# maniac-mc/maniac-mc

Measured on AMD Instinct MI355X. Metric: MC moves/sec, higher is better.
Workload: dtype f64

## Files before the change

include/maniac_gpu.h:

```cpp
#ifndef MANIAC_GPU_H
#define MANIAC_GPU_H

#ifdef __cplusplus
extern "C" {
#endif

#define MGPU_OK 0
#define MGPU_ERR_INVALID_ARG 1
#define MGPU_ERR_HIP 2
#define MGPU_ERR_CAPACITY 3
#define MGPU_ERR_NO_DEVICE 4
#define MGPU_ERR_STATE 5


#define MGPU_MOVE 0
#define MGPU_CREATION 1
#define MGPU_DELETION 2
#define MGPU_NONE 3
#define MGPU_FOURIER_ADD 4

#define MGPU_KERNEL_PAIR 0
#define MGPU_KERNEL_RECIP 1
#define MGPU_KERNEL_COMMIT 2
#define MGPU_KERNEL_SFACTOR 3
#define MGPU_KERNEL_COUNT 4

typedef struct mgpu_engine mgpu_engine;

const char *mgpu_last_error(void);

#define MGPU_ABI_VERSION 2
int mgpu_abi_version(void);

int mgpu_device_count(int *count);


int mgpu_box_prepare(const double box_matrix[9], int *box_type, double *volume,
                     double reciprocal[9], double metrics[9]);

int mgpu_ewald_setup(const double metrics[9], double *rc, double *tol, double *alpha,
                     double *screening_factor, double *fourier_precision, int kmax[3],
                     int *n_kvectors);

int mgpu_ewald_kvectors(const double reciprocal[9], double alpha, const int kmax[3], int n_kvectors,
                        int *kx, int *ky, int *kz, double *k2mag, double *form_factor,
                        double *weights);

int mgpu_coulomb_table_eval(double alpha, double r2_max, int n, const double *r2, double *out);

int mgpu_rng_seed_streams(long long seed, int n_streams, long long *state);
int mgpu_rng_fill(long long *state, int n_streams, int n_per, double *out);
void mgpu_host_prefetch(const void *p, int bytes);


int mgpu_engine_create(mgpu_engine **out, int device, int n_replicas, int n_res,
                       const int *atoms_in_res, const int *mol_capacity, int max_atom,
                       const int *atom_types, const double *charges, const int *is_active,
                       int n_types, const double *epsilon, const double *sigma,
                       const double box_matrix[9], const double bounds_lo[3],
                       double real_space_cutoff, double ewald_tolerance);
int mgpu_engine_destroy(mgpu_engine *e);

int mgpu_engine_get_ewald(const mgpu_engine *e, double *alpha, double *real_space_cutoff,
                          double *ewald_tolerance, int kmax[3], int *n_kvectors, double *volume,
                          int *box_type);
int mgpu_engine_get_kvectors(const mgpu_engine *e, int *kx, int *ky, int *kz, double *k2mag,
                             double *form_factor, double *weights);


int mgpu_replica_set_molecules(mgpu_engine *e, int replica, int t, int n_mol, const double *sites);
int mgpu_replica_get_molecules(mgpu_engine *e, int replica, int t, int *n_mol, double *sites);
int mgpu_replica_num_molecules(const mgpu_engine *e, int replica, int t, int *n_mol);
int mgpu_replica_copy(mgpu_engine *e, int dst, int src);


int mgpu_system_energy(mgpu_engine *e, int replica, double out[6]);

int mgpu_init_structure_factor(mgpu_engine *e, int replica, int mode);
int mgpu_get_structure_factor(mgpu_engine *e, int replica, double *a);
int mgpu_set_structure_factor(mgpu_engine *e, int replica, const double *a);
int mgpu_structure_factor_add(mgpu_engine *e, int replica, int t, const double *sites);


int mgpu_pair_energy_candidates(mgpu_engine *e, int n_candidates, const int *replica, const int *t,
                                const int *m, const int *use_resident, const double *sites,
                                int site_stride, double *e_non_coulomb, double *e_coulomb);

int mgpu_recip_energy_candidates(mgpu_engine *e, int n_candidates, const int *replica, const int *t,
                                 const int *m, const int *kind, const double *sites,
                                 int site_stride, double *u_recip);

#define MGPU_RECIP_TRIAL 0
#define MGPU_RECIP_COMMIT 1
#define MGPU_RECIP_FORM_ROWS 0
#define MGPU_RECIP_FORM_WIDE_VECTOR 1
#define MGPU_RECIP_FORM_WIDE_MFMA 2
#define MGPU_RECIP_FORM_WIDE_MFMA_TILED 3
#define MGPU_RECIP_FORM_PER_K 4
int mgpu_recip_form(const mgpu_engine *e, int n1_max, int kind, int out[4]);

#define MGPU_PAIR_LAYOUT_LEN 12
int mgpu_pair_layout(const mgpu_engine *e, int out[MGPU_PAIR_LAYOUT_LEN]);

int mgpu_self_energy(const mgpu_engine *e, int t, double *e_self);

int mgpu_intra_energy_candidates(mgpu_engine *e, int n_candidates, const int *replica, const int *t,
                                 const int *m, const int *use_resident, const double *sites,
                                 int site_stride, double *u_intra);

int mgpu_trial_energy_candidates(mgpu_engine *e, int n_candidates, const int *replica, const int *t,
                                 const int *m, const double *sites, int site_stride,
                                 double *old_energy, double *new_energy);

int mgpu_commit_candidates(mgpu_engine *e, int n_candidates, const int *replica, const int *t,
                           const int *m, const int *kind, const double *sites, int site_stride,
                           const int *accept);

#define MGPU_LANES 4
int mgpu_replica_set_frames(mgpu_engine *e, int replica, int t, int n_mol, const double *com, const double *off);
int mgpu_replica_get_frames(mgpu_engine *e, int replica, int t, int *n_mol, double *com, double *off);
int mgpu_move_trial_submit(mgpu_engine *e, int lane, int n_candidates, const int *replica, const int *t, const int *m,
                           const int *move, const double *u, double translation_step, double rotation_step);
int mgpu_set_triclinic_moves(mgpu_engine *e, int on);
int mgpu_replica_set_reservoir(mgpu_engine *e, int replica, int t, int n, int cap, const double *off);
int mgpu_replica_get_reservoir(mgpu_engine *e, int replica, int t, int *n, double *off);
int mgpu_farm_snapshot_submit(mgpu_engine *e, int n, const int *replicas, long long *bytes);
int mgpu_farm_snapshot_wait(mgpu_engine *e, const void **data, long long *bytes);
int mgpu_move_trial_decide_submit(mgpu_engine *e, int lane, int n_candidates, const int *replica, const int *t, const int *m,
                                  const int *move, const double *u, double translation_step, double rotation_step,
                                  const double *accept_u, const double *accept_pref, double temperature);
int mgpu_gcmc_trial_decide_submit(mgpu_engine *e, int lane, int n_candidates, const int *replica, const int *t, const int *m,
                                  const int *kind, const double *sites, int site_stride, const double *accept_u,
                                  const double *accept_pref, double temperature);
int mgpu_trial_decide_wait(mgpu_engine *e, int lane, double *old_energy, double *new_energy, int *accepted);
int mgpu_lane_site_buffer(mgpu_engine *e, int lane, int n_max, int site_stride, double **sites);
int mgpu_set_host_team(mgpu_engine *e, int n_threads);
int mgpu_trial_submit(mgpu_engine *e, int lane, int n_candidates, const int *replica, const int *t,
                      const int *m, const double *sites, int site_stride);
int mgpu_trial_wait(mgpu_engine *e, int lane, double *old_energy, double *new_energy);
int mgpu_commit_submit(mgpu_engine *e, int lane, int n_candidates, const int *replica, const int *t,
                       const int *m, const int *kind, const double *sites, int site_stride,
                       const int *accept);

int mgpu_gcmc_trial_submit(mgpu_engine *e, int lane, int n_candidates, const int *replica, const int *t,
                           const int *m, const int *kind, const double *sites, int site_stride);
int mgpu_gcmc_trial_wait(mgpu_engine *e, int lane, double *old_energy, double *new_energy);

int mgpu_replica_replace_molecule(mgpu_engine *e, int replica, int t, int m_dst, int m_src);
int mgpu_replica_set_num_molecules(mgpu_engine *e, int replica, int t, int n_mol);


int mgpu_chain_window_capacity(const mgpu_engine *e, int *max_candidates);
int mgpu_chain_set_wide(mgpu_engine *e, int on);
int mgpu_chain_window(mgpu_engine *e, int replica, int n, const int *t, const int *m, const int *kind, const int *link,
                      const double *sites, int site_stride, const double *accept_u, const double *accept_pref,
                      double temperature, double recip_energy, double *old_energy, double *new_energy,
                      int *first_accepted, int *undecided);
int mgpu_chain_set_margin(mgpu_engine *e, double relative_margin);
int mgpu_chain_get_stats(const mgpu_engine *e, long long *windows, long long *undecided);
int mgpu_chain_set_timing(mgpu_engine *e, int on);
int mgpu_chain_get_timing(mgpu_engine *e, double us[15]);

int mgpu_farm_window_capacity(const mgpu_engine *e, int *max_chains, int *max_in_flight);
int mgpu_farm_window_submit(mgpu_engine *e, int lane, int n, const int *replica, const int *t, const int *m, const int *move,
                            const int *forced, const double *u5, const double *accept_u, const double *accept_pref,
                            const double *slot_u, double t_step, double r_step, double temperature);
int mgpu_farm_window_wait(mgpu_engine *e, int lane, double *old_energy, double *new_energy, int *verdict);
int mgpu_farm_window_flush(mgpu_engine *e);
int mgpu_farm_window_get_stats(const mgpu_engine *e, long long *windows, long long *undecided);

int mgpu_chain_run_capacity(const mgpu_engine *e, int *max_k, int *max_in_flight, int *ring_steps);
int mgpu_chain_run_set_triclinic(mgpu_engine *e, int on);
int mgpu_chain_run_open(mgpu_engine *e, int replica, int k, double t_step, double r_step, double temperature);
int mgpu_chain_run_push(mgpu_engine *e, int n, const int *t, const int *m, const int *move, const double *u5, const double *accept_u);
int mgpu_chain_run_launch(mgpu_engine *e, int n_launches);
int mgpu_chain_run_collect(mgpu_engine *e, int max_steps, int wait, double *old_energy, double *new_energy, int *verdict, int *n_got,
                           int *stalled_at);
int mgpu_chain_run_force(mgpu_engine *e, int step, int accept);
int mgpu_chain_run_close(mgpu_engine *e);
int mgpu_chain_run_get_stats(mgpu_engine *e, long long *launches, long long *steps, long long *void_launches, long long *undecided);
int mgpu_chain_run_get_launches(mgpu_engine *e, int max_launches, int *first, int *consumed, int *n_got);

typedef struct mgpu_comm mgpu_comm;
#define MGPU_COMM_ID_BYTES 128
int mgpu_comm_unique_id(void *id128);
// ... 24 lines not shown
```

maniac_mc_amd/_lib.py:

```python
from __future__ import annotations

import ctypes as C
import os
import subprocess

_HERE = os.path.dirname(os.path.abspath(__file__))
LIB_PATH = os.path.join(_HERE, "libmaniac_hip.so")
CSRC = os.path.join(_HERE, "csrc")
SOURCES = ["mgpu_engine.hip", "mgpu_launch.hip", "mgpu_lanes.hip", "mgpu_windows.hip", "mgpu_host_setup.cpp", "mgpu_comm.cpp"]
HEADERS = ["mgpu_kernels.h", "mgpu_kernels_common.h", "mgpu_kernels_pair.h", "mgpu_kernels_recip.h", "mgpu_kernels_windows.h",
           "mgpu_internal.h", "mgpu_engine.h"]

MGPU_OK = 0
ABI_VERSION = 2
MGPU_MOVE, MGPU_CREATION, MGPU_DELETION, MGPU_NONE = 0, 1, 2, 3
KERNEL_PAIR, KERNEL_RECIP, KERNEL_COMMIT, KERNEL_SFACTOR = 0, 1, 2, 3
RECIP_TRIAL, RECIP_COMMIT = 0, 1
RECIP_FORMS = ("rows", "wide-vector", "wide-mfma", "wide-mfma-tiled", "per-k")
PAIR_LAYOUT_LEN = 12

EXPORTS = [
    "mgpu_last_error", "mgpu_abi_version", "mgpu_device_count", "mgpu_box_prepare", "mgpu_ewald_setup",
    "mgpu_ewald_kvectors", "mgpu_coulomb_table_eval", "mgpu_rng_seed_streams", "mgpu_rng_fill", "mgpu_host_prefetch", "mgpu_engine_create", "mgpu_engine_destroy", "mgpu_engine_get_ewald",
    "mgpu_engine_get_kvectors", "mgpu_replica_set_molecules", "mgpu_replica_get_molecules",
    "mgpu_replica_num_molecules", "mgpu_replica_copy", "mgpu_system_energy", "mgpu_init_structure_factor",
    "mgpu_get_structure_factor", "mgpu_set_structure_factor", "mgpu_structure_factor_add", "mgpu_pair_energy_candidates",
    "mgpu_recip_energy_candidates", "mgpu_recip_form", "mgpu_pair_layout", "mgpu_self_energy", "mgpu_intra_energy_candidates",
    "mgpu_trial_energy_candidates", "mgpu_commit_candidates", "mgpu_trial_submit", "mgpu_trial_wait",
    "mgpu_commit_submit", "mgpu_lane_site_buffer", "mgpu_set_host_team", "mgpu_set_triclinic_moves", "mgpu_replica_set_frames", "mgpu_replica_get_frames", "mgpu_replica_set_reservoir", "mgpu_replica_get_reservoir", "mgpu_farm_snapshot_submit", "mgpu_farm_snapshot_wait", "mgpu_move_trial_submit", "mgpu_move_trial_decide_submit", "mgpu_gcmc_trial_decide_submit", "mgpu_trial_decide_wait", "mgpu_gcmc_trial_submit", "mgpu_gcmc_trial_wait", "mgpu_replica_replace_molecule",
    "mgpu_replica_set_num_molecules", "mgpu_chain_window_capacity", "mgpu_chain_window", "mgpu_chain_set_margin", "mgpu_chain_set_wide",
    "mgpu_chain_get_stats", "mgpu_chain_set_timing", "mgpu_chain_get_timing", "mgpu_farm_window_capacity", "mgpu_farm_window_submit",
    "mgpu_farm_window_wait", "mgpu_farm_window_flush", "mgpu_farm_window_get_stats",
    "mgpu_chain_run_capacity", "mgpu_chain_run_open", "mgpu_chain_run_push", "mgpu_chain_run_launch", "mgpu_chain_run_collect",
    "mgpu_chain_run_force", "mgpu_chain_run_close", "mgpu_chain_run_get_stats", "mgpu_chain_run_get_launches", "mgpu_chain_run_set_triclinic", "mgpu_comm_unique_id", "mgpu_comm_create",
    "mgpu_comm_destroy", "mgpu_comm_rank", "mgpu_allgather_block_stats", "mgpu_append_atom_records", "mgpu_format_fixed", "mgpu_phase_factors", "mgpu_synchronize", "mgpu_profile_enable", "mgpu_profile_reset",
    "mgpu_profile_get",
]


class MgpuError(RuntimeError):
    def __init__(self, code, msg):
        super().__init__(f"maniac_gpu error {code}: {msg}")
        self.code = code


def build(force: bool = False, verbose: bool = False) -> str:
    srcs = [os.path.join(CSRC, s) for s in SOURCES]
    deps = srcs + [os.path.join(CSRC, h) for h in HEADERS if os.path.exists(os.path.join(CSRC, h))]
    deps.append(os.path.join(_HERE, "..", "include", "maniac_gpu.h"))
    if not force and os.path.exists(LIB_PATH):
        if os.path.getmtime(LIB_PATH) >= max(os.path.getmtime(d) for d in deps):
            return LIB_PATH
    from concurrent.futures import ThreadPoolExecutor
    obj_dir = os.path.join(_HERE, "..", "build", "hip_obj")
    os.makedirs(obj_dir, exist_ok=True)
    flags = ["--offload-arch=gfx950", "-O3", "-fPIC", "-std=c++17", "-fopenmp"]

    def compile_one(src):
        obj = os.path.join(obj_dir, os.path.basename(src) + ".o")
        cmd = ["hipcc"] + flags + ["-c", src, "-o", obj]
        if verbose:
            print(" ".join(cmd), flush=True)
        subprocess.check_call(cmd)
        return obj

    with ThreadPoolExecutor(max_workers=min(len(srcs), max(1, (os.cpu_count() or 2) // 2))) as pool:
        objs = list(pool.map(compile_one, srcs))
    cmd = ["hipcc", "--offload-arch=gfx950", "-fPIC", "-shared", "-fopenmp", "-o", LIB_PATH] + objs + \
          ["-L/opt/rocm/lib", "-lrccl", "-Wl,-rpath,/opt/rocm/lib"]
    if verbose:
        print(" ".join(cmd), flush=True)
    subprocess.check_call(cmd)
    return LIB_PATH


def source_digest() -> str:
    import hashlib
    h = hashlib.sha256()
    files = sorted(os.path.join(CSRC, f) for f in os.listdir(CSRC) if f.endswith((".hip", ".cpp", ".h")))
    files.append(os.path.join(_HERE, "..", "include", "maniac_gpu.h"))
    for f in files:
        h.update(os.path.basename(f).encode() + b"\0")
        with open(f, "rb") as fh:
            h.update(fh.read())
    return h.hexdigest()


_lib = None


def lib():
    global _lib
    if _lib is None:
        if not os.path.exists(LIB_PATH):
            raise RuntimeError(f"{LIB_PATH} is missing: build it with `python -c 'import __graft_entry__ as g; "
                               "g.build()'` (hipcc --offload-arch=gfx950); there is no CPU fallback")
        L = C.CDLL(LIB_PATH)
        L.mgpu_last_error.restype = C.c_char_p
        L.mgpu_abi_version.restype = C.c_int
        if L.mgpu_abi_version() != ABI_VERSION:
            raise RuntimeError(f"{LIB_PATH} reports ABI version {L.mgpu_abi_version()}, this package binds version {ABI_VERSION}: "
                               "rebuild it (python -c 'import __graft_entry__ as g; g.build()')")
        for name in EXPORTS:
            if name in ("mgpu_last_error", "mgpu_host_prefetch"):
                continue
            getattr(L, name).restype = C.c_int
        _lib = L
    return _lib


# ... 4 lines not shown
```

maniac_mc_amd/csrc/mgpu_engine.h:

```cpp
#ifndef MGPU_ENGINE_H
#define MGPU_ENGINE_H

#include <hip/hip_runtime.h>
#include <hip/hip_ext.h>

#include <algorithm>
#include <cmath>
#include <cstdio>
#include <cstdlib>
#include <cstring>
#include <deque>
#include <omp.h>
#include <string>
#include <atomic>
#include <mutex>
#include <type_traits>
#include <vector>

#include "../../include/maniac_gpu.h"
#include "mgpu_internal.h"
#include "mgpu_kernels.h"

namespace mgpu {

// ... 118 lines not shown
            if (d_res) (void)hipFree(d_res);
            if (d_tickets) (void)hipFree(d_tickets);
            h_recs = nullptr; h_out = nullptr; h_tag = nullptr; d_part = nullptr; d_res = nullptr; d_tickets = nullptr;
            cap = 0;
            pending.clear();
        }
    } farm;
    void release() {
        farm.release();
        if (commit_staged_ev) { (void)hipEventDestroy(commit_staged_ev); commit_staged_ev = nullptr; }
        d_items.release(); d_items2.release(); d_sites.release(); d_partials.release(); d_out.release();
        d_scratch.release(); d_recip_sums.release();
        d_tickets.release();
        h_in.release(); h_commit.release(); h_out.release();
    }
};
constexpr int kLanes = 4;
constexpr int kFarmDepth = 4;
constexpr int kFarmMaxChains = 4096;
constexpr int kRunRingSteps = 4096;
constexpr int kRunMaxInFlight = 64;
constexpr int kRunLaunchRing = 256;
constexpr int kRunLogMax = 1024;
constexpr size_t kChainWideRowsBytes = (size_t)kChainMaxCand * kFarmWideSites * 3 * sizeof(double);

template <class F>
void with_bools(F &&f) { f(); }
template <class F, class... Rest>
void with_bools(F &&f, bool first, Rest... rest) {
    if (first) with_bools([&](auto... cs) { f(std::true_type{}, cs...); }, rest...);
    else with_bools([&](auto... cs) { f(std::false_type{}, cs...); }, rest...);
}
template <int Lo, int Hi, class F>
bool with_int(int v, F &&f) {
    if constexpr (Lo > Hi) return false;
    else {
        if (v == Lo) { f(std::integral_constant<int, Lo>{}); return true; }
        return with_int<Lo + 1, Hi>(v, f);
    }
}
template <class F, class... Done>
void for_all_bools(F &&f, std::integral_constant<int, 0>, Done... done) { f(done...); }
template <int N, class F, class... Done>
void for_all_bools(F &&f, std::integral_constant<int, N>, Done... done) {
    for_all_bools(f, std::integral_constant<int, N - 1>{}, done..., std::false_type{});
    for_all_bools(f, std::integral_constant<int, N - 1>{}, done..., std::true_type{});
}

}

using namespace mgpu;

struct mgpu_engine {
    int device = 0;
    int n_replicas = 0;
    Lane lanes[kLanes];
    Topo tp{};
    BoxDev bx{};
    std::vector<int> atoms_in_res, mol_capacity, is_active, atom_types;
    std::vector<double> charges, epsilon, sigma;
    std::vector<int> kx, ky, kz;
    std::vector<double> k2mag, form_factor, weights;
    std::vector<int> h_nmol;
    std::vector<char> in_range;
    double rc = 0, tol = 0, alpha = 0, volume = 0;
    int box_type = 0, kmax[3] = {0, 0, 0}, nk = 0;
    double box_matrix[9]{}, bounds_lo[3]{}, reciprocal[9]{}, metrics[9]{};
    double *d_pos = nullptr;
    int *d_nmol = nullptr;
    double2 *d_A = nullptr;
    int *d_kpack = nullptr;
    double *d_kw = nullptr;
    int *d_trj = nullptr;
    double2 *d_tw = nullptr;
    int *d_kslot = nullptr;
    std::vector<int> kslot;
    int n_slots = 0;
    RecipRow *d_rrows = nullptr;
    int *d_row_first = nullptr;
    int n_rtasks = 0, n_rrows = 0;
    double2 *d_pair_tab = nullptr;
    char *d_coul_tab = nullptr;
    size_t coul_bytes = 0;
    int n_cu = 256;
    int pair_blocks_per_cu = kPairBlock >= 1024 ? 1 : 2;
    int pair_nsplit = 1;
    std::vector<double> self_of_type;
    bool rows_contiguous = false;
    bool recip_no_mfma = false;
    bool pair_fast_fold = true;
    bool recip_force_per_k = false;
    double *d_res_q = nullptr;
    int *d_res_atype = nullptr;
    std::vector<std::vector<int>> site_perm;
    std::vector<char> frozen;
    bool any_frozen = false;
    int flat_groups = 0, flat_planes = 0;
    int *d_atom_ty = nullptr;
    std::vector<std::vector<double>> frozen_ref;
    std::vector<char> frozen_same;
    std::vector<int> frozen_diff;
    bool frozen_batch = true;
    int host_team = 1;
    double *d_com = nullptr, *d_off = nullptr;
    std::vector<char> frames_ok;
    std::vector<char> frames_tight;
    std::vector<char> frames_held;
    std::vector<double *> rsv_ptr;
    std::vector<int> rsv_cap;
    std::vector<char> rsv_tight;
    double **d_rsv = nullptr;
    int *d_rsv_nc = nullptr;
    bool tri_moves = false;
    bool rsv_any = false;
    bool pair_flat = false;
    int *d_atom_res = nullptr, *d_atom_mol = nullptr;
    double *d_atom_q = nullptr;
    double *d_atom_q_on = nullptr;
    double2 *d_phase_tab = nullptr;
    double2 *d_S = nullptr;
    hipStream_t &stream = lanes[0].stream;
    DevBuf &d_items = lanes[0].d_items, &d_items2 = lanes[0].d_items2, &d_sites = lanes[0].d_sites,
           &d_partials = lanes[0].d_partials, &d_out = lanes[0].d_out;
    HostBuf &h_out = lanes[0].h_out;
    HostBuf h_stage;
    DevBuf d_snap, d_snap_items;
    HostBuf h_snap, h_snap_items;
    size_t snap_bytes = 0;
    bool snap_pending = false;
    struct Chain {
        double *h_out = nullptr;
        unsigned long long *h_tag = nullptr;
        Topo *d_topo = nullptr;
        bool topo_stale = true;
        ChainResult *d_res = nullptr;
        double2 *d_part = nullptr;
        double2 *d_alt = nullptr;
        int *d_ticket = nullptr;
        unsigned long long seq = 0;
        double margin = 16.0 * 2.220446049250313e-16;
        long long windows = 0, undecided = 0;
        bool timing = false;
        bool wide = false;
        double *h_rows = nullptr;
        size_t wide_lds_opted = 0;
    } chain;
    double2 *d_A_alt = nullptr;
    int *d_acur = nullptr;
    std::atomic<bool> a_switched{false};
    std::vector<unsigned long long> alt_owner;
    std::atomic<unsigned long long> trial_stamps{0};
    bool commit_pass = false;
    std::mutex alt_mu;
    struct Farm {
        int *d_stalled = nullptr;
        std::atomic<long long> windows{0}, undecided{0};
        std::mutex mu;
    } farm;
    struct Run {
        bool open = false;
        bool triclinic = false;
        int replica = -1, k = 0;
        double t_step = 0.0, r_step = 0.0, temperature = 0.0;
        bool fast = false;
        RunState *d_state = nullptr;
        RunRec *d_ring = nullptr, *h_ring = nullptr;
        int *h_pushed = nullptr;
        double *h_out = nullptr;
        unsigned long long *h_step_tag = nullptr;
        unsigned long long *h_launch = nullptr;
        double2 *d_part = nullptr, *d_alt = nullptr;
        ChainResult *d_res = nullptr;
        int *d_ticket = nullptr;
        long long pushed = 0, collected = 0;
        long long stalled_at = -1;
        bool dev_stalled = false;
        unsigned long long seq = 0, seq_done = 0;
        long long launches = 0, steps = 0, void_launches = 0, undecided = 0;
        std::deque<std::pair<int, int>> log;
    } run;
    bool profiling = false;
};

namespace mgpu {

const char *last_error_text();
int use_device(const mgpu_engine *e);
int prof_begin(mgpu_engine *e, Lane &ln, int kernel, hipEvent_t *a, hipEvent_t *b);
int prof_end(mgpu_engine *e, Lane &ln, int kernel, hipEvent_t a, hipEvent_t b);
int prof_collect(mgpu_engine *e, Lane &ln);
void finish_decided(mgpu_engine *e, Lane &ln);
void frozen_changed(mgpu_engine *e, int replica, int t);
int sync_lane(mgpu_engine *e, Lane &ln);
int sync_stream(mgpu_engine *e);
int sync_all_lanes(mgpu_engine *e);
int check_candidate(const mgpu_engine *e, int c, int replica, int t, int m, bool need_resident);
bool sites_in_range(const mgpu_engine *e, const double *sites, int n_sites);
bool replica_in_range(const mgpu_engine *e, int replica);
inline bool has_reservoir(const mgpu_engine *e, size_t idx) { return !e->rsv_ptr.empty() && e->rsv_ptr[idx] != nullptr; }
enum { kAdmitFrames = 1, kAdmitMove = 2, kAdmitInsertion = 4, kAdmitRange = 8, kAdmitAll = 15 };
inline int admit_built(const mgpu_engine *e, size_t idx, int k, int mv, int checks, const char *who, const char *noun, int c,
                       std::string &msg, char &ok, bool &fast) {
    if ((checks & kAdmitFrames) && (!e->d_com || !e->frames_ok[idx])) {
        msg = std::string(who) + ": no molecule frames for " + noun + " " + std::to_string(c) + " (mgpu_replica_set_frames)";
        return MGPU_ERR_STATE;
    }
    if ((checks & kAdmitMove) && (mv < 1 || mv > 4 || (k == MGPU_MOVE) != (mv <= 2) || (k == MGPU_CREATION) != (mv == 3))) {
        msg = std::string(who) + ": move code does not match the candidate kind";
        return MGPU_ERR_INVALID_ARG;
    }
    if ((checks & kAdmitInsertion) && k == MGPU_CREATION && !e->frames_held[idx] && !has_reservoir(e, idx)) {
        msg = std::string(who) + ": an insertion copies the geometry of molecule 1 of its type, and this type has never held one on this replica";
        return MGPU_ERR_STATE;
    }
    if ((checks & kAdmitRange) && k != MGPU_DELETION) { ok = e->frames_tight[idx]; fast = fast && ok; }
    return MGPU_OK;
}
int engine_nsplit(const mgpu_engine *e);
void permute_frozen_rows(const mgpu_engine *e, double *rows, int n_rows, int site_stride, const int *t);
bool any_frozen(const mgpu_engine *e, int n, const int *t);
int upload_sites(Lane &ln, const double *sites, int n_rows, int site_stride);
int upload_sites(mgpu_engine *e, const double *sites, int n_rows, int site_stride, const int *t);
double self_energy_host(const mgpu_engine *e, int t);
int normalize_A(mgpu_engine *e);
int alt_reserve(mgpu_engine *e);
void alt_forget(mgpu_engine *e, int replica);
bool one_record_per_replica(Lane &ln, int n_replicas, const int *replica, int n);
int wait_for_tag(hipStream_t stream, const volatile unsigned long long *tag, int n, unsigned long long seq, long long first_check,
                 long long check_every, const char *what);
int farm_clear_stall(mgpu_engine *e, int replica);
int chain_topo(mgpu_engine *e, const Topo **d_topo);
void chain_run_release(mgpu_engine *e);
int launch_pair(mgpu_engine *e, Lane &ln, const PairItem *d_items, int n_items, int common_n1, int site_stride,
                int nsplit, double *d_lj, double *d_c, bool ordered = false, double2 *host_partials = nullptr,
                bool fused = false, bool fast_fold = false, bool skip_frozen = false);
int frozen_chunk_atoms(const mgpu_engine *e, int n_atoms);
int launch_frozen(mgpu_engine *e, Lane &ln, const PairItem *d_items, int n_items, int n1, int site_stride, bool fused, bool fast_fold,
                  int t_frozen, double2 *d_scratch, double2 *d_extra);
static_assert((3 * sizeof(PairItem) + sizeof(RecipItem)) % 8 == 0, "the items end 8-byte aligned: TrialStaging::moves is their end");
inline TrialStaging trial_staging(int n, int site_stride, bool built, bool reservoir_pick, bool decide) {
    return trial_staging<sizeof(PairItem), sizeof(RecipItem), sizeof(DecideItem)>(n, site_stride, built, reservoir_pick, decide);
}
inline size_t lane_site_buffer_bytes(int n_max, int site_stride) {
    return lane_site_buffer_bytes<sizeof(PairItem), sizeof(RecipItem), sizeof(DecideItem)>(n_max, site_stride);
}
static_assert(sizeof(double2) == kLdsPhase && sizeof(int4) == kLdsRowRec, "mgpu_internal.h sizes the LDS tables with these");
inline int recip_ktot(const mgpu_engine *e) { return recip_ktot(e->kmax); }
inline size_t recip_rows_lds_bytes(const mgpu_engine *e, int n1_max) { return recip_rows_lds_bytes(recip_ktot(e), e->n_rrows, n1_max); }
inline size_t farm_resolver_scratch_bytes(int nsplit) { return (size_t)kPairWaves * (4 * nsplit + 4) * sizeof(double); }
bool recip_by_rows(const mgpu_engine *e, int n1_max);
struct RecipPlan {
    int form = MGPU_RECIP_FORM_ROWS;
    bool by_rows = true;
    int tile = 1;
    int mfma_tile = 0;
    int wide_rpt = 0;
    int wide_nss = 0;
    size_t lds = 0;
    size_t wide_lds = 0;
};
RecipPlan recip_plan(const mgpu_engine *e, int n1_max, bool wide_ok);
void recip_groups(const mgpu_engine *e, const RecipItem *items, int n, std::vector<RecipGroup> &groups, std::vector<int> &order);
int launch_recip(mgpu_engine *e, Lane &ln, const RecipItem *d_items, int n_items, int n1_max, int site_stride,
                 bool commit, double2 *A_base, double *d_u, double *d_u_old = nullptr, const AcceptBits *accept = nullptr,
                 const double *sites_override = nullptr, const DecideArgs *decide = nullptr, bool store_alt = false);
int launch_commit_switch(mgpu_engine *e, Lane &ln, const RecipItem *d_items, int n_items, int site_stride, const AcceptBits &accept);
int launch_sfactor(mgpu_engine *e, int replica, double2 *dst);
int launch_intra(mgpu_engine *e, Lane &ln, const PairItem *d_items, int n_items, const double *d_sites, int site_stride, double *d_out);

constexpr int kHostPartMin = 1024;
constexpr int kMaxHostParts = 16;
static int host_parts(const mgpu_engine *e, int n) {
    return (e->host_team > 1 && n >= kHostPartMin) ? std::min(e->host_team, kMaxHostParts) : 1;
}
static void part_range(int n, int parts, int part, int &c0, int &c1) {
    const int words = (n + 31) / 32;
    c0 = std::min(n, (int)((long long)words * part / parts) * 32);
    c1 = std::min(n, (int)((long long)words * (part + 1) / parts) * 32);
}
template <class F>
static void for_parts(int parts, F &&f) {
    if (parts <= 1) { f(0); return; }
#pragma omp parallel for num_threads(parts) schedule(static, 1)
    for (int part = 0; part < parts; ++part) f(part);
}
struct PartError {
    int c = -1, rc = MGPU_OK;
    std::string msg;
    void set(int cand, int code, const std::string &m) { if (c < 0) { c = cand; rc = code; msg = m; } }
};
static int report_first(const PartError *errs, int parts) {
    const PartError *first = nullptr;
    for (int q = 0; q < parts; ++q)
        if (errs[q].c >= 0 && (!first || errs[q].c < first->c)) first = &errs[q];
    return first ? set_error(first->rc, first->msg) : MGPU_OK;
}

template <class Item>
int common_site_count(const mgpu_engine *e, const std::vector<Item> &items) {
    int n1 = 0;
    for (const auto &it : items) {
// ... 11 lines not shown
```

maniac_mc_amd/csrc/mgpu_engine.hip:

```cpp
#include "mgpu_engine.h"

namespace mgpu {

static thread_local std::string g_last_error;

int set_error(int code, const std::string &msg) {
    g_last_error = msg;
    return code;
}
const char *last_error_text() { return g_last_error.c_str(); }

int use_device(const mgpu_engine *e) {
    HIP_TRY(hipSetDevice(e->device));
    return MGPU_OK;
}

int prof_begin(mgpu_engine *e, Lane &ln, int kernel, hipEvent_t *a, hipEvent_t *b) {
    if (!e->profiling) return MGPU_OK;
    for (hipEvent_t *ev : {a, b}) {
        if (!ln.ev_pool.empty()) { *ev = ln.ev_pool.back(); ln.ev_pool.pop_back(); }
        else HIP_TRY(hipEventCreate(ev));
    }
    (void)kernel;
    return MGPU_OK;
// ... 11 lines not shown
        ln.prof[p.kernel].total_ms += ms;
        ln.ev_pool.push_back(p.a);
        ln.ev_pool.push_back(p.b);
    }
    ln.pending.clear();
    return MGPU_OK;
}

void finish_decided(mgpu_engine *e, Lane &ln);
void frozen_changed(mgpu_engine *e, int replica, int t);
int sync_lane(mgpu_engine *e, Lane &ln) {
    HIP_TRY(hipStreamSynchronize(ln.stream));
    ln.dirty = false;
    if (ln.decided_n) finish_decided(e, ln);
    return prof_collect(e, ln);
}
int sync_stream(mgpu_engine *e) { return sync_lane(e, e->lanes[0]); }
int sync_all_lanes(mgpu_engine *e) {
    for (auto &ln : e->lanes)
        if (&ln == &e->lanes[0] || ln.dirty || !ln.pending.empty())
            if (int rc = sync_lane(e, ln)) return rc;
    if (e->a_switched) return normalize_A(e);
    alt_forget(e, -1);
    return MGPU_OK;
}

void finish_decided(mgpu_engine *e, Lane &ln) {
    const int n = ln.decided_n;
    ln.decided_n = 0;
    const int *flags = (const int *)((const char *)ln.h_out.p + ln.result.flags_bytes());
    const RecipItem *items = ln.h_trial_items;
    for (int c = 0; c < n; ++c) {
        if (!flags[c]) continue;
        const int idx = items[c].replica * e->tp.n_res + items[c].t;
        if (items[c].kind == MGPU_CREATION) e->h_nmol[idx] += 1;
        if (items[c].kind == MGPU_DELETION) e->h_nmol[idx] -= 1;
        if (items[c].kind != MGPU_DELETION && !(c < (int)ln.cand_ok.size() && ln.cand_ok[c])) e->in_range[idx] = 0;
        frozen_changed(e, items[c].replica, items[c].t);
    }
    ln.forget_trial();
}

bool one_record_per_replica(Lane &ln, int n_replicas, const int *replica, int n) {
    if ((int)ln.mark.size() != n_replicas) ln.mark.assign(n_replicas, -1);
    bool twice = false;
    for (int c = 0; c < n; ++c) {
        twice = twice || ln.mark[replica[c]] == -3;
        ln.mark[replica[c]] = -3;
    }
    for (int c = 0; c < n; ++c) ln.mark[replica[c]] = -1;
    return !twice;
}

void frozen_changed(mgpu_engine *e, int replica, int t) {
    if (!e->frozen[t]) return;
    auto clear = [&](int r) {
        char &f = e->frozen_same[(size_t)r * e->tp.n_res + t];
        if (f) { e->frozen_diff[t] += 1; f = 0; }
    };
    if (replica == 0) for (int r = 0; r < e->n_replicas; ++r) clear(r);
    else clear(replica);
}
int check_candidate(const mgpu_engine *e, int c, int replica, int t, int m, bool need_resident) {
    if (replica < 0 || replica >= e->n_replicas)
        return set_error(MGPU_ERR_INVALID_ARG, "candidate " + std::to_string(c) + ": replica out of range");
    if (t < 0 || t >= e->tp.n_res)
        return set_error(MGPU_ERR_INVALID_ARG, "candidate " + std::to_string(c) + ": residue type out of range");
    const int nm = e->h_nmol[replica * e->tp.n_res + t];
    if (m >= nm || m < -1)
        return set_error(MGPU_ERR_INVALID_ARG, "candidate " + std::to_string(c) + ": molecule slot " +
                                                   std::to_string(m) + " not live (count " + std::to_string(nm) + ")");
    if (need_resident && m < 0)
        return set_error(MGPU_ERR_INVALID_ARG, "candidate " + std::to_string(c) + ": needs a resident molecule");
    return MGPU_OK;
}

constexpr double kFastFoldRange = 0.745;
bool sites_in_range(const mgpu_engine *e, const double *sites, int n_sites) {
    for (int i = 0; i < n_sites; ++i)
        for (int d = 0; d < 3; ++d)
            if (!(std::fabs(sites[3 * (size_t)i + d] - e->bx.ctr[d]) <= kFastFoldRange * e->bx.L[d])) return false;
    return true;
}
bool replica_in_range(const mgpu_engine *e, int replica) {
    for (int t = 0; t < e->tp.n_res; ++t)
        if (!e->in_range[(size_t)replica * e->tp.n_res + t]) return false;
    return true;
}

int engine_nsplit(const mgpu_engine *e) {
    int units = 0;
    for (int t = 0; t < e->tp.n_res; ++t) {
        const int cap = e->tp.cap[t], n1 = e->tp.n1[t];
        units += e->tp.site_major[t] ? cap * ((n1 + 63) / 64) : n1 * ((cap + 63) / 64);
    }
    int cap_split = 32, per_wave = 2;
    if (e->n_replicas >= 48 && e->n_replicas <= 1024) {
        const int want = (e->n_replicas < 512 ? 1024 : 2048) / e->n_replicas;
        cap_split = 2;
        while (cap_split * 2 <= std::min(want, 32)) cap_split *= 2;
    } else if (e->n_replicas >= 256) {
        per_wave = 8;
        int want = std::max(1, e->n_cu * 64 / e->n_replicas);
        if (units <= 128) want *= 2;
        const int cap_want = e->n_replicas >= 1024 ? std::min(want, 4) : std::min(want / 4, 16);
        cap_split = 1;
        while (cap_split * 2 <= cap_want) cap_split *= 2;
    }
    int ns = std::max(1, std::min(units / per_wave, cap_split));
    if (const char *ov = std::getenv("MGPU_PAIR_NSPLIT")) ns = std::max(1, std::min(std::atoi(ov), std::max(1, units)));
    return ns;
}

void permute_frozen_rows(const mgpu_engine *e, double *rows, int n_rows, int site_stride, const int *t) {
    std::vector<double> tmp;
    for (int c = 0; c < n_rows; ++c) {
        if (t[c] < 0 || t[c] >= e->tp.n_res || !e->frozen[t[c]]) continue;
        const int n1 = e->tp.n1[t[c]];
        if (n1 > site_stride) continue;
        double *r = rows + (size_t)c * site_stride * 3;
        tmp.assign(r, r + (size_t)n1 * 3);
        const int *perm = e->site_perm[t[c]].data();
        for (int a = 0; a < n1; ++a)
            for (int d = 0; d < 3; ++d) r[(size_t)perm[a] * 3 + d] = tmp[(size_t)a * 3 + d];
    }
}
bool any_frozen(const mgpu_engine *e, int n, const int *t) {
    for (int c = 0; c < n; ++c)
        if (t[c] >= 0 && t[c] < e->tp.n_res && e->frozen[t[c]]) return true;
    return false;
}

int upload_sites(Lane &ln, const double *sites, int n_rows, int site_stride) {
    if (!sites || n_rows == 0) return MGPU_OK;
    ln.forget_trial();
    const size_t bytes = (size_t)n_rows * site_stride * 3 * sizeof(double);
    int rc = ln.d_sites.reserve(bytes);
    if (rc) return rc;
    HIP_TRY(hipMemcpyAsync(ln.d_sites.p, sites, bytes, hipMemcpyHostToDevice, ln.stream));
    return MGPU_OK;
}
int upload_sites(mgpu_engine *e, const double *sites, int n_rows, int site_stride, const int *t) {
    if (sites && n_rows > 0 && any_frozen(e, n_rows, t)) {
        const size_t bytes = (size_t)n_rows * site_stride * 3 * sizeof(double);
        int rc = e->h_stage.reserve(bytes);
        if (rc) return rc;
        std::memcpy(e->h_stage.p, sites, bytes);
        permute_frozen_rows(e, (double *)e->h_stage.p, n_rows, site_stride, t);
        if ((rc = upload_sites(e->lanes[0], (const double *)e->h_stage.p, n_rows, site_stride))) return rc;
        HIP_TRY(hipStreamSynchronize(e->lanes[0].stream));
        return MGPU_OK;
    }
    return upload_sites(e->lanes[0], sites, n_rows, site_stride);
}

double self_energy_host(const mgpu_engine *e, int t) {
    double s = 0.0;
    const double sqrtpi = std::sqrt(kPi);
    for (int a = 0; a < e->tp.n1[t]; ++a) {
        const double q = e->charges[(size_t)t * e->tp.max_atom + a];
        if (std::fabs(q) < kErrorTol) continue;
        s = s - e->alpha / sqrtpi * (q * q);
    }
    return s * kEps0InvEvA / kKbEvK;
}

// ... 243 lines not shown
        for (size_t r = 0; r < rrows.size(); ++r)
            for (int j = 0; j <= e->kmax[2]; ++j)
                if (plus[r][j] >= 0 || minus[r][j] >= 0) rtasks.push_back(RecipTask{plus[r][j], minus[r][j], (int)r, j});
        size_t covered = 0;
        for (const auto &tk : rtasks) covered += (tk.kp >= 0) + (tk.km >= 0);
        if (covered != (size_t)e->nk) { rrows.clear(); rtasks.clear(); }
        e->rows_contiguous = !rtasks.empty() && e->kmax[2] < 255;
        for (size_t ti = 1; ti < rtasks.size(); ++ti)
            if (rtasks[ti].row == rtasks[ti - 1].row && rtasks[ti].j != rtasks[ti - 1].j + 1) e->rows_contiguous = false;
    }
    e->n_rrows = (int)rrows.size();
    e->n_rtasks = (int)rtasks.size();
    e->kslot.assign(e->nk, 0);
    std::vector<int> trj(rtasks.size());
    std::vector<double2> tw(rtasks.size());
    if (e->n_rtasks > 0) {
        e->n_slots = 2 * e->n_rtasks;
        for (size_t ti = 0; ti < rtasks.size(); ++ti) {
            const RecipTask &tk = rtasks[ti];
            trj[ti] = (tk.row << 8) | tk.j | (tk.kp >= 0 ? kTaskHasP : 0) | (tk.km >= 0 ? kTaskHasM : 0);
            tw[ti] = make_double2(tk.kp >= 0 ? kw[tk.kp] : 0.0, tk.km >= 0 ? kw[tk.km] : 0.0);
            if (tk.kp >= 0) e->kslot[tk.kp] = 2 * (int)ti;
            if (tk.km >= 0) e->kslot[tk.km] = 2 * (int)ti + 1;
        }
    } else {
        e->n_slots = e->nk;
        for (int i = 0; i < e->nk; ++i) e->kslot[i] = i;
    }
    bx.n_slots = e->n_slots;
    std::vector<double2> ptab((size_t)n_types * n_types);
    for (int i = 0; i < n_types * n_types; ++i) ptab[i] = make_double2(4.0 * epsilon[i], sigma[i] * sigma[i]);
    std::vector<int> atype0((size_t)n_res * max_atom, 0);
    std::vector<double> q_dev((size_t)n_res * max_atom, 0.0);
    for (int t = 0; t < n_res; ++t)
        for (int a = 0; a < atoms_in_res[t]; ++a) {
            const int ap = e->site_perm[t][a];
            atype0[(size_t)t * max_atom + ap] = atom_types[(size_t)t * max_atom + a] - 1;
            q_dev[(size_t)t * max_atom + ap] = charges[(size_t)t * max_atom + a];
        }
    std::vector<int> a_res(tp.n_cap_atoms), a_mol(tp.n_cap_atoms), a_ty(tp.n_cap_atoms);
    std::vector<double> a_q(tp.n_cap_atoms);
    for (int t = 0; t < n_res; ++t)
        for (int m = 0; m < tp.cap[t]; ++m)
            for (int a = 0; a < tp.n1[t]; ++a) {
                const int ap = e->site_perm[t][a];
                const int j = tp.site_major[t] ? tp.seg_off[t] + m * tp.n1[t] + ap : tp.seg_off[t] + ap * tp.cap[t] + m;
                a_res[j] = t; a_mol[j] = m; a_q[j] = charges[(size_t)t * max_atom + a];
                a_ty[j] = atom_types[(size_t)t * max_atom + a] - 1;
            }

    auto fail = [&](int code) { mgpu_engine_destroy(e); return code; };
#define HIP_TRY_E(expr)                                                                                          \
    do {                                                                                                         \
        hipError_t err__ = (expr);                                                                               \
        if (err__ != hipSuccess)                                                                                 \
            return fail(set_error(MGPU_ERR_HIP, std::string(#expr) + ": " + hipGetErrorString(err__)));          \
    } while (0)
    HIP_TRY_E(hipSetDevice(device));
    for (auto &ln : e->lanes) HIP_TRY_E(hipStreamCreateWithFlags(&ln.stream, hipStreamNonBlocking));
    const size_t ncap = tp.n_cap_atoms, R = n_replicas;
    const int ktot = recip_ktot(e);
    HIP_TRY_E(hipMalloc(&e->d_pos, R * 3 * ncap * sizeof(double)));
    HIP_TRY_E(hipMemset(e->d_pos, 0, R * 3 * ncap * sizeof(double)));
    HIP_TRY_E(hipMalloc(&e->d_nmol, R * n_res * sizeof(int)));
    HIP_TRY_E(hipMemset(e->d_nmol, 0, R * n_res * sizeof(int)));
    HIP_TRY_E(hipMalloc(&e->d_A, R * e->n_slots * sizeof(double2)));
    HIP_TRY_E(hipMemset(e->d_A, 0, R * e->n_slots * sizeof(double2)));
    HIP_TRY_E(hipMalloc(&e->d_kpack, e->nk * sizeof(int)));
    HIP_TRY_E(hipMalloc(&e->d_kw, e->nk * sizeof(double)));
    HIP_TRY_E(hipMalloc(&e->d_pair_tab, ptab.size() * sizeof(double2)));
    {
        std::vector<CoulRow> rows;
        const double sum_len = e->metrics[0] + e->metrics[1] + e->metrics[2];
        const double s_max = bx.triclinic ? sum_len * sum_len
                                          : 0.25 * (bx.L[0] * bx.L[0] + bx.L[1] * bx.L[1] + bx.L[2] * bx.L[2]) * 1.0001;
        int idx_base = 0;
        if (int rc2 = build_coulomb_table(e->alpha, std::max(s_max, 1.0), rows, &idx_base)) return fail(rc2);
        e->bx.coul_idx_base = idx_base;
        e->bx.coul_last_row = (int)rows.size() - 1;
        e->coul_bytes = rows.size() * sizeof(CoulRow);
        if (e->coul_bytes + 16 * 1024 > 150 * 1024) return fail(set_error(MGPU_ERR_CAPACITY, "Coulomb table does not fit LDS"));
        HIP_TRY_E(hipMalloc(&e->d_coul_tab, e->coul_bytes));
        HIP_TRY_E(hipMemcpy(e->d_coul_tab, rows.data(), e->coul_bytes, hipMemcpyHostToDevice));
    }
    {
        hipDeviceProp_t prop;
        HIP_TRY_E(hipGetDeviceProperties(&prop, device));
        e->n_cu = std::max(1, prop.multiProcessorCount);
        e->pair_nsplit = engine_nsplit(e);
    }
    HIP_TRY_E(hipMalloc(&e->d_res_q, e->charges.size() * sizeof(double)));
    HIP_TRY_E(hipMalloc(&e->d_res_atype, atype0.size() * sizeof(int)));
    HIP_TRY_E(hipMalloc(&e->d_atom_res, ncap * sizeof(int)));
    HIP_TRY_E(hipMalloc(&e->d_atom_mol, ncap * sizeof(int)));
    HIP_TRY_E(hipMalloc(&e->d_atom_q, ncap * sizeof(double)));
    HIP_TRY_E(hipMalloc(&e->d_atom_q_on, ncap * sizeof(double)));
    HIP_TRY_E(hipMalloc(&e->d_phase_tab, (size_t)ktot * ncap * sizeof(double2)));
    HIP_TRY_E(hipMalloc(&e->d_S, e->n_slots * sizeof(double2)));
    HIP_TRY_E(hipMemset(e->d_S, 0, e->n_slots * sizeof(double2)));
    HIP_TRY_E(hipMalloc(&e->d_kslot, e->nk * sizeof(int)));
    HIP_TRY_E(hipMemcpy(e->d_kslot, e->kslot.data(), e->nk * sizeof(int), hipMemcpyHostToDevice));
    HIP_TRY_E(hipMemcpy(e->d_kpack, kpack.data(), e->nk * sizeof(int), hipMemcpyHostToDevice));
    if (e->n_rtasks > 0) {
        HIP_TRY_E(hipMalloc(&e->d_trj, trj.size() * sizeof(int)));
        HIP_TRY_E(hipMalloc(&e->d_tw, tw.size() * sizeof(double2)));
        HIP_TRY_E(hipMalloc(&e->d_rrows, rrows.size() * sizeof(RecipRow)));
        HIP_TRY_E(hipMemcpy(e->d_trj, trj.data(), trj.size() * sizeof(int), hipMemcpyHostToDevice));
        HIP_TRY_E(hipMemcpy(e->d_tw, tw.data(), tw.size() * sizeof(double2), hipMemcpyHostToDevice));
        HIP_TRY_E(hipMemcpy(e->d_rrows, rrows.data(), rrows.size() * sizeof(RecipRow), hipMemcpyHostToDevice));
        std::vector<int> row_first(rrows.size() + 1, (int)rtasks.size());
        for (int ti = (int)rtasks.size() - 1; ti >= 0; --ti) row_first[rtasks[ti].row] = ti;
        HIP_TRY_E(hipMalloc(&e->d_row_first, row_first.size() * sizeof(int)));
        HIP_TRY_E(hipMemcpy(e->d_row_first, row_first.data(), row_first.size() * sizeof(int), hipMemcpyHostToDevice));
    }
    HIP_TRY_E(hipMemcpy(e->d_kw, kw.data(), e->nk * sizeof(double), hipMemcpyHostToDevice));
    HIP_TRY_E(hipMemcpy(e->d_pair_tab, ptab.data(), ptab.size() * sizeof(double2), hipMemcpyHostToDevice));
    HIP_TRY_E(hipMemcpy(e->d_res_q, q_dev.data(), q_dev.size() * sizeof(double), hipMemcpyHostToDevice));
    HIP_TRY_E(hipMalloc(&e->d_atom_ty, ncap * sizeof(int)));
    HIP_TRY_E(hipMemcpy(e->d_atom_ty, a_ty.data(), ncap * sizeof(int), hipMemcpyHostToDevice));
    tp.slot_q = e->d_atom_q;
    tp.slot_ty = e->d_atom_ty;
    HIP_TRY_E(hipMemcpy(e->d_res_atype, atype0.data(), atype0.size() * sizeof(int), hipMemcpyHostToDevice));
    HIP_TRY_E(hipMemcpy(e->d_atom_res, a_res.data(), ncap * sizeof(int), hipMemcpyHostToDevice));
    HIP_TRY_E(hipMemcpy(e->d_atom_mol, a_mol.data(), ncap * sizeof(int), hipMemcpyHostToDevice));
    HIP_TRY_E(hipMemcpy(e->d_atom_q, a_q.data(), ncap * sizeof(double), hipMemcpyHostToDevice));
    {
        std::vector<double> a_q_on(a_q);
        for (double &q : a_q_on)
            if (!(std::fabs(q) >= kErrorTol)) q = 0.0;
        HIP_TRY_E(hipMemcpy(e->d_atom_q_on, a_q_on.data(), ncap * sizeof(double), hipMemcpyHostToDevice));
    }
#undef HIP_TRY_E
    e->self_of_type.resize(n_res);
    for (int t = 0; t < n_res; ++t) e->self_of_type[t] = self_energy_host(e, t);
    *out = e;
    return MGPU_OK;
}

int mgpu_engine_destroy(mgpu_engine *e) {
    if (!e) return MGPU_OK;
    (void)hipSetDevice(e->device);
    for (auto &ln : e->lanes) if (ln.stream) (void)hipStreamSynchronize(ln.stream);
    for (void *p : {(void *)e->d_pos, (void *)e->d_nmol, (void *)e->d_A, (void *)e->d_kpack, (void *)e->d_kw,
                    (void *)e->d_pair_tab, (void *)e->d_coul_tab, (void *)e->d_res_q, (void *)e->d_res_atype, (void *)e->d_atom_res,
                    (void *)e->d_atom_mol, (void *)e->d_atom_q, (void *)e->d_atom_q_on, (void *)e->d_phase_tab, (void *)e->d_S, (void *)e->d_trj,
                    (void *)e->d_tw, (void *)e->d_kslot, (void *)e->d_rrows, (void *)e->d_row_first, (void *)e->d_atom_ty, (void *)e->d_com, (void *)e->d_off})
        if (p) (void)hipFree(p);
    for (double *p : e->rsv_ptr)
        if (p) (void)hipFree(p);
    for (void *p : {(void *)e->d_rsv, (void *)e->d_rsv_nc})
        if (p) (void)hipFree(p);
    e->h_stage.release();
    e->h_snap.release();
    e->h_snap_items.release();
    e->d_snap.release();
    e->d_snap_items.release();
    for (void *p : {(void *)e->chain.h_out, (void *)e->chain.h_tag, (void *)e->chain.h_rows})
        if (p) (void)hipHostFree(p);
    for (void *p : {(void *)e->chain.d_res, (void *)e->chain.d_part, (void *)e->chain.d_ticket, (void *)e->chain.d_topo, (void *)e->chain.d_alt,
                    (void *)e->d_A_alt, (void *)e->d_acur, (void *)e->farm.d_stalled})
        if (p) (void)hipFree(p);
    chain_run_release(e);
    for (auto &ln : e->lanes) {
        ln.release();
        for (auto &p : ln.pending) { (void)hipEventDestroy(p.a); (void)hipEventDestroy(p.b); }
        if (ln.stream) (void)hipStreamDestroy(ln.stream);
    }
    for (auto &ln : e->lanes)
        for (auto ev : ln.ev_pool) (void)hipEventDestroy(ev);
    delete e;
    return MGPU_OK;
}

int mgpu_engine_get_ewald(const mgpu_engine *e, double *alpha, double *rc, double *tol, int kmax[3], int *nk,
                          double *volume, int *box_type) {
    if (!e) return set_error(MGPU_ERR_INVALID_ARG, "null engine");
    if (alpha) *alpha = e->alpha;
    if (rc) *rc = e->rc;
    if (tol) *tol = e->tol;
    if (kmax) { kmax[0] = e->kmax[0]; kmax[1] = e->kmax[1]; kmax[2] = e->kmax[2]; }
    if (nk) *nk = e->nk;
    if (volume) *volume = e->volume;
    if (box_type) *box_type = e->box_type;
    return MGPU_OK;
}

int mgpu_engine_get_kvectors(const mgpu_engine *e, int *kx, int *ky, int *kz, double *k2mag, double *ff, double *w) {
    if (!e) return set_error(MGPU_ERR_INVALID_ARG, "null engine");
    if (kx) std::memcpy(kx, e->kx.data(), e->nk * sizeof(int));
    if (ky) std::memcpy(ky, e->ky.data(), e->nk * sizeof(int));
    if (kz) std::memcpy(kz, e->kz.data(), e->nk * sizeof(int));
    if (k2mag) std::memcpy(k2mag, e->k2mag.data(), e->nk * sizeof(double));
    if (ff) std::memcpy(ff, e->form_factor.data(), e->nk * sizeof(double));
    if (w) std::memcpy(w, e->weights.data(), e->nk * sizeof(double));
    return MGPU_OK;
}


static int check_replica_t(const mgpu_engine *e, int replica, int t) {
    if (!e) return set_error(MGPU_ERR_INVALID_ARG, "null engine");
    if (replica < 0 || replica >= e->n_replicas) return set_error(MGPU_ERR_INVALID_ARG, "replica out of range");
    if (t < 0 || t >= e->tp.n_res) return set_error(MGPU_ERR_INVALID_ARG, "residue type out of range");
    return MGPU_OK;
}

int mgpu_replica_set_molecules(mgpu_engine *e, int replica, int t, int n_mol, const double *sites) {
    int rc = check_replica_t(e, replica, t);
    if (rc) return rc;
    if (n_mol < 0 || n_mol > e->tp.cap[t]) return set_error(MGPU_ERR_CAPACITY, "n_mol exceeds the residue type's mol_capacity");
    if (n_mol > 0 && !sites) return set_error(MGPU_ERR_INVALID_ARG, "null sites");
    if ((rc = use_device(e))) return rc;
    const Topo &tp = e->tp;
    const int n1 = tp.n1[t], cap = tp.cap[t];
    const size_t seg = (size_t)n1 * cap;
    rc = e->h_stage.reserve(3 * seg * sizeof(double));
    if (rc) return rc;
    double *st = (double *)e->h_stage.p;
    std::memset(st, 0, 3 * seg * sizeof(double));
    const int *perm = e->site_perm[t].data();
    for (int m = 0; m < n_mol; ++m)
        for (int a = 0; a < n1; ++a) {
            const size_t j = tp.site_major[t] ? (size_t)m * n1 + perm[a] : (size_t)a * cap + m;
            for (int d = 0; d < 3; ++d) st[d * seg + j] = sites[((size_t)m * n1 + a) * 3 + d];
        }
    if ((rc = sync_all_lanes(e))) return rc;
    if ((rc = farm_clear_stall(e, replica))) return rc;
    for (int d = 0; d < 3; ++d)
// ... 617 lines not shown
```

maniac_mc_amd/csrc/mgpu_host_setup.cpp:

```cpp
#include <cmath>
#include <cstdio>
#include <cstring>
#include <string>
#include <vector>

#include "../../include/maniac_gpu.h"
#include "mgpu_internal.h"

namespace mgpu {

static inline void cross3(const double a[3], const double b[3], double c[3]) {
    c[0] = a[1] * b[2] - a[2] * b[1];
    c[1] = a[2] * b[0] - a[0] * b[2];
    c[2] = a[0] * b[1] - a[1] * b[0];
}
static inline double dot3(const double a[3], const double b[3]) {
    return a[0] * b[0] + a[1] * b[1] + a[2] * b[2];
}

int box_prepare(const double m[9], int *box_type, double *volume, double rcp[9], double metrics[9]) {
    if (!m || !box_type || !volume || !rcp || !metrics) return set_error(MGPU_ERR_INVALID_ARG, "box_prepare: null argument");
    const double od[6] = {m[1], m[2], m[3], m[5], m[6], m[7]};
    double mx = 0.0;
    for (double v : od) mx = std::fmax(mx, std::fabs(v));
// ... 82 lines not shown
    for (int i = 0; i < nk; ++i) w[i] = std::exp(-k2mag[i] / (4.0 * a2)) / k2mag[i];
    return MGPU_OK;
}

int build_coulomb_table(double alpha, double s_max, std::vector<CoulRow> &rows, int *idx_base) {
    if (!(alpha > 0.0) || !(s_max > 0.0) || !std::isfinite(s_max))
        return set_error(MGPU_ERR_INVALID_ARG, "build_coulomb_table: bad alpha / range");
    int emax = kCoulEmin;
    while (std::ldexp(1.0, emax + 1) <= s_max) ++emax;
    if (emax - kCoulEmin + 1 > 40) return set_error(MGPU_ERR_CAPACITY, "build_coulomb_table: range too large");
    const int per_oct = 1 << kCoulM, n_oct = emax - kCoulEmin + 1;
    rows.assign((size_t)n_oct * per_oct + 1, CoulRow{});
    *idx_base = (1023 + kCoulEmin) * per_oct;
    constexpr int N = kCoulDeg + 1;
    const long double pi = 3.14159265358979323846264338327950288L;
    long double node[N], cosjk[N][N];
    for (int k = 0; k < N; ++k) {
        node[k] = cosl(pi * (2 * k + 1) / (2.0L * N));
        for (int j = 0; j < N; ++j) cosjk[j][k] = cosl(pi * j * (2 * k + 1) / (2.0L * N));
    }
    long double T[N][N] = {};
    T[0][0] = 1.0L;
    T[1][1] = 1.0L;
    for (int j = 2; j < N; ++j)
        for (int i = 0; i < N; ++i) T[j][i] = (i > 0 ? 2.0L * T[j - 1][i - 1] : 0.0L) - T[j - 2][i];
    long double binom[N][N] = {};
    for (int j = 0; j < N; ++j) {
        binom[j][0] = 1.0L;
        for (int i = 1; i <= j; ++i) binom[j][i] = binom[j - 1][i - 1] + (i <= j - 1 ? binom[j - 1][i] : 0.0L);
    }
    const long double al = alpha;
    for (int o = 0; o < n_oct; ++o)
        for (int q = 0; q < per_oct; ++q) {
            const long double base = ldexpl(1.0L, kCoulEmin + o);
            const long double a = base * (1.0L + (long double)q / per_oct), b = base * (1.0L + (long double)(q + 1) / per_oct);
            long double f[N], c[N], mono[N] = {}, tc[N] = {};
            for (int k = 0; k < N; ++k) {
                const long double sv = 0.5L * (a + b) + 0.5L * (b - a) * node[k], r = sqrtl(sv);
                f[k] = erfcl(al * r) / r;
            }
            for (int j = 0; j < N; ++j) {
                long double acc = 0.0L;
                for (int k = 0; k < N; ++k) acc += f[k] * cosjk[j][k];
                c[j] = acc * 2.0L / N;
            }
            c[0] *= 0.5L;
            for (int j = 0; j < N; ++j)
                for (int i = 0; i <= j; ++i) mono[i] += c[j] * T[j][i];
            for (int j = 0; j < N; ++j)
                for (int i = 0; i <= j; ++i) {
                    const long double sign = ((j - i) & 1) ? -1.0L : 1.0L;
                    tc[i] += mono[j] * binom[j][i] * ldexpl(1.0L, i) * sign;
                }
            CoulRow &row = rows[(size_t)o * per_oct + q];
            const int sh = kCoulM - (kCoulEmin + o);
            for (int i = 0; i < 5; ++i) row.c[i] = (double)ldexpl(tc[i], sh * i);
            row.c5 = (float)ldexpl(tc[5], sh * 5);
            row.c6 = (float)ldexpl(tc[6], sh * 6);
        }
    return MGPU_OK;
}

double coulomb_table_eval_host(const std::vector<CoulRow> &rows, int idx_base, double alpha, double s) {
    unsigned long long bits;
    std::memcpy(&bits, &s, 8);
    const int hi = (int)(bits >> 32);
    int row = (hi >> (20 - kCoulM)) - idx_base;
    if (row < 0) {
        const double r = std::sqrt(s);
        return std::erfc(alpha * r) / r;
    }
    const int last = (int)rows.size() - 1;
    if (row > last) row = last;
    const unsigned long long ab = bits & ~((1ull << (52 - kCoulM)) - 1);
    double a;
    std::memcpy(&a, &ab, 8);
    const double t = s - a;
    const CoulRow &r = rows[row];
    double p = std::fma((double)r.c6, t, (double)r.c5);
    for (int i = 4; i >= 0; --i) p = std::fma(p, t, r.c[i]);
    return p;
}

}

namespace {

bool format_fixed(char *out, int w, int d, double x) {
    if (!std::isfinite(x)) return false;
    const bool neg = std::signbit(x);
    const double ax = std::fabs(x);
    auto stars = [&]() { std::memset(out, '*', (size_t)w); return true; };
    int e = 0;
    unsigned long long m = 0;
    if (ax != 0.0) {
        const double fr = std::frexp(ax, &e);
        m = (unsigned long long)std::ldexp(fr, 53);
        e -= 53;
    }
    if (e >= 0 && m != 0) return stars();
    static const unsigned long long p10[] = {1ull, 10ull, 100ull, 1000ull, 10000ull, 100000ull, 1000000ull, 10000000ull, 100000000ull,
                                             1000000000ull};
    if (d < 0 || d > 9) return false;
    unsigned __int128 P = (unsigned __int128)m * p10[d];
    unsigned __int128 N = 0;
    const int sh = -e;
    if (m != 0) {
        if (sh >= 127) {
            N = 0;
        } else {
            N = P >> sh;
            const unsigned __int128 rem = P & ((((unsigned __int128)1) << sh) - 1), half = ((unsigned __int128)1) << (sh - 1);
            if (rem > half || (rem == half && (N & 1))) N += 1;
        }
    }
    if (N >> 64) return stars();
    const unsigned long long n64 = (unsigned long long)N, ip = n64 / p10[d], fp = n64 % p10[d];
    char tmp[64];
    int len = 0;
    char digits[24];
    int nd = 0;
    unsigned long long v = ip;
    do { digits[nd++] = (char)('0' + v % 10); v /= 10; } while (v);
    if (neg) tmp[len++] = '-';
    for (int k = nd - 1; k >= 0; --k) tmp[len++] = digits[k];
    tmp[len++] = '.';
    for (int k = d - 1; k >= 0; --k) tmp[len++] = (char)('0' + (fp / p10[k]) % 10);
    if (len > w) {
        if (ip == 0 && len - 1 == w) {
            std::memmove(tmp + (neg ? 1 : 0), tmp + (neg ? 2 : 1), (size_t)(len - (neg ? 2 : 1)));
            len -= 1;
        } else {
            return stars();
        }
    }
    std::memset(out, ' ', (size_t)(w - len));
    std::memcpy(out + (w - len), tmp, (size_t)len);
    return true;
}

void format_int(char *out, int w, long long v) {
    char tmp[32];
    const int len = std::snprintf(tmp, sizeof tmp, "%lld", v);
    if (len > w) { std::memset(out, '*', (size_t)w); return; }
    std::memset(out, ' ', (size_t)(w - len));
    std::memcpy(out + (w - len), tmp, (size_t)len);
}

}

using mgpu::set_error;

extern "C" {

int mgpu_append_atom_records(const char *path, int n, int first_serial, const int *mol, const int *type, const double *charge,
                             const double *xyz) {
    if (!path || n < 0 || !type || !xyz || (mol && !charge)) return set_error(MGPU_ERR_INVALID_ARG, "append_atom_records: bad argument");
    const int reclen = mol ? (6 + 1 + 6 + 1 + 4 + 1 + 12 + 3 * 13 + 1) : (6 + 1 + 4 + 3 * 13 + 1);
    std::vector<char> buf((size_t)n * reclen);
    for (int i = 0; i < n; ++i) {
        char *r = buf.data() + (size_t)i * reclen;
        int at = 0;
        format_int(r + at, 6, (long long)first_serial + i); at += 6;
        r[at++] = ' ';
        if (mol) {
            format_int(r + at, 6, mol[i]); at += 6;
            r[at++] = ' ';
        }
        format_int(r + at, 4, type[i]); at += 4;
        if (mol) {
            r[at++] = ' ';
            if (!format_fixed(r + at, 12, 8, charge[i])) return set_error(MGPU_ERR_INVALID_ARG, "append_atom_records: charge not finite");
            at += 12;
        }
        for (int dd = 0; dd < 3; ++dd) {
            r[at++] = ' ';
            if (!format_fixed(r + at, 12, 7, xyz[(size_t)i * 3 + dd])) return set_error(MGPU_ERR_INVALID_ARG, "append_atom_records: coordinate not finite");
            at += 12;
        }
        r[at++] = '\n';
    }
    FILE *f = std::fopen(path, "ab");
    if (!f) return set_error(MGPU_ERR_STATE, std::string("append_atom_records: cannot open ") + path);
    const size_t wrote = buf.empty() ? 0 : std::fwrite(buf.data(), 1, buf.size(), f);
    const int rc = std::fclose(f);
    if (wrote != buf.size() || rc != 0) return set_error(MGPU_ERR_STATE, std::string("append_atom_records: short write to ") + path);
    return MGPU_OK;
}

int mgpu_format_fixed(int n, const double *x, int w, int d, char *out) {
    if (n < 0 || !x || !out || w < 1 || w > 40) return set_error(MGPU_ERR_INVALID_ARG, "format_fixed: bad argument");
    for (int i = 0; i < n; ++i)
        if (!format_fixed(out + (size_t)i * w, w, d, x[i])) std::memset(out + (size_t)i * w, '?', (size_t)w);
    return MGPU_OK;
}

int mgpu_box_prepare(const double box_matrix[9], int *box_type, double *volume, double reciprocal[9], double metrics[9]) {
    return mgpu::box_prepare(box_matrix, box_type, volume, reciprocal, metrics);
}

int mgpu_ewald_setup(const double metrics[9], double *rc, double *tol, double *alpha, double *screening_factor,
                     double *fourier_precision, int kmax[3], int *n_kvectors) {
    return mgpu::ewald_setup(metrics, rc, tol, alpha, screening_factor, fourier_precision, kmax, n_kvectors);
}

int mgpu_coulomb_table_eval(double alpha, double r2_max, int n, const double *r2, double *out) {
    if (n < 0 || (n > 0 && (!r2 || !out))) return mgpu::set_error(MGPU_ERR_INVALID_ARG, "mgpu_coulomb_table_eval: bad argument");
    std::vector<mgpu::CoulRow> rows;
    int idx_base = 0;
    int rc = mgpu::build_coulomb_table(alpha, r2_max, rows, &idx_base);
    if (rc) return rc;
    for (int k = 0; k < n; ++k) out[k] = mgpu::coulomb_table_eval_host(rows, idx_base, alpha, r2[k]);
    return MGPU_OK;
}

void mgpu_host_prefetch(const void *p, int bytes) {
    for (int o = 0; o < bytes; o += 64) __builtin_prefetch((const char *)p + o, 0, 3);
}

int mgpu_rng_seed_streams(long long seed, int n_streams, long long *state) {
    if (n_streams < 0 || (n_streams > 0 && !state)) return mgpu::set_error(MGPU_ERR_INVALID_ARG, "mgpu_rng_seed_streams: bad argument");
    auto splitmix = [](unsigned long long &x) {
        unsigned long long z = (x += 0x9e3779b97f4a7c15ULL);
        z = (z ^ (z >> 30)) * 0xbf58476d1ce4e5b9ULL;
        z = (z ^ (z >> 27)) * 0x94d049bb133111ebULL;
        return z ^ (z >> 31);
    };
    unsigned long long base = (unsigned long long)seed;
    base = splitmix(base);
    for (int r = 0; r < n_streams; ++r) {
        unsigned long long x = base + 0xd1342543de82ef95ULL * (unsigned long long)(r + 1);
        unsigned long long w[4];
        do {
            for (auto &v : w) v = splitmix(x);
        } while ((w[0] | w[1] | w[2] | w[3]) == 0ULL);
        for (int i = 0; i < 4; ++i) state[4 * (size_t)r + i] = (long long)w[i];
    }
    return MGPU_OK;
}

namespace {
inline void rng_fill_scalar(unsigned long long *st, int n, int n_per, double *out) {
    for (int r = 0; r < n; ++r) {
        unsigned long long s0 = st[4 * (size_t)r], s1 = st[4 * (size_t)r + 1], s2 = st[4 * (size_t)r + 2], s3 = st[4 * (size_t)r + 3];
        double *o = out + (size_t)r * n_per;
        for (int i = 0; i < n_per; ++i) {
            o[i] = (double)((s0 + s3) >> 11) * (1.0 / 9007199254740992.0);
            const unsigned long long t = s1 << 17;
            s2 ^= s0; s3 ^= s1; s1 ^= s2; s0 ^= s3;
            s2 ^= t;
            s3 = (s3 << 45) | (s3 >> 19);
        }
        st[4 * (size_t)r] = s0; st[4 * (size_t)r + 1] = s1; st[4 * (size_t)r + 2] = s2; st[4 * (size_t)r + 3] = s3;
    }
}
#if defined(__x86_64__)
#include <immintrin.h>
__attribute__((target("avx2"))) void rng_fill_avx2(unsigned long long *st, int n, int n_per, double *out) {
    const __m256i magic = _mm256_set1_epi64x(0x4330000000000000LL);
    const __m256d two52 = _mm256_set1_pd(4503599627370496.0), two32 = _mm256_set1_pd(4294967296.0);
    const __m256d scale = _mm256_set1_pd(1.0 / 9007199254740992.0);
    const __m256i lo_mask = _mm256_set1_epi64x(0xffffffffLL);
    int r = 0;
    for (; r + 4 <= n; r += 4) {
        const __m256i a = _mm256_loadu_si256((const __m256i *)(st + 4 * (size_t)r)), b = _mm256_loadu_si256((const __m256i *)(st + 4 * (size_t)r + 4));
        const __m256i c = _mm256_loadu_si256((const __m256i *)(st + 4 * (size_t)r + 8)), d = _mm256_loadu_si256((const __m256i *)(st + 4 * (size_t)r + 12));
        const __m256i ab_lo = _mm256_unpacklo_epi64(a, b), ab_hi = _mm256_unpackhi_epi64(a, b);
        const __m256i cd_lo = _mm256_unpacklo_epi64(c, d), cd_hi = _mm256_unpackhi_epi64(c, d);
        __m256i s0 = _mm256_permute2x128_si256(ab_lo, cd_lo, 0x20), s1 = _mm256_permute2x128_si256(ab_hi, cd_hi, 0x20);
        __m256i s2 = _mm256_permute2x128_si256(ab_lo, cd_lo, 0x31), s3 = _mm256_permute2x128_si256(ab_hi, cd_hi, 0x31);
        for (int i = 0; i < n_per; ++i) {
            const __m256i x = _mm256_srli_epi64(_mm256_add_epi64(s0, s3), 11);
            const __m256d hi = _mm256_sub_pd(_mm256_castsi256_pd(_mm256_or_si256(_mm256_srli_epi64(x, 32), magic)), two52);
            const __m256d lo = _mm256_sub_pd(_mm256_castsi256_pd(_mm256_or_si256(_mm256_and_si256(x, lo_mask), magic)), two52);
            const __m256d v = _mm256_mul_pd(_mm256_add_pd(_mm256_mul_pd(hi, two32), lo), scale);
            alignas(32) double tmp[4];
            _mm256_store_pd(tmp, v);
            for (int q = 0; q < 4; ++q) out[(size_t)(r + q) * n_per + i] = tmp[q];
            const __m256i t = _mm256_slli_epi64(s1, 17);
            s2 = _mm256_xor_si256(s2, s0); s3 = _mm256_xor_si256(s3, s1); s1 = _mm256_xor_si256(s1, s2); s0 = _mm256_xor_si256(s0, s3);
            s2 = _mm256_xor_si256(s2, t);
            s3 = _mm256_or_si256(_mm256_slli_epi64(s3, 45), _mm256_srli_epi64(s3, 19));
        }
        const __m256i t0 = _mm256_unpacklo_epi64(s0, s1), t1 = _mm256_unpackhi_epi64(s0, s1);
        const __m256i t2 = _mm256_unpacklo_epi64(s2, s3), t3 = _mm256_unpackhi_epi64(s2, s3);
        _mm256_storeu_si256((__m256i *)(st + 4 * (size_t)r), _mm256_permute2x128_si256(t0, t2, 0x20));
        _mm256_storeu_si256((__m256i *)(st + 4 * (size_t)r + 4), _mm256_permute2x128_si256(t1, t3, 0x20));
        _mm256_storeu_si256((__m256i *)(st + 4 * (size_t)r + 8), _mm256_permute2x128_si256(t0, t2, 0x31));
        _mm256_storeu_si256((__m256i *)(st + 4 * (size_t)r + 12), _mm256_permute2x128_si256(t1, t3, 0x31));
    }
    if (r < n) rng_fill_scalar(st + 4 * (size_t)r, n - r, n_per, out + (size_t)r * n_per);
}
#endif
}

// ... 21 lines not shown
```

maniac_mc_amd/csrc/mgpu_internal.h:

```cpp
#ifndef MGPU_INTERNAL_H
#define MGPU_INTERNAL_H

#include <algorithm>
#include <cstddef>
#include <string>
#include <vector>

namespace mgpu {

constexpr double kPi = 3.14159265358979323846;
constexpr double kTwoPi = 2.0 * kPi;
constexpr double kEps0InvEvA = 14.40198;
constexpr double kKbEvK = 8.6173852e-5;
constexpr double kErrorTol = 1.0e-10;

int set_error(int code, const std::string &msg);

int box_prepare(const double m[9], int *box_type, double *volume, double rcp[9], double metrics[9]);
int ewald_setup(const double metrics[9], double *rc, double *tol, double *alpha, double *screening,
                double *fourier_precision, int kmax[3], int *nk);
int ewald_kvectors(const double rcp[9], double alpha, const int kmax[3], int nk, int *kx, int *ky, int *kz,
                   double *k2mag, double *ff, double *w);

constexpr int kCoulM = 6;
constexpr int kCoulDeg = 6;
constexpr int kCoulEmin = -2;
constexpr double kCoulSlowBelow = 0.25;
struct CoulRow {
    double c[5];
    float c5, c6;
};
static_assert(sizeof(CoulRow) == 48, "CoulRow must be three 16-byte LDS reads");
constexpr int kCoulRowVec = sizeof(CoulRow) / 16;
int build_coulomb_table(double alpha, double s_max, std::vector<CoulRow> &rows, int *idx_base);
double coulomb_table_eval_host(const std::vector<CoulRow> &rows, int idx_base, double alpha, double s);

constexpr size_t kLdsDefaultMax = 64 * 1024;
constexpr size_t kLdsPhase = 16, kLdsRowRec = 16;
inline int recip_ktot(const int kmax[3]) { return kmax[0] + kmax[1] + kmax[2] + 3; }
inline size_t recip_lds_bytes(int ktot, int n1) { return (size_t)2 * n1 * ktot * kLdsPhase + (size_t)n1 * sizeof(double); }
inline size_t recip_rows_lds_bytes(int ktot, int n_rrows, int n1) {
    return recip_lds_bytes(ktot, n1) + (size_t)n_rrows * (2 * n1 * kLdsPhase);
}
inline size_t recip_wide_lds_bytes(int ktot, int n_rrows, size_t nss, int rpt, bool mfma) {
    return nss * ktot * kLdsPhase + (size_t)rpt * nss * kLdsPhase + nss * sizeof(double) + (mfma ? (size_t)n_rrows * kLdsRowRec : 0);
}
constexpr size_t kRecipTileBytes = 48 * 1024;
constexpr size_t kRecipRowsLdsMax = 40 * 1024;
constexpr size_t kRecipWideTableBytes = 40 * 1024, kRecipWideLdsBytes = 60 * 1024;
inline int recip_tile_sites(int ktot, int n1_max) {
    return std::max(1, std::min(n1_max, (int)(kRecipTileBytes / recip_lds_bytes(ktot, 1))));
}
inline int recip_wide_rows_per_tile(int ktot, int n_rrows, int n1_max) {
    const size_t nss = (size_t)2 * n1_max, tables = recip_wide_lds_bytes(ktot, 0, nss, 0, false);
    if (tables > kRecipWideTableBytes) return 0;
    const int rpt = (int)((kRecipWideLdsBytes - tables) / (nss * kLdsPhase));
    return rpt >= 8 ? std::min(rpt, n_rrows) : 0;
}
inline int recip_wide_mfma_tile(int ktot, int n_rrows, int n1_max) {
    const size_t nss = ((size_t)2 * n1_max + 3) & ~(size_t)3;
    const size_t per_ss = recip_wide_lds_bytes(ktot, 0, 1, 0, false), fixed = recip_wide_lds_bytes(ktot, n_rrows, 0, 0, true);
    if (fixed + 4 * per_ss > kRecipWideLdsBytes) return 0;
    const size_t fit = ((kRecipWideLdsBytes - fixed) / per_ss) & ~(size_t)3;
    const size_t n_tiles = (nss + fit - 1) / fit;
    return (int)((((nss + n_tiles - 1) / n_tiles) + 3) & ~(size_t)3);
}

constexpr int kWideRowSites = 64;
constexpr size_t wide_k_front_bytes() { return (size_t)kWideRowSites * 3 * sizeof(double) + 2 * (size_t)kWideRowSites * 4 * sizeof(double); }
inline size_t chain_wide_k_lds_bytes(size_t form_bytes) { return wide_k_front_bytes() + form_bytes; }
inline size_t chain_wide_pair_at(size_t coul_bytes) { return (coul_bytes + 15) & ~(size_t)15; }
constexpr size_t wide_pair_slab_bytes(int pair_waves, int site_chunk) {
    return (size_t)pair_waves * (((size_t)kWideRowSites * 3 + (size_t)site_chunk * 4) * sizeof(double) + (size_t)site_chunk * sizeof(int));
}
inline size_t chain_wide_pair_lds_bytes(size_t coul_bytes, int pair_waves, int site_chunk) {
    return chain_wide_pair_at(coul_bytes) + wide_pair_slab_bytes(pair_waves, site_chunk);
}
inline size_t chain_resolver_lds_bytes(int n_ent, int nsplit) { return (size_t)n_ent * nsplit * kLdsPhase; }
inline int chain_window_steps_by_lds(int nsplit) { return (int)(kLdsDefaultMax / chain_resolver_lds_bytes(2, nsplit)); }
inline size_t chain_run_resolver_lds_bytes(int k, int nsplit) { return chain_resolver_lds_bytes(2 * k, nsplit); }

struct TrialStaging {
    int row_sites, frame_at, pick_at;
    size_t sites, pair_items, k_items, intra_items, moves, uniforms, decide_items, total;
};
template <size_t PairB, size_t RecipB, size_t DecideB>
inline TrialStaging trial_staging(int n, int site_stride, bool built, bool reservoir_pick, bool decide) {
    const auto up8 = [](size_t v) { return (v + 7) & ~(size_t)7; };
    TrialStaging s{};
    s.row_sites = built ? 2 * site_stride + 1 + (reservoir_pick ? 1 : 0) : site_stride;
    s.frame_at = built ? site_stride : 0;
    s.pick_at = built && reservoir_pick ? 2 * site_stride + 1 : 0;
    s.pair_items = (size_t)n * s.row_sites * 3 * sizeof(double);
    s.k_items = s.pair_items + 2 * (size_t)n * PairB;
    s.intra_items = s.k_items + (size_t)n * RecipB;
    s.moves = up8(s.intra_items + (size_t)n * PairB);
    s.uniforms = s.moves + up8((size_t)n * sizeof(int));
    s.decide_items = up8(built ? s.uniforms + (size_t)5 * n * sizeof(double) : s.moves);
    s.total = s.decide_items + (decide ? (size_t)n * DecideB : 0);
    return s;
}
template <size_t PairB, size_t RecipB, size_t DecideB>
inline size_t lane_site_buffer_bytes(int n_max, int site_stride) {
    const TrialStaging host = trial_staging<PairB, RecipB, DecideB>(n_max, site_stride, false, false, true);
    const TrialStaging built = trial_staging<PairB, RecipB, DecideB>(n_max, site_stride, true, true, true);
    return std::max(host.total + 16, built.total + 32 + (size_t)n_max * sizeof(int) + 8 - (built.uniforms - built.moves));
}
struct TrialResult {
    size_t partials, u_old, u_new, intra, extra, flags, total;
    size_t flags_bytes() const { return flags * sizeof(double); }
};
inline TrialResult trial_result(int n, int n_partials, int n_pair, bool frozen_extra, bool decide) {
    TrialResult r{};
    r.u_old = 2 * (size_t)n_partials;
    r.u_new = r.u_old + n;
    r.intra = r.u_new + n;
    r.extra = r.intra + n;
    r.flags = r.extra + (frozen_extra ? 2 * (size_t)n_pair : 0);
// ... 8 lines not shown
```

maniac_mc_amd/csrc/mgpu_kernels_common.h:

```cpp
#ifndef MGPU_KERNELS_COMMON_H
#define MGPU_KERNELS_COMMON_H

#include <hip/hip_runtime.h>

#include <type_traits>

#include "mgpu_internal.h"

namespace mgpu {

constexpr int kMaxRes = 8;
constexpr int kBlock = 256;
constexpr int kWavesPerBlock = kBlock / 64;
constexpr int kSiteChunk = 32;
#ifndef MGPU_PAIR_BLOCK
#define MGPU_PAIR_BLOCK 512
#endif
#ifndef MGPU_PAIR_MINWAVES
#define MGPU_PAIR_MINWAVES 4
#endif
constexpr int kPairBlock = MGPU_PAIR_BLOCK;
constexpr int kPairWaves = kPairBlock / 64;
constexpr int kMaxTypes = 16;
constexpr int kMaxGrp = 32;
// ... 146 lines not shown
__device__ __forceinline__ double image_r2_search27(double dx, double dy, double dz, const double *__restrict__ m) {
    double best = 1.7976931348623157e308;
    for (int sx = -1; sx <= 1; ++sx)
        for (int sy = -1; sy <= 1; ++sy)
            for (int sz = -1; sz <= 1; ++sz) {
                const double tx = dx + sx * m[0] + sy * m[1] + sz * m[2];
                const double ty = dy + sx * m[3] + sy * m[4] + sz * m[5];
                const double tz = dz + sx * m[6] + sy * m[7] + sz * m[8];
                const double t2 = fma(tz, tz, fma(ty, ty, tx * tx));
                best = t2 < best ? t2 : best;
            }
    return best;
}

template <bool TRI>
__device__ __forceinline__ double image_r2(double dx, double dy, double dz, const BoxDev &bx) {
    if constexpr (TRI) {
        if (bx.tri_lower) {
            double r2;
            if (!image_r2_tri_lower(dx, dy, dz, bx, r2)) r2 = image_r2_search27(dx, dy, dz, bx.m);
            return r2;
        }
    }
    if constexpr (!TRI) {
        dx = min_image(dx, bx.L[0], bx.invL[0]);
        dy = min_image(dy, bx.L[1], bx.invL[1]);
        dz = min_image(dz, bx.L[2], bx.invL[2]);
        return fma(dz, dz, fma(dy, dy, dx * dx));
    } else {
        double best = 1.7976931348623157e308;
        for (int sx = -1; sx <= 1; ++sx)
            for (int sy = -1; sy <= 1; ++sy)
                for (int sz = -1; sz <= 1; ++sz) {
                    const double tx = dx + sx * bx.m[0] + sy * bx.m[1] + sz * bx.m[2];
                    const double ty = dy + sx * bx.m[3] + sy * bx.m[4] + sz * bx.m[5];
                    const double tz = dz + sx * bx.m[6] + sy * bx.m[7] + sz * bx.m[8];
                    const double t2 = fma(tz, tz, fma(ty, ty, tx * tx));
                    best = t2 < best ? t2 : best;
                }
        return best;
    }
}

__device__ __forceinline__ double image_r2_fast(double dx, double dy, double dz, const BoxDev &bx) {
    const double ax = fabs(dx), ay = fabs(dy), az = fabs(dz);
    const double mx = fmin(ax, bx.L[0] - ax), my = fmin(ay, bx.L[1] - ay), mz = fmin(az, bx.L[2] - az);
    return fma(mz, mz, fma(my, my, mx * mx));
}

__device__ __forceinline__ double fast_rsqrt(double x) {
    const double y = __builtin_amdgcn_rsq(x);
    const double e = fma(-(x * y), y, 1.0);
    return fma(y * e, fma(0.375, e, 0.5), y);
}

__device__ __forceinline__ double fast_rcp(double x) {
    const double y = __builtin_amdgcn_rcp(x);
    const double e = fma(-x, y, 1.0);
    return fma(y, fma(e, e, e), y);
}

__device__ __forceinline__ const char *coul_tab_adjusted(const char *tab, int idx_base) {
    return tab - (size_t)idx_base * sizeof(CoulRow);
}
__device__ __forceinline__ double coul_lds(double s, const char *__restrict__ tab_adj, unsigned &sh_out) {
    const int hi = __double2hiint(s);
    const unsigned sh = (unsigned)hi >> (20 - kCoulM);
    sh_out = sh;
    constexpr int kMant = (1 << (20 - kCoulM)) - 1;
    const double s0 = __hiloint2double(hi & ~kMant, 0);
    const double t = s - s0;
    const double2 *r = reinterpret_cast<const double2 *>(tab_adj + __umul24(sh, (unsigned)sizeof(CoulRow)));
    const double2 c01 = r[0], c23 = r[1], c4f = r[2];
    const double c5 = (double)__int_as_float(__double2loint(c4f.y));
    double p = fma((double)__int_as_float(__double2hiint(c4f.y)), t, c5);
    p = fma(p, t, c4f.x);
    p = fma(p, t, c23.y);
    p = fma(p, t, c23.x);
    p = fma(p, t, c01.y);
    p = fma(p, t, c01.x);
    return p;
}

__device__ __attribute__((noinline)) double coul_slow(double s, double alpha, bool guard) {
    const double r = sqrt(s);
    if (guard && r < kErrorTol) return 0.0;
    return erfc(alpha * r) / r;
}

template <bool GUARD_R0, bool TRI, bool FASTW = false>
__device__ __forceinline__ void pair_term(double dx, double dy, double dz, const BoxDev &bx, double qq,
                                          double eps4, double sig2, bool do_lj, bool do_c,
                                          const char *__restrict__ coul_tab, double &elj, double &ec) {
    const double r2 = FASTW ? image_r2_fast(dx, dy, dz, bx) : image_r2<TRI>(dx, dy, dz, bx);
    if (do_lj) {
        const double s2 = sig2 * fast_rcp(r2);
        const double s6 = s2 * s2 * s2;
        const double e = eps4 * fma(s6, s6, -s6);
        elj += (r2 < bx.rc2) ? e : 0.0;
    }
    if (do_c) {
        unsigned sh;
        double g = coul_lds(r2, coul_tab_adjusted(coul_tab, bx.coul_idx_base), sh);
        if (sh >= (unsigned)(bx.coul_idx_base + bx.coul_last_row)) g = 0.0;
        if (sh < (unsigned)bx.coul_idx_base) g = coul_slow(r2, bx.alpha, GUARD_R0);
        ec += qq * g;
    }
}

}

#endif
```

maniac_mc_amd/csrc/mgpu_kernels_pair.h:

```cpp
#ifndef MGPU_KERNELS_PAIR_H
#define MGPU_KERNELS_PAIR_H

#include "mgpu_kernels_common.h"

namespace mgpu {

template <int NS, bool ORDERED, bool TRI, bool FUSED, bool FASTW, bool SC1OUT = false>
__device__ __forceinline__ void pair_sweep_item(
    const Topo &tp, const BoxDev &bx, const double *__restrict__ pos, const int *__restrict__ nmol,
    const double *__restrict__ res_q, const int *__restrict__ res_atype, const double2 *__restrict__ pair_tab,
    const char *__restrict__ s_coul, const double2 *__restrict__ s_pair, double *__restrict__ w_site, int *__restrict__ w_sty,
    const PairItem it, const double *__restrict__ cand_sites, int site_stride, int split, int nsplit, int lane,
    double2 *__restrict__ partials, int w) {
    static_assert(!FUSED || (NS > 0 && !ORDERED && !TRI), "the fused old + new sweep is a register-site, unordered, orthorhombic path");
    static_assert(!FASTW || (NS > 0 && !ORDERED && !TRI), "the two-instruction fold is a register-site, unordered, orthorhombic path");
    constexpr int NTY = NS > 0 ? NS : 1;
    constexpr int NST = FUSED ? 2 : 1;
    constexpr int NREG = NTY * NST;
    const int nt = tp.n_types;
    [[maybe_unused]] const char *coul_adj = coul_tab_adjusted(s_coul, bx.coul_idx_base);
    {
        const double *px = pos + (size_t)it.replica * 3 * tp.n_cap_atoms;
        const double *py = px + tp.n_cap_atoms, *pz = py + tp.n_cap_atoms;
        const int *nm_r = nmol + it.replica * tp.n_res;
        const int n1 = NS > 0 ? NS : tp.n1[it.t];
        constexpr bool ordered = ORDERED;

        auto load_site = [&](int a, double &x, double &y, double &z) {
            if (it.src < 0) {
                const int j = atom_slot(tp, it.t, it.m, a);
                x = px[j]; y = py[j]; z = pz[j];
            } else {
                const double *c = cand_sites + ((size_t)it.src * site_stride + a) * 3;
                x = c[0]; y = c[1]; z = c[2];
            }
        };
        double rx[NREG], ry[NREG], rz[NREG], rq[NTY];
        int rty[NTY];
        if constexpr (NS > 0) {
#pragma unroll
            for (int a = 0; a < NTY; ++a) {
                if constexpr (FUSED) {
                    const int j = atom_slot(tp, it.t, it.m, a);
                    rx[a] = px[j]; ry[a] = py[j]; rz[a] = pz[j];
                    const double *c = cand_sites + ((size_t)it.src * site_stride + a) * 3;
                    rx[NTY + a] = c[0]; ry[NTY + a] = c[1]; rz[NTY + a] = c[2];
                    asm volatile("" : "+v"(rx[NTY + a]), "+v"(ry[NTY + a]), "+v"(rz[NTY + a]));
                } else {
                    load_site(a, rx[a], ry[a], rz[a]);
                }
                rq[a] = res_q[it.t * tp.max_atom + a];
                rty[a] = res_atype[it.t * tp.max_atom + a];
                asm volatile("" : "+v"(rx[a]), "+v"(ry[a]), "+v"(rz[a]));
            }
        }

        double elj[NST], ec[NST];
#pragma unroll
        for (int st = 0; st < NST; ++st) { elj[st] = 0.0; ec[st] = 0.0; }
        for (int sb = 0; sb < n1; sb += kSiteChunk) {
            const int ns = NS > 0 ? NS : min(kSiteChunk, n1 - sb);
            if constexpr (NS == 0) {
                __builtin_amdgcn_fence(__ATOMIC_ACQ_REL, "wavefront");
                __builtin_amdgcn_wave_barrier();
                if (lane < ns) {
                    double x, y, z;
                    load_site(sb + lane, x, y, z);
                    w_site[lane * 4 + 0] = x; w_site[lane * 4 + 1] = y; w_site[lane * 4 + 2] = z;
                    w_site[lane * 4 + 3] = res_q[it.t * tp.max_atom + sb + lane];
                    w_sty[lane] = res_atype[it.t * tp.max_atom + sb + lane];
                }
                __builtin_amdgcn_fence(__ATOMIC_ACQ_REL, "wavefront");
                __builtin_amdgcn_wave_barrier();
            }
            for (int t2 = 0, plane_base = 0; t2 < tp.n_res; plane_base += tp.n1[t2], ++t2) {
                if (ordered && t2 < it.t) continue;
                const int nm = nm_r[t2], n2 = tp.n1[t2];
                if (nm == 0) continue;
                const bool same_t = (t2 == it.t) && (it.m >= 0);
                [[maybe_unused]] auto plane_sweep = [&](const double *pxp, const double *pyp, const double *pzp,
                                                        int nm, bool excl, int dummy_m, double qj, int tyj, int key) {
                    const int cpp = (nm + 63) >> 6;
                    const bool qj_on = fabs(qj) >= kErrorTol;
                    double e4[NTY], sg2[NTY], qq[NTY];
                    bool lj[NTY], c_on[NTY];
                    bool any_c = false, all_c = true, any_lj = false;
#pragma unroll
                    for (int s = 0; s < NTY; ++s) {
                        const double2 pt = pair_tab[rty[s] * nt + tyj];
                        e4[s] = pt.x; sg2[s] = pt.y;
                        lj[s] = pt.x != 0.0;
                        c_on[s] = qj_on && (fabs(rq[s]) >= kErrorTol);
                        qq[s] = c_on[s] ? rq[s] * qj : 0.0;
                        any_c = any_c || c_on[s]; all_c = all_c && c_on[s]; any_lj = any_lj || lj[s];
                    }
                    if (!(any_c || any_lj)) return;
                    int c = split - (key * cpp) % nsplit;
                    if (c < 0) c += nsplit;
                    if (c >= cpp) return;
                    auto is_special = [&](int cc) {
                        return ORDERED || (cc == cpp - 1 && (nm & 63) != 0) || (excl && cc == (it.m >> 6));
                    };
                    auto fetch = [&](int cc, bool special, double &x, double &y, double &z, bool &ok) {
                        int m2 = cc * 64 + lane;
                        ok = true;
                        if (special) {
                            asm volatile("" ::: "memory");
                            ok = m2 < nm;
                            if (excl) ok = ok && (ORDERED ? (m2 > it.m) : (m2 != it.m));
                            m2 = ok ? m2 : dummy_m;
                        }
                        const unsigned ob = (unsigned)m2 * 8u;
                        x = *reinterpret_cast<const double *>(reinterpret_cast<const char *>(pxp) + ob);
                        y = *reinterpret_cast<const double *>(reinterpret_cast<const char *>(pyp) + ob);
                        z = *reinterpret_cast<const double *>(reinterpret_cast<const char *>(pzp) + ob);
                    };
                    double acc[NREG];
#pragma unroll
                    for (int s = 0; s < NREG; ++s) acc[s] = 0.0;
                    auto sweep_plane = [&](auto all_tag) {
                        constexpr bool ALL_C = decltype(all_tag)::value;
                        auto unit = [&](double xj, double yj, double zj, double wq, bool valid) {
                            const double rc2l = valid ? bx.rc2 : -1.0;
                            double r2[NREG], g[NREG];
                            unsigned sh_min = ~0u;
                            if constexpr (TRI) {
                                bool ok = bx.tri_lower != 0;
                                if (ok) {
#pragma unroll
                                    for (int s = 0; s < NREG; ++s) ok = image_r2_tri_lower(xj - rx[s], yj - ry[s], zj - rz[s], bx, r2[s]) && ok;
                                }
                                if (!__all(ok)) {
                                    asm volatile("" ::: "memory");
#pragma unroll
                                    for (int s = 0; s < NREG; ++s) r2[s] = image_r2_search27(xj - rx[s], yj - ry[s], zj - rz[s], bx.m);
                                }
                            } else {
#pragma unroll
                                for (int s = 0; s < NREG; ++s) {
                                    r2[s] = FASTW ? image_r2_fast(xj - rx[s], yj - ry[s], zj - rz[s], bx)
                                                  : image_r2<false>(xj - rx[s], yj - ry[s], zj - rz[s], bx);
                                }
                            }
#pragma unroll
                            for (int s = 0; s < NREG; ++s) {
                                if (!ALL_C && !c_on[s % NTY]) { g[s] = 0.0; continue; }
                                unsigned sh;
                                g[s] = coul_lds(r2[s], coul_adj, sh);
                                sh_min = min(sh_min, sh);
                            }
                            if (sh_min < (unsigned)bx.coul_idx_base) {
#pragma unroll
                                for (int s = 0; s < NREG; ++s)
                                    if ((ALL_C || c_on[s % NTY]) && r2[s] < kCoulSlowBelow) g[s] = coul_slow(r2[s], bx.alpha, ORDERED);
                            }
#pragma unroll
                            for (int s = 0; s < NREG; ++s)
                                if (ALL_C || c_on[s % NTY]) acc[s] = fma(wq, g[s], acc[s]);
                            if (any_lj) {
#pragma unroll
                                for (int s = 0; s < NREG; ++s) {
                                    if (!lj[s % NTY]) continue;
                                    const double s2 = sg2[s % NTY] * fast_rcp(r2[s]);
                                    const double s6 = s2 * s2 * s2;
                                    const double e = e4[s % NTY] * fma(s6, s6, -s6);
                                    elj[s / NTY] += (r2[s] < rc2l) ? e : 0.0;
                                }
                            }
                        };
                        double xj, yj, zj;
                        bool valid, special = is_special(c);
                        fetch(c, special, xj, yj, zj, valid);
                        for (; c < cpp; c += nsplit) {
                            double xn = xj, yn = yj, zn = zj;
                            bool vn = true;
                            const bool special_n = is_special(c + nsplit);
                            if (c + nsplit < cpp) fetch(c + nsplit, special_n, xn, yn, zn, vn);
                            unit(xj, yj, zj, valid ? 1.0 : 0.0, valid);
                            xj = xn; yj = yn; zj = zn; valid = vn; special = special_n;
                        }
                    };
                    if (all_c) sweep_plane(std::true_type{});
                    else sweep_plane(std::false_type{});
#pragma unroll
                    for (int s = 0; s < NREG; ++s) ec[s / NTY] = fma(qq[s % NTY], acc[s], ec[s / NTY]);
                };
                if (!tp.site_major[t2]) {
                    if constexpr (NS > 0) {
                        const int cap2 = tp.cap[t2], seg2 = tp.seg_off[t2];
                        int dummy_m = 0;
                        if (same_t) {
                            if (ORDERED) { if (it.m + 1 >= nm) continue; dummy_m = nm - 1; }
                            else { if (nm == 1) continue; dummy_m = (it.m == 0) ? 1 : 0; }
                        }
                        for (int a2 = 0; a2 < n2; ++a2) {
                            const double qj = res_q[t2 * tp.max_atom + a2];
                            const int tyj = res_atype[t2 * tp.max_atom + a2];
                            plane_sweep(px + seg2 + a2 * cap2, py + seg2 + a2 * cap2, pz + seg2 + a2 * cap2, nm, same_t, dummy_m, qj, tyj,
                                        plane_base + a2);
                        }
                    } else {
                        const int cpp = (nm + 63) >> 6, units = n2 * cpp;
                        for (int u = split; u < units; u += nsplit) {
                            const int a2 = u / cpp, m2 = (u - a2 * cpp) * 64 + lane;
                            bool valid = m2 < nm;
                            if (same_t) valid = valid && (ordered ? (m2 > it.m) : (m2 != it.m));
                            const double qj = res_q[t2 * tp.max_atom + a2];
                            const int tyj = res_atype[t2 * tp.max_atom + a2];
                            const bool qj_on = fabs(qj) >= kErrorTol;
                            double xj = 0.0, yj = 0.0, zj = 0.0;
                            if (valid) {
                                const int j = tp.seg_off[t2] + a2 * tp.cap[t2] + m2;
                                xj = px[j]; yj = py[j]; zj = pz[j];
                            }
                            for (int s = 0; s < ns; ++s) {
                                const double qs = w_site[s * 4 + 3];
                                const double2 pt = s_pair[w_sty[s] * nt + tyj];
                                const bool do_c = qj_on && (fabs(qs) >= kErrorTol);
                                const bool do_lj = pt.x != 0.0;
                                if ((do_c || do_lj) && valid)
                                    pair_term<ORDERED, TRI>(xj - w_site[s * 4 + 0], yj - w_site[s * 4 + 1], zj - w_site[s * 4 + 2],
                                                       bx, qs * qj, pt.x, pt.y, do_lj, do_c, s_coul, elj[0], ec[0]);
                            }
                        }
                    }
                } else {
                    const int cpp = (n2 + 63) >> 6, units = nm * cpp;
                    for (int u = split; u < units; u += nsplit) {
                        const int m2 = u / cpp, a2 = (u - m2 * cpp) * 64 + lane;
                        if (same_t && (ordered ? (m2 <= it.m) : (m2 == it.m))) continue;
                        const bool valid = a2 < n2;
                        double xj = 0.0, yj = 0.0, zj = 0.0, qj = 0.0;
                        int tyj = 0;
                        if (valid) {
                            const int j = tp.seg_off[t2] + m2 * n2 + a2;
                            xj = px[j]; yj = py[j]; zj = pz[j];
                            qj = res_q[t2 * tp.max_atom + a2];
                            tyj = res_atype[t2 * tp.max_atom + a2];
                        }
                        const bool qj_on = fabs(qj) >= kErrorTol;
                        auto one_site = [&](double sx, double sy, double sz, double qs, int tys, double &elj_s, double &ec_s) {
                            const double2 pt = s_pair[tys * nt + tyj];
                            const bool do_c = qj_on && (fabs(qs) >= kErrorTol);
                            const bool do_lj = pt.x != 0.0;
                            if (valid && (do_lj || do_c))
                                pair_term<ORDERED, TRI, FASTW>(xj - sx, yj - sy, zj - sz, bx, qs * qj, pt.x, pt.y, do_lj, do_c, s_coul, elj_s, ec_s);
                        };
                        if constexpr (NS > 0) {
#pragma unroll
                            for (int s = 0; s < NREG; ++s) one_site(rx[s], ry[s], rz[s], rq[s % NTY], rty[s % NTY], elj[s / NTY], ec[s / NTY]);
                        } else {
                            for (int s = 0; s < ns; ++s)
                                one_site(w_site[s * 4 + 0], w_site[s * 4 + 1], w_site[s * 4 + 2], w_site[s * 4 + 3], w_sty[s], elj[0], ec[0]);
                        }
                    }
                }
            }
        }
#pragma unroll
        for (int st = 0; st < NST; ++st) {
            const double a = wave_sum(elj[st]), b = wave_sum(ec[st]);
            if (lane == 0) store_partial<SC1OUT>(partials + (size_t)w * NST + st, a, b);
        }
    }
}

template <int NS, bool ORDERED, bool TRI, bool FUSED = false, bool FASTW = false>
__global__ __launch_bounds__(kPairBlock, MGPU_PAIR_MINWAVES) void pair_sweep_kernel(
    Topo tp, BoxDev bx, const double *__restrict__ pos, const int *__restrict__ nmol,
    const double *__restrict__ res_q, const int *__restrict__ res_atype, const double2 *__restrict__ pair_tab,
    const char *__restrict__ coul_tab_g, const PairItem *__restrict__ items, const double *__restrict__ cand_sites,
    int site_stride, int nsplit, int n_work, double2 *__restrict__ partials) {
    constexpr int NST = FUSED ? 2 : 1;
    constexpr int NSLAB = NS > 0 ? 1 : kPairWaves * kSiteChunk;
    extern __shared__ __attribute__((aligned(16))) char s_coul[];
    __shared__ double2 s_pair[kMaxTypes * kMaxTypes];
    __shared__ double s_site[NSLAB * 4];
    __shared__ int s_sty[NSLAB];

    for (int i = threadIdx.x; i < (bx.coul_last_row + 1) * kCoulRowVec; i += kPairBlock)
        reinterpret_cast<double2 *>(s_coul)[i] = reinterpret_cast<const double2 *>(coul_tab_g)[i];
    const int nt = tp.n_types;
    for (int i = threadIdx.x; i < nt * nt; i += kPairBlock) s_pair[i] = pair_tab[i];
    __syncthreads();

    const int lane = threadIdx.x & 63;
    const int wave = __builtin_amdgcn_readfirstlane(threadIdx.x >> 6);
    const int n_waves = gridDim.x * kPairWaves;
    double *w_site = s_site + (NS > 0 ? 0 : wave * kSiteChunk * 4);
    int *w_sty = s_sty + (NS > 0 ? 0 : wave * kSiteChunk);

    for (int w = blockIdx.x * kPairWaves + wave; w < n_work; w += n_waves) {
        const int item_id = w / nsplit, split = w - item_id * nsplit;
        const PairItem it = items[item_id];
        pair_sweep_item<NS, ORDERED, TRI, FUSED, FASTW>(tp, bx, pos, nmol, res_q, res_atype, pair_tab, s_coul, s_pair, w_site, w_sty, it,
                                                        cand_sites, site_stride, split, nsplit, lane, partials, w);
    }
}


template <int NS, bool FUSED, bool FASTW, bool SC1OUT = false>
__device__ __forceinline__ void pair_flat_item(
    const Topo &tp, const BoxDev &bx, const double *__restrict__ pos, const int *__restrict__ nmol,
    const double *__restrict__ res_q, const int *__restrict__ res_atype, const char *__restrict__ s_coul,
    const double2 *__restrict__ s_pair, const int4 *__restrict__ s_grp, int4 *__restrict__ w_plane, const PairItem it,
    const double *__restrict__ cand_sites, int site_stride, int split, int nsplit, int lane, int skip_frozen,
    double2 *__restrict__ partials, int w) {
    static_assert(NS > 0, "register sites only");
    constexpr int NTY = NS;
    constexpr int NST = FUSED ? 2 : 1;
    constexpr int NREG = NTY * NST;
    const int nt = tp.n_types;
    const char *coul_adj = coul_tab_adjusted(s_coul, bx.coul_idx_base);
    {
        const double *px = pos + (size_t)it.replica * 3 * tp.n_cap_atoms;
        const double *py = px + tp.n_cap_atoms, *pz = py + tp.n_cap_atoms;
        const int *nm_r = nmol + it.replica * tp.n_res;
        int nmv[kMaxRes];
#pragma unroll
        for (int i = 0; i < kMaxRes; ++i) nmv[i] = i < tp.n_res ? nm_r[i] : 0;

        double rx[NREG], ry[NREG], rz[NREG], rq[NTY];
        int rty[NTY];
#pragma unroll
        for (int a = 0; a < NTY; ++a) {
            if constexpr (FUSED) {
                const int j = atom_slot(tp, it.t, it.m, a);
                rx[a] = px[j]; ry[a] = py[j]; rz[a] = pz[j];
                const double *c = cand_sites + ((size_t)it.src * site_stride + a) * 3;
                rx[NTY + a] = c[0]; ry[NTY + a] = c[1]; rz[NTY + a] = c[2];
            } else if (it.src < 0) {
                const int j = atom_slot(tp, it.t, it.m, a);
                rx[a] = px[j]; ry[a] = py[j]; rz[a] = pz[j];
            } else {
                const double *c = cand_sites + ((size_t)it.src * site_stride + a) * 3;
                rx[a] = c[0]; ry[a] = c[1]; rz[a] = c[2];
            }
            rq[a] = res_q[it.t * tp.max_atom + a];
            rty[a] = res_atype[it.t * tp.max_atom + a] * nt;
        }
#pragma unroll
        for (int k = 0; k < NREG; ++k) asm volatile("" : "+v"(rx[k]), "+v"(ry[k]), "+v"(rz[k]));
        bool any_c = false;
#pragma unroll
        for (int s = 0; s < NTY; ++s) {
            const bool on = fabs(rq[s]) >= kErrorTol;
            any_c = any_c || on;
            rq[s] = on ? rq[s] : 0.0;
        }

        int e_off = 0, e_cnt = 0, e_flags = 0;
        {
            int first = 0;
#pragma unroll
            for (int i = 0; i < kMaxRes; ++i) {
                const int nm2 = nmv[i];
                const bool frozen = tp.site_major[i] == 2;
                const int npl = nm2 == 0 ? 0 : (frozen ? nm2 * tp.n_grp[i] : tp.n1[i]);
                const bool same_t = (i == it.t) && (it.m >= 0);
                const int pl = lane - first;
                if (pl >= 0 && pl < npl) {
                    if (frozen) {
                        const int ng = tp.n_grp[i];
                        const int m2 = nm2 == 1 ? 0 : pl / ng;
                        const int4 gr = s_grp[tp.grp_off[i] + (pl - m2 * ng)];
                        e_off = tp.seg_off[i] + m2 * tp.n1[i] + gr.x;
                        e_cnt = ((same_t && m2 == it.m) || skip_frozen) ? 0 : gr.y;
                        e_flags = 0;
                    } else {
                        e_off = tp.seg_off[i] + pl * tp.cap[i];
                        e_cnt = (same_t && nm2 == 1) ? 0 : nm2;
                        e_flags = same_t ? (1 | ((it.m == 0 ? 1 : 0) << 1)) : 0;
                    }
                }
                first += npl;
            }
        }
        const int e_units = (e_cnt + 63) >> 6;
        int e_incl = e_units;
// ... 401 lines not shown
```

maniac_mc_amd/csrc/mgpu_lanes.hip:

```cpp
#include "mgpu_engine.h"

extern "C" {

static int frozen_batch_type(const mgpu_engine *e) {
    if (!e->pair_flat || !e->frozen_batch || e->bx.triclinic) return -1;
    int nf = 0, t_frozen = -1;
    for (int tt = 0; tt < e->tp.n_res; ++tt)
        if (e->frozen[tt]) { ++nf; t_frozen = tt; }
    if (nf != 1 || e->frozen_diff[t_frozen] != 0 || e->h_nmol[t_frozen] < 1) return -1;
    return t_frozen;
}


static int candidate_pair_items(const mgpu_engine *e, int n, const int *replica, const int *t, const int *m, const int *use_resident,
                                const double *sites, int site_stride, const char *who, std::vector<PairItem> &items, bool &any_sites) {
    items.resize(n);
    any_sites = false;
    for (int c = 0; c < n; ++c) {
        const bool res = use_resident && use_resident[c];
        if (int rc = check_candidate(e, c, replica[c], t[c], m[c], res)) return rc;
        if (!res) {
            any_sites = true;
            if (e->tp.n1[t[c]] > site_stride) return set_error(MGPU_ERR_INVALID_ARG, "site_stride smaller than atoms_in_res");
        }
// ... 28 lines not shown
        if (fast && !(use_resident && use_resident[c]))
            fast = sites_in_range(e, sites + (size_t)c * site_stride * 3, e->tp.n1[t[c]]);
    }
    if ((rc = launch_pair(e, e->lanes[0], (const PairItem *)e->d_items.p, n, common_site_count(e, items), site_stride, nsplit, d_lj, d_c,
                          false, nullptr, false, fast))) return rc;
    HIP_TRY(hipMemcpyAsync(e->h_out.p, e->d_out.p, (size_t)2 * n * sizeof(double), hipMemcpyDeviceToHost, e->stream));
    if ((rc = sync_stream(e))) return rc;
    std::memcpy(e_nc, e->h_out.p, n * sizeof(double));
    std::memcpy(e_c, (double *)e->h_out.p + n, n * sizeof(double));
    return MGPU_OK;
}

int mgpu_recip_energy_candidates(mgpu_engine *e, int n, const int *replica, const int *t, const int *m, const int *kind,
                                 const double *sites, int site_stride, double *u) {
    if (!e) return set_error(MGPU_ERR_INVALID_ARG, "null engine");
    if (n == 0) return MGPU_OK;
    if (n < 0 || !replica || !t || !m || !kind || !u) return set_error(MGPU_ERR_INVALID_ARG, "recip_energy_candidates: bad argument");
    int rc = use_device(e);
    if (rc) return rc;
    if ((rc = sync_all_lanes(e))) return rc;
    std::vector<RecipItem> items(n);
    bool any_sites = false;
    for (int c = 0; c < n; ++c) {
        if (kind[c] < MGPU_MOVE || kind[c] > MGPU_NONE) return set_error(MGPU_ERR_INVALID_ARG, "unknown candidate kind");
        const bool need_old = (kind[c] == MGPU_MOVE || kind[c] == MGPU_DELETION);
        const bool need_new = (kind[c] == MGPU_MOVE || kind[c] == MGPU_CREATION);
        if ((rc = check_candidate(e, c, replica[c], t[c], m[c], need_old))) return rc;
        if (need_new) {
            any_sites = true;
            if (e->tp.n1[t[c]] > site_stride) return set_error(MGPU_ERR_INVALID_ARG, "site_stride smaller than atoms_in_res");
        }
        items[c] = RecipItem{replica[c], t[c], m[c], kind[c], need_new ? c : -1, 0};
    }
    if (any_sites && !sites) return set_error(MGPU_ERR_INVALID_ARG, "recip_energy_candidates: sites is null");
    std::vector<RecipGroup> groups;
    std::vector<int> order;
    recip_groups(e, items.data(), n, groups, order);
    if (!order.empty()) {
        std::vector<RecipItem> by_form(n);
        for (int s = 0; s < n; ++s) by_form[s] = items[order[s]];
        items.swap(by_form);
    }
    if ((rc = e->d_items2.reserve(n * sizeof(RecipItem)))) return rc;
    if ((rc = e->d_out.reserve((size_t)n * sizeof(double)))) return rc;
    if ((rc = e->h_out.reserve((size_t)n * sizeof(double)))) return rc;
    HIP_TRY(hipMemcpyAsync(e->d_items2.p, items.data(), n * sizeof(RecipItem), hipMemcpyHostToDevice, e->stream));
    if (any_sites && (rc = upload_sites(e, sites, n, site_stride, t))) return rc;
    for (const RecipGroup &g : groups)
        if ((rc = launch_recip(e, e->lanes[0], (const RecipItem *)e->d_items2.p + g.first, g.n, g.n1_max, site_stride, false, e->d_A,
                               (double *)e->d_out.p + g.first)))
            return rc;
    HIP_TRY(hipMemcpyAsync(e->h_out.p, e->d_out.p, (size_t)n * sizeof(double), hipMemcpyDeviceToHost, e->stream));
    if ((rc = sync_stream(e))) return rc;
    if (order.empty()) std::memcpy(u, e->h_out.p, n * sizeof(double));
    else for (int s = 0; s < n; ++s) u[order[s]] = ((const double *)e->h_out.p)[s];
    return MGPU_OK;
}

int mgpu_recip_form(const mgpu_engine *e, int n1_max, int kind, int out[4]) {
    if (!e || !out) return set_error(MGPU_ERR_INVALID_ARG, "mgpu_recip_form: null argument");
    if (n1_max < 1) return set_error(MGPU_ERR_INVALID_ARG, "mgpu_recip_form: n1_max must be positive");
    if (kind != MGPU_RECIP_TRIAL && kind != MGPU_RECIP_COMMIT) return set_error(MGPU_ERR_INVALID_ARG, "mgpu_recip_form: unknown kind");
    const RecipPlan p = recip_plan(e, n1_max, true);
    if (p.lds > kLdsDefaultMax) return set_error(MGPU_ERR_CAPACITY, "mgpu_recip_form: kmax too large for the LDS phase tables");
    out[0] = p.form;
    out[2] = 0;
    out[3] = 1;
    switch (p.form) {
        case MGPU_RECIP_FORM_ROWS: out[1] = 2 * n1_max; out[2] = e->n_rrows; break;
        case MGPU_RECIP_FORM_WIDE_VECTOR: out[1] = 2 * n1_max; out[2] = p.wide_rpt; break;
        case MGPU_RECIP_FORM_PER_K: out[1] = 2 * p.tile; out[3] = (n1_max + p.tile - 1) / p.tile; break;
        default: out[1] = p.mfma_tile; out[3] = (((2 * n1_max + 3) & ~3) + p.mfma_tile - 1) / p.mfma_tile; break;
    }
    return MGPU_OK;
}

int mgpu_pair_layout(const mgpu_engine *e, int out[MGPU_PAIR_LAYOUT_LEN]) {
    if (!e || !out) return set_error(MGPU_ERR_INVALID_ARG, "mgpu_pair_layout: null argument");
    out[0] = e->pair_flat ? 1 : 0;
    out[1] = e->flat_groups;
    out[2] = e->flat_planes;
    out[3] = frozen_batch_type(e);
    for (int t = 0; t < kMaxRes; ++t) out[4 + t] = t < e->tp.n_res ? e->tp.site_major[t] : -1;
    return MGPU_OK;
}

int mgpu_self_energy(const mgpu_engine *e, int t, double *e_self) {
    if (!e || !e_self) return set_error(MGPU_ERR_INVALID_ARG, "mgpu_self_energy: null argument");
    if (t < 0 || t >= e->tp.n_res) return set_error(MGPU_ERR_INVALID_ARG, "residue type out of range");
    *e_self = self_energy_host(e, t);
    return MGPU_OK;
}

int mgpu_intra_energy_candidates(mgpu_engine *e, int n, const int *replica, const int *t, const int *m,
                                 const int *use_resident, const double *sites, int site_stride, double *u) {
    if (!e) return set_error(MGPU_ERR_INVALID_ARG, "null engine");
    if (n == 0) return MGPU_OK;
    if (n < 0 || !replica || !t || !m || !u) return set_error(MGPU_ERR_INVALID_ARG, "intra_energy_candidates: bad argument");
    int rc = use_device(e);
    if (rc) return rc;
    if ((rc = sync_all_lanes(e))) return rc;
    std::vector<PairItem> items;
    bool any_sites;
    if ((rc = candidate_pair_items(e, n, replica, t, m, use_resident, sites, site_stride, "intra_energy_candidates", items, any_sites))) return rc;
    if ((rc = e->d_items.reserve(n * sizeof(PairItem)))) return rc;
    if ((rc = e->d_out.reserve((size_t)n * sizeof(double)))) return rc;
    if ((rc = e->h_out.reserve((size_t)n * sizeof(double)))) return rc;
    HIP_TRY(hipMemcpyAsync(e->d_items.p, items.data(), n * sizeof(PairItem), hipMemcpyHostToDevice, e->stream));
    if (any_sites && (rc = upload_sites(e, sites, n, site_stride, t))) return rc;
    if ((rc = launch_intra(e, e->lanes[0], (const PairItem *)e->d_items.p, n, (const double *)e->d_sites.p, site_stride, (double *)e->d_out.p)))
        return rc;
    HIP_TRY(hipMemcpyAsync(e->h_out.p, e->d_out.p, (size_t)n * sizeof(double), hipMemcpyDeviceToHost, e->stream));
    if ((rc = sync_stream(e))) return rc;
    std::memcpy(u, e->h_out.p, n * sizeof(double));
    return MGPU_OK;
}

struct TrialBuild {
    const int *move;
    const double *u;
    double t_step, r_step;
};
struct TrialDecide {
    const double *u, *pref;
    double temperature;
};
constexpr double kSwitchMinShare = 0.5;

struct Seg { int n1, fused, first_item, n_items, first_entry, n_entries, type, nsplit, first_partial, batched; };
struct TrialPlan {
    int n = 0, n_cls = 0;
    int cls_n1[kMaxRes], cls_moves[kMaxRes], cls_single[kMaxRes], cls_type[kMaxRes];
    int seg_fused[kMaxRes], seg_single[kMaxRes];
    std::vector<Seg> segs;
    int n_pair = 0, n_partials = 0, n_intra = 0, n1_max = 1;
    bool fast = true;
    int t_frozen = -1, n_chunks_f = 0;
    size_t scratch_records = 0;
    TrialStaging in{};
    TrialResult out{};
};

static int trial_plan(const mgpu_engine *e, int n, const int *t, const int *kind, bool decide, TrialPlan &pl) {
    for (int c = 0; c < n; ++c) {
        const int k = kind ? kind[c] : MGPU_MOVE;
        if (k < MGPU_MOVE || k > MGPU_DELETION) return set_error(MGPU_ERR_INVALID_ARG, "trial_submit: unknown candidate kind");
        if (t[c] < 0 || t[c] >= e->tp.n_res) return set_error(MGPU_ERR_INVALID_ARG, "trial_submit: residue type out of range");
        const int n1 = e->tp.n1[t[c]];
        int ci = 0;
        while (ci < pl.n_cls && pl.cls_type[ci] != t[c]) ++ci;
        if (ci == pl.n_cls) { pl.cls_n1[ci] = n1; pl.cls_moves[ci] = 0; pl.cls_single[ci] = 0; pl.cls_type[ci] = t[c]; ++pl.n_cls; }
        const bool fz = k == MGPU_MOVE && n1 <= kMaxFusedSites && !e->bx.triclinic;
        if (fz) pl.cls_moves[ci] += 1;
        else pl.cls_single[ci] += (k == MGPU_MOVE) ? 2 : 1;
    }
    pl.t_frozen = frozen_batch_type(e);
    const int n_atoms_f = pl.t_frozen >= 0 ? e->h_nmol[pl.t_frozen] * e->tp.n1[pl.t_frozen] : 0;
    pl.n_chunks_f = pl.t_frozen >= 0 ? (n_atoms_f + frozen_chunk_atoms(e, n_atoms_f) - 1) / frozen_chunk_atoms(e, n_atoms_f) : 0;
    int n_items_total = 0;
    for (int ci = 0; ci < pl.n_cls; ++ci) {
        const int n1 = pl.cls_n1[ci], ty = pl.cls_type[ci];
        const int batched = pl.t_frozen >= 0 && ty != pl.t_frozen && n1 <= kMaxFusedSitesWide;
        const int ns_seg = batched ? 0 : e->pair_nsplit;
        auto add_seg = [&](int fused, int n_items, int &seg_of_class) {
            seg_of_class = n_items ? (int)pl.segs.size() : -1;
            if (!n_items) return;
// ... 726 lines not shown
```

maniac_mc_amd/csrc/mgpu_launch.hip:

```cpp
#include "mgpu_engine.h"

namespace mgpu {

template <auto Kernel>
int resident_blocks(Lane &ln, size_t dyn_lds) {
    const void *key = (const void *)Kernel;
    for (const auto &o : ln.occ)
        if (o.kernel == key && o.lds == dyn_lds) return o.blocks;
    int v = 0;
    if (hipOccupancyMaxActiveBlocksPerMultiprocessor(&v, Kernel, kPairBlock, dyn_lds) != hipSuccess || v < 1) v = 1;
    ln.occ.push_back({key, dyn_lds, std::min(v, 4)});
    return ln.occ.back().blocks;
}

int launch_pair(mgpu_engine *e, Lane &ln, const PairItem *d_items, int n_items, int common_n1, int site_stride,
                int nsplit, double *d_lj, double *d_c, bool ordered, double2 *host_partials, bool fused, bool fast_fold,
                bool skip_frozen) {
    const int n_work = n_items * nsplit;
    int rc = MGPU_OK;
    if (fused && (!host_partials || ordered || e->bx.triclinic || common_n1 < 1 || common_n1 > kMaxFusedSites))
        return set_error(MGPU_ERR_STATE, "launch_pair: fused sweep needs register sites, an orthorhombic box and a partials buffer");
    if (!host_partials && (rc = ln.d_partials.reserve((size_t)n_work * sizeof(double2)))) return rc;
    double2 *d_part = host_partials ? host_partials : (double2 *)ln.d_partials.p;
    const int per_cu = e->pair_blocks_per_cu;
    const int grid = std::max(1, std::min((n_work + kPairWaves - 1) / kPairWaves, e->n_cu * per_cu));
    hipEvent_t a = nullptr, b = nullptr;
    rc = prof_begin(e, ln, MGPU_KERNEL_PAIR, &a, &b);
    if (rc) return rc;
    auto launch = [&](auto kernel, int grid_k, auto... tail) {
        hipExtLaunchKernelGGL(kernel, dim3(grid_k), dim3(kPairBlock), e->coul_bytes, ln.stream, a, b, 0, e->tp, e->bx, e->d_pos, e->d_nmol,
                              e->d_res_q, e->d_res_atype, e->d_pair_tab, e->d_coul_tab, d_items, (const double *)ln.d_sites.p, site_stride,
                              nsplit, n_work, d_part, tail...);
    };
    const bool ff = fast_fold && !ordered && !e->bx.triclinic && e->pair_fast_fold;
    auto sweep = [&](auto NS, auto FU) {
        with_bools([&](auto FW) { launch(pair_sweep_kernel<decltype(NS)::value, false, false, decltype(FU)::value, decltype(FW)::value>, grid); }, ff);
    };
    auto flat_sweep = [&](auto NS, auto FU) {
        with_bools([&](auto FW) {
            constexpr auto kernel = &pair_flat_kernel<decltype(NS)::value, decltype(FU)::value, decltype(FW)::value>;
            const int nb = resident_blocks<kernel>(ln, e->coul_bytes);
            launch(kernel, std::max(1, std::min((n_work + kPairWaves - 1) / kPairWaves, e->n_cu * nb)), skip_frozen ? 1 : 0);
        }, ff);
    };
    const bool flat = e->pair_flat && !ordered && !e->bx.triclinic && common_n1 >= 1 && common_n1 <= kMaxFusedSitesWide;
    if (flat && fused) {
        with_int<1, kMaxFusedSites>(common_n1, [&](auto NS) { flat_sweep(NS, std::true_type{}); });
    } else if (flat) {
        with_int<1, kMaxFusedSitesWide>(common_n1, [&](auto NS) { flat_sweep(NS, std::false_type{}); });
    } else if (fused) {
        with_int<1, kMaxFusedSites>(common_n1, [&](auto NS) { sweep(NS, std::true_type{}); });
    } else if (e->bx.triclinic) {
        if (ordered) launch(pair_sweep_kernel<0, true, true>, grid);
        else if (!with_int<1, kMaxFusedSitesWide>(common_n1, [&](auto NS) { launch(pair_sweep_kernel<decltype(NS)::value, false, true>, grid); }))
            launch(pair_sweep_kernel<0, false, true>, grid);
    } else if (ordered) {
        launch(pair_sweep_kernel<0, true, false>, grid);
    } else if (!with_int<1, kMaxFusedSitesWide>(common_n1, [&](auto NS) { sweep(NS, std::false_type{}); })) {
        launch(pair_sweep_kernel<0, false, false>, grid);
    }
    rc = prof_end(e, ln, MGPU_KERNEL_PAIR, a, b);
    if (rc) return rc;
    if (!host_partials)
        hipLaunchKernelGGL(pair_finalize_kernel, dim3((n_items + 255) / 256), dim3(256), 0, ln.stream,
                           (const double2 *)ln.d_partials.p, n_items, nsplit, d_lj, d_c);
    HIP_TRY(hipGetLastError());
    return MGPU_OK;
}

int frozen_chunk_atoms(const mgpu_engine *e, int n_atoms) {
    const int n_slots = kPairWaves * std::max(1, (n_atoms + kPairWaves * 30 - 1) / (kPairWaves * 30));
    return std::max(1, std::min(64, (n_atoms + n_slots - 1) / n_slots));
}

int launch_frozen(mgpu_engine *e, Lane &ln, const PairItem *d_items, int n_items, int n1, int site_stride, bool fused, bool fast_fold,
                  int t_frozen, double2 *d_scratch, double2 *d_extra) {
    const int n_atoms = e->h_nmol[t_frozen] * e->tp.n1[t_frozen];
    const int chunk_atoms = frozen_chunk_atoms(e, n_atoms);
    const int n_chunks = (n_atoms + chunk_atoms - 1) / chunk_atoms;
    if (n_chunks == 0 || n_items == 0) return MGPU_OK;
    const int n_wg_units = ((n_items + 63) / 64) * ((n_chunks + kPairWaves - 1) / kPairWaves);
    const bool ff = fast_fold && e->pair_fast_fold;
    hipEvent_t a = nullptr, b = nullptr;
    int rc;
    {
        const size_t need = (size_t)((n_items + 63) / 64) * sizeof(int);
        const void *before = ln.d_tickets.p;
        if ((rc = ln.d_tickets.reserve(need))) return rc;
        if (ln.d_tickets.p != before) HIP_TRY(hipMemsetAsync(ln.d_tickets.p, 0, ln.d_tickets.bytes, ln.stream));
    }
    if ((rc = prof_begin(e, ln, MGPU_KERNEL_PAIR, &a, &b))) return rc;
    auto launch = [&](auto NS, auto FU) {
        with_bools([&](auto FW) {
            constexpr auto kernel = &pair_frozen_kernel<decltype(NS)::value, decltype(FU)::value, decltype(FW)::value>;
            const int nb = resident_blocks<kernel>(ln, e->coul_bytes);
            hipExtLaunchKernelGGL(kernel, dim3(std::max(1, std::min(n_wg_units, e->n_cu * nb))), dim3(kPairBlock), e->coul_bytes, ln.stream,
                                  a, b, 0, e->tp, e->bx, e->d_pos, e->d_nmol, e->d_res_q, e->d_res_atype, e->d_pair_tab, e->d_coul_tab,
                                  d_items, (const double *)ln.d_sites.p, site_stride, n_items, t_frozen, n_chunks, chunk_atoms, d_scratch,
                                  (int *)ln.d_tickets.p, d_extra, (const double *)e->d_atom_q_on, (const int *)e->tp.slot_ty);
        }, ff);
    };
    if (fused && n1 > kMaxFusedSites) return set_error(MGPU_ERR_STATE, "launch_frozen: fused items have at most three sites");
    const bool took = fused ? with_int<1, kMaxFusedSites>(n1, [&](auto NS) { launch(NS, std::true_type{}); })
                            : with_int<1, kMaxFusedSitesWide>(n1, [&](auto NS) { launch(NS, std::false_type{}); });
    if (!took) return set_error(MGPU_ERR_STATE, "launch_frozen: items of one to five register sites only");
    if ((rc = prof_end(e, ln, MGPU_KERNEL_PAIR, a, b))) return rc;
    HIP_TRY(hipGetLastError());
    return MGPU_OK;
}

bool recip_by_rows(const mgpu_engine *e, int n1_max) {
    return !e->recip_force_per_k && e->n_rtasks > 0 && recip_rows_lds_bytes(e, n1_max) <= kRecipRowsLdsMax;
}

static int wide_rows_per_tile(const mgpu_engine *e, int n1_max) {
    if (e->recip_force_per_k || e->n_rtasks <= 0 || !e->d_row_first) return 0;
    return recip_wide_rows_per_tile(recip_ktot(e), e->n_rrows, n1_max);
}

static int wide_mfma_tile(const mgpu_engine *e, int n1_max) {
    if (e->recip_force_per_k || e->recip_no_mfma || e->n_rtasks <= 0 || !e->d_row_first || !e->rows_contiguous) return 0;
    return recip_wide_mfma_tile(recip_ktot(e), e->n_rrows, n1_max);
}

RecipPlan recip_plan(const mgpu_engine *e, int n1_max, bool wide_ok) {
    RecipPlan p;
    const int ktot = recip_ktot(e);
    p.by_rows = recip_by_rows(e, n1_max);
    p.tile = p.by_rows ? n1_max : recip_tile_sites(ktot, n1_max);
    p.lds = p.by_rows ? recip_rows_lds_bytes(e, n1_max) : recip_lds_bytes(ktot, p.tile);
    const bool wide = wide_ok && !p.by_rows;
    p.mfma_tile = wide ? wide_mfma_tile(e, n1_max) : 0;
    p.wide_rpt = (wide && !p.mfma_tile) ? wide_rows_per_tile(e, n1_max) : 0;
    if (p.mfma_tile || p.wide_rpt) {
        p.wide_nss = p.mfma_tile ? p.mfma_tile : 2 * n1_max;
        p.wide_lds = recip_wide_lds_bytes(ktot, e->n_rrows, p.wide_nss, p.wide_rpt, p.mfma_tile > 0);
    }
    const int nss = ((2 * n1_max + 3) & ~3);
    if (p.by_rows) p.form = MGPU_RECIP_FORM_ROWS;
    else if (p.mfma_tile) p.form = p.mfma_tile < nss ? MGPU_RECIP_FORM_WIDE_MFMA_TILED : MGPU_RECIP_FORM_WIDE_MFMA;
    else if (p.wide_rpt) p.form = MGPU_RECIP_FORM_WIDE_VECTOR;
    else p.form = MGPU_RECIP_FORM_PER_K;
    return p;
// ... 153 lines not shown
```

maniac_mc_amd/csrc/mgpu_windows.hip:

```cpp
#include "mgpu_engine.h"

namespace mgpu {

int chain_topo(mgpu_engine *e, const Topo **d_topo) {
    mgpu_engine::Chain &ch = e->chain;
    if (!ch.d_topo) {
        HIP_TRY(hipMalloc((void **)&ch.d_topo, sizeof(Topo)));
        ch.topo_stale = true;
    }
    if (ch.topo_stale) {
        for (auto &ln : e->lanes) HIP_TRY(hipStreamSynchronize(ln.stream));
        HIP_TRY(hipMemcpy(ch.d_topo, &e->tp, sizeof(Topo), hipMemcpyHostToDevice));
        ch.topo_stale = false;
    }
    *d_topo = ch.d_topo;
    return MGPU_OK;
}

int normalize_A(mgpu_engine *e) {
    e->a_switched = false;
    if (!e->d_A_alt) return MGPU_OK;
    for (auto &ln : e->lanes) HIP_TRY(hipStreamSynchronize(ln.stream));
    hipLaunchKernelGGL(farm_normalize_kernel, dim3(e->n_replicas), dim3(kBlock), 0, e->lanes[0].stream, e->d_acur, e->d_A,
                       (const double2 *)e->d_A_alt, e->n_slots);
// ... 27 lines not shown
    if (e->farm.d_stalled) HIP_TRY(hipMemset(e->farm.d_stalled + replica, 0, sizeof(int)));
    mgpu_engine::Run &rn = e->run;
    if (rn.open && rn.replica == replica) {
        HIP_TRY(hipMemset(&rn.d_state->stalled, 0, sizeof(int)));
        rn.stalled_at = -1;
        rn.dev_stalled = false;
    }
    return MGPU_OK;
}

void chain_run_release(mgpu_engine *e) {
    mgpu_engine::Run &rn = e->run;
    for (void *p : {(void *)rn.h_ring, (void *)rn.h_pushed, (void *)rn.h_out, (void *)rn.h_step_tag, (void *)rn.h_launch})
        if (p) (void)hipHostFree(p);
    for (void *p : {(void *)rn.d_state, (void *)rn.d_ring, (void *)rn.d_part, (void *)rn.d_alt, (void *)rn.d_res, (void *)rn.d_ticket})
        if (p) (void)hipFree(p);
    rn = mgpu_engine::Run{};
}

int wait_for_tag(hipStream_t stream, const volatile unsigned long long *tag, int n, unsigned long long seq, long long first_check,
                 long long check_every, const char *what) {
    long long spins = 0;
    for (int c = 0; c < n; ++c) {
        while (tag[c] != seq) {
            __builtin_ia32_pause();
            if (++spins >= first_check && (spins % check_every) == 0) {
                const hipError_t q = hipStreamQuery(stream);
                if (q == hipSuccess && tag[c] != seq) return set_error(MGPU_ERR_HIP, std::string(what) + ": the kernel finished without publishing its results");
                if (q != hipSuccess && q != hipErrorNotReady) return set_error(MGPU_ERR_HIP, std::string(what) + ": " + hipGetErrorString(q));
            }
        }
    }
    __atomic_thread_fence(__ATOMIC_ACQUIRE);
    return MGPU_OK;
}

}

extern "C" {

struct FarmTypeForm {
    int form = kFarmFormRows, rpt = 0, nss = 0;
    size_t lds = 0;
};
static bool farm_type_form(const mgpu_engine *e, int t, FarmTypeForm &f) {
    const int n1 = e->tp.n1[t];
    if (e->tp.site_major[t] || n1 >= kFarmWideSites) return false;
    const RecipPlan p = recip_plan(e, n1, true);
    f = FarmTypeForm{};
    if (n1 <= kMaxFusedSitesWide) {
        if (p.form != MGPU_RECIP_FORM_ROWS) return false;
        f.lds = recip_rows_lds_bytes(e, n1);
        return true;
    }
    if (e->bx.triclinic) return false;
    switch (p.form) {
        case MGPU_RECIP_FORM_ROWS:
            f.lds = kFarmKFront + recip_rows_lds_bytes(e, n1);
            return true;
        case MGPU_RECIP_FORM_WIDE_VECTOR:
        case MGPU_RECIP_FORM_WIDE_MFMA:
            f.form = p.mfma_tile ? kFarmFormWideMfma : kFarmFormWideVector;
            f.rpt = p.wide_rpt; f.nss = p.wide_nss;
            f.lds = kFarmKFront + p.wide_lds;
            return true;
        default:
            return false;
    }
}


constexpr size_t kFarmWideStaticMax = 16 * 1024, kFarmWideLdsMax = 160 * 1024 - kFarmWideStaticMax;
static size_t chain_wide_lds(const mgpu_engine *e) {
    size_t lds = chain_wide_pair_lds_bytes(e->coul_bytes, kPairWaves, kSiteChunk);
    for (int t = 0; t < e->tp.n_res; ++t) {
        FarmTypeForm f;
        if (e->frozen[t] || !farm_type_form(e, t, f)) continue;
        lds = std::max(lds, e->tp.n1[t] > kMaxFusedSitesWide ? chain_wide_k_lds_bytes(f.lds - kFarmKFront) : f.lds);
    }
    return lds;
}

static int chain_max_candidates(const mgpu_engine *e) {
    int n1_max = 1;
    bool wide = false;
    for (int t = 0; t < e->tp.n_res; ++t) {
        if (!e->is_active[t]) continue;
        if (e->tp.site_major[t]) return 0;
        if (e->tp.n1[t] > kMaxFusedSitesWide) {
            FarmTypeForm f;
            if (!e->chain.wide || !farm_type_form(e, t, f)) return 0;
            wide = true;
            continue;
        }
        n1_max = std::max(n1_max, e->tp.n1[t]);
    }
    if (!recip_by_rows(e, n1_max)) return 0;
    if (e->coul_bytes > kLdsDefaultMax) return 0;
    if (wide && chain_wide_lds(e) > kFarmWideLdsMax) return 0;
    const int by_lds = chain_window_steps_by_lds(e->pair_nsplit);
    return std::max(0, std::min(kChainMaxCand, by_lds));
}

int mgpu_chain_set_wide(mgpu_engine *e, int on) {
    if (!e) return set_error(MGPU_ERR_INVALID_ARG, "null engine");
    e->chain.wide = on != 0;
    return MGPU_OK;
}

int mgpu_chain_window_capacity(const mgpu_engine *e, int *max_candidates) {
    if (!e || !max_candidates) return set_error(MGPU_ERR_INVALID_ARG, "chain_window_capacity: null argument");
    *max_candidates = chain_max_candidates(e);
    return MGPU_OK;
}

int mgpu_chain_set_margin(mgpu_engine *e, double relative_margin) {
    if (!e || !(relative_margin >= 0.0)) return set_error(MGPU_ERR_INVALID_ARG, "chain_set_margin: bad argument");
    e->chain.margin = relative_margin;
    return MGPU_OK;
}

int mgpu_chain_set_timing(mgpu_engine *e, int on) {
    if (!e) return set_error(MGPU_ERR_INVALID_ARG, "null engine");
    e->chain.timing = on != 0;
    return MGPU_OK;
}

int mgpu_chain_get_timing(mgpu_engine *e, double us[15]) {
    if (!e || !us) return set_error(MGPU_ERR_INVALID_ARG, "chain_get_timing: null argument");
    if (!e->chain.h_out) return set_error(MGPU_ERR_STATE, "chain_get_timing: no window has run");
    int rc = use_device(e);
    if (rc) return rc;
    HIP_TRY(hipStreamSynchronize(e->lanes[0].stream));
    const long long *ts = (const long long *)(e->chain.h_out + 10 * kChainMaxCand + 2);
    const long long t0 = std::min(ts[0], ts[kChainStamps]);
    const int first = ((const int *)(e->chain.h_out + 10 * (size_t)kChainMaxCand))[0];
    int k = 0;
    for (int i = 0; i < 4; ++i) us[k++] = (double)(ts[i] - t0) * 0.01;
    for (int i = 0; i < 4; ++i) us[k++] = (double)(ts[kChainStamps + i] - t0) * 0.01;
    for (int i = 0; i < 7; ++i) us[k++] = (i >= 5 && first < 0) ? 0.0 : (double)(ts[2 * kChainStamps + i] - t0) * 0.01;
    return MGPU_OK;
}

int mgpu_chain_get_stats(const mgpu_engine *e, long long *windows, long long *undecided) {
    if (!e) return set_error(MGPU_ERR_INVALID_ARG, "null engine");
    if (windows) *windows = e->chain.windows;
    if (undecided) *undecided = e->chain.undecided;
    return MGPU_OK;
}

int mgpu_chain_window(mgpu_engine *e, int replica, int n, const int *t, const int *m, const int *kind, const int *link,
                      const double *sites, int site_stride, const double *accept_u, const double *accept_pref,
                      double temperature, double recip_energy, double *old_energy, double *new_energy, int *first_accepted,
                      int *undecided) {
    if (!e) return set_error(MGPU_ERR_INVALID_ARG, "null engine");
    if (!t || !m || !kind || !link || !sites || !accept_u || !accept_pref || !old_energy || !new_energy || !first_accepted || !undecided)
        return set_error(MGPU_ERR_INVALID_ARG, "chain_window: null argument");
    const int n_max = chain_max_candidates(e);
    if (n_max == 0) return set_error(MGPU_ERR_STATE, "chain_window: not available for this engine (mgpu_chain_window_capacity)");
    if (n < 1 || n > n_max) return set_error(MGPU_ERR_INVALID_ARG, "chain_window: window size out of range");
    if (replica < 0 || replica >= e->n_replicas) return set_error(MGPU_ERR_INVALID_ARG, "chain_window: replica out of range");
    if (!(temperature > 0.0)) return set_error(MGPU_ERR_INVALID_ARG, "chain_window: temperature must be positive");
    int rc = use_device(e);
    if (rc) return rc;
    Lane &ln = e->lanes[0];
    if (ln.n_submitted != 0) return set_error(MGPU_ERR_STATE, "chain_window: lane 0 still holds an un-waited trial");
    mgpu_engine::Chain &ch = e->chain;
    if (!ch.h_tag) {
        HIP_TRY(hipHostMalloc((void **)&ch.h_out, sizeof(double) * (10 * kChainMaxCand + 2 + 3 * kChainStamps), hipHostMallocCoherent));
        std::memset(ch.h_out, 0, sizeof(double) * (10 * kChainMaxCand + 2 + 3 * kChainStamps));
        HIP_TRY(hipHostMalloc((void **)&ch.h_tag, 64, hipHostMallocCoherent));
        *ch.h_tag = 0;
        HIP_TRY(hipMalloc((void **)&ch.d_res, sizeof(ChainResult) * kChainMaxCand));
        HIP_TRY(hipMalloc((void **)&ch.d_part, sizeof(double2) * 2 * kChainMaxCand * (size_t)e->pair_nsplit));
        HIP_TRY(hipMalloc((void **)&ch.d_alt, sizeof(double2) * kChainMaxCand * (size_t)e->n_slots));
        HIP_TRY(hipMalloc((void **)&ch.d_ticket, sizeof(int)));
        HIP_TRY(hipMemset(ch.d_ticket, 0, sizeof(int)));
        HIP_TRY(hipDeviceSynchronize());
    }
    if (ch.wide && !ch.h_rows) {
        HIP_TRY(hipHostMalloc((void **)&ch.h_rows, 2 * kChainWideRowsBytes, hipHostMallocCoherent));
    }
    const Topo *d_topo = nullptr;
    if ((rc = chain_topo(e, &d_topo))) return rc;
    if (e->a_switched && (rc = normalize_A(e))) return rc;
    alt_forget(e, replica);
    ChainArgs g{};
    bool fast = replica_in_range(e, replica);
    char cand_ok[kChainMaxCand];
    int n1_max = 1, n_ent = 0;
    bool wide = false;
    double *wide_rows = ch.h_rows ? ch.h_rows + ((ch.seq + 1) & 1) * (kChainWideRowsBytes / sizeof(double)) : nullptr;
    for (int c = 0; c < n; ++c) {
        const int k = kind[c];
        if (k < MGPU_MOVE || k > MGPU_DELETION) return set_error(MGPU_ERR_INVALID_ARG, "chain_window: unknown candidate kind");
        if (t[c] < 0 || t[c] >= e->tp.n_res) return set_error(MGPU_ERR_INVALID_ARG, "chain_window: residue type out of range");
        const int n1 = e->tp.n1[t[c]];
        const bool wide_row = n1 > kMaxFusedSitesWide;
        FarmTypeForm tf;
        if (n1 > site_stride || e->tp.site_major[t[c]] || (wide_row && (!ch.wide || !farm_type_form(e, t[c], tf))))
            return set_error(MGPU_ERR_INVALID_ARG, "chain_window: molecule too large for the one-launch path");
        wide = wide || wide_row;
        const size_t idx = (size_t)replica * e->tp.n_res + t[c];
        if (e->d_com && e->frames_ok[idx])
            return set_error(MGPU_ERR_STATE, "chain_window: this replica holds molecule frames (mgpu_replica_set_frames)");
        const int lk = link[c];
        if (lk < -2 || lk >= n) return set_error(MGPU_ERR_INVALID_ARG, "chain_window: bad link");
        if (lk >= 0 && (k != MGPU_DELETION || link[lk] != -2 || kind[lk] != MGPU_CREATION || t[lk] != t[c]))
            return set_error(MGPU_ERR_INVALID_ARG, "chain_window: an as-written deletion links to an energy-only creation row of its type");
        if (lk == -2 && k != MGPU_CREATION) return set_error(MGPU_ERR_INVALID_ARG, "chain_window: energy-only rows are creation-kind");
        const int mc = (k == MGPU_CREATION) ? -1 : m[c];
        if ((rc = check_candidate(e, c, replica, t[c], mc, k != MGPU_CREATION))) return rc;
        if (k == MGPU_CREATION && lk != -2 && e->h_nmol[idx] >= e->tp.cap[t[c]])
            return set_error(MGPU_ERR_CAPACITY, "chain_window: residue type is at mol_capacity");
        if (!wide_row) n1_max = std::max(n1_max, n1);
        g.t[c] = t[c]; g.m[c] = mc; g.kind[c] = (signed char)k; g.link[c] = (signed char)lk;
        g.u[c] = accept_u[c]; g.pref[c] = accept_pref[c];
        const double *row = sites + (size_t)c * site_stride * 3;
        cand_ok[c] = 1;
        if (k != MGPU_DELETION) {
            if (e->frozen[t[c]]) return set_error(MGPU_ERR_INVALID_ARG, "chain_window: frozen residue types do not move");
            std::memcpy(wide_row ? wide_rows + (size_t)c * kFarmWideSites * 3 : &g.sites[c][0][0], row, (size_t)n1 * 3 * sizeof(double));
            cand_ok[c] = sites_in_range(e, row, n1) ? 1 : 0;
            if (lk != -2) fast = fast && cand_ok[c];
        }
        g.ent_old_of[c] = g.ent_new_of[c] = -1;
        if (lk == -2) continue;
        if (k != MGPU_CREATION) { g.ent_old_of[c] = (signed char)n_ent; g.ent_c[n_ent] = (unsigned char)c; g.ent_new[n_ent] = 0; ++n_ent; }
        if (k != MGPU_DELETION) { g.ent_new_of[c] = (signed char)n_ent; g.ent_c[n_ent] = (unsigned char)c; g.ent_new[n_ent] = 1; ++n_ent; }
    }
    const int nsplit = e->pair_nsplit;
    const size_t lds = std::max(wide ? chain_wide_lds(e) : std::max(e->coul_bytes, recip_rows_lds_bytes(e, n1_max)),
                                chain_resolver_lds_bytes(n_ent, nsplit));
    if (lds > (wide ? kFarmWideLdsMax : kLdsDefaultMax)) return set_error(MGPU_ERR_CAPACITY, "chain_window: the window does not fit the LDS budget");
    auto wide_family = [](auto &&f, auto FLAT, auto FASTW) { f(chain_window_kernel<decltype(FLAT)::value, decltype(FASTW)::value, false, true>); };
    if (lds > kLdsDefaultMax && lds > ch.wide_lds_opted) {
        hipError_t err = hipSuccess;
        auto opt_in = [&](auto kernel) {
            if (err == hipSuccess) err = hipFuncSetAttribute((const void *)kernel, hipFuncAttributeMaxDynamicSharedMemorySize, (int)lds);
        };
        for_all_bools([&](auto... flags) { wide_family(opt_in, flags...); }, std::integral_constant<int, 2>{});
        if (err != hipSuccess)
            return set_error(MGPU_ERR_HIP, std::string("hipFuncSetAttribute(k, hipFuncAttributeMaxDynamicSharedMemorySize, (int)lds): ") + hipGetErrorString(err));
        ch.wide_lds_opted = lds;
    }
    ch.seq += 1;
    for (int tt = 0; tt < e->tp.n_res; ++tt) g.self_of_type[tt] = e->self_of_type[tt];
    g.stamps = ch.timing ? 1 : 0;
    g.res = ch.d_res; g.partials = ch.d_part; g.ticket = ch.d_ticket; g.alt = ch.d_alt;
    g.host_out = ch.h_out; g.host_tag = ch.h_tag; g.seq = ch.seq;
    g.n = n; g.n_ent = n_ent; g.nsplit = nsplit; g.replica = replica;
    g.temperature = temperature; g.e_recip = recip_energy; g.margin = ch.margin;
    if (wide) {
        g.wide_sites = wide_rows;
        g.row_first = e->d_row_first;
        g.wide_at = (int)chain_wide_pair_at(e->coul_bytes);
        for (int tt = 0; tt < e->tp.n_res; ++tt) {
            FarmTypeForm f;
            if (!farm_type_form(e, tt, f)) continue;
            g.kform[tt] = (signed char)f.form; g.wide_rpt[tt] = f.rpt; g.wide_nss[tt] = f.nss;
        }
    }
    const int grid = n + (n_ent * nsplit + kPairWaves - 1) / kPairWaves;
    const bool ff = fast && e->pair_fast_fold;
    ln.dirty = true;
    ln.forget_trial();
    auto launch = [&](auto kernel) {
        hipLaunchKernelGGL(kernel, dim3(grid), dim3(kChainBlock), lds, ln.stream, d_topo, e->bx, e->d_pos, e->d_nmol, e->d_res_q, e->d_res_atype,
                           e->d_pair_tab, e->d_coul_tab, e->d_trj, e->d_tw, e->n_rtasks, e->d_rrows, e->n_rrows, e->d_A, g);
    };
    if (e->bx.triclinic) launch(chain_window_kernel<false, false, true>);
    else if (wide) with_bools([&](auto... flags) { wide_family(launch, flags...); }, e->pair_flat, ff);
    else with_bools([&](auto FLAT, auto FASTW) { launch(chain_window_kernel<decltype(FLAT)::value, decltype(FASTW)::value>); }, e->pair_flat, ff);
    HIP_TRY(hipGetLastError());
    if ((rc = wait_for_tag(ln.stream, ch.h_tag, 1, ch.seq, 20000, 4096, "chain_window"))) return rc;
    for (int c = 0; c < n; ++c) {
        std::memcpy(old_energy + 5 * (size_t)c, ch.h_out + 10 * (size_t)c, 5 * sizeof(double));
        std::memcpy(new_energy + 5 * (size_t)c, ch.h_out + 10 * (size_t)c + 5, 5 * sizeof(double));
    }
    const int *hi = (const int *)(ch.h_out + 10 * (size_t)kChainMaxCand);
    const int first = hi[0], und = hi[1];
    *first_accepted = first;
    *undecided = und;
    ch.windows += 1;
    if (und >= 0) ch.undecided += 1;
    if (first >= 0) {
        const size_t idx = (size_t)replica * e->tp.n_res + t[first];
        if (kind[first] == MGPU_CREATION) e->h_nmol[idx] += 1;
        if (kind[first] == MGPU_DELETION) e->h_nmol[idx] -= 1;
        if (kind[first] != MGPU_DELETION && !cand_ok[first]) e->in_range[idx] = 0;
        frozen_changed(e, replica, t[first]);
    }
    return MGPU_OK;
}



static size_t farm_wide_lds(const mgpu_engine *e) {
    size_t lds = ((e->coul_bytes + 15) & ~(size_t)15) + kFarmWidePairBytes;
    lds = std::max(lds, farm_resolver_scratch_bytes(e->pair_nsplit));
    for (int t = 0; t < e->tp.n_res; ++t) {
        FarmTypeForm f;
        if (!e->frozen[t] && farm_type_form(e, t, f)) lds = std::max(lds, f.lds);
    }
    return lds;
}

static int farm_max_chains(const mgpu_engine *e) {
    if (e->bx.triclinic && !e->tri_moves) return 0;
    bool wide = false;
    for (int t = 0; t < e->tp.n_res; ++t) {
        if (!e->is_active[t]) continue;
        FarmTypeForm f;
        if (!farm_type_form(e, t, f)) return 0;
        wide = wide || e->tp.n1[t] > kMaxFusedSitesWide;
    }
    if (e->coul_bytes > kLdsDefaultMax) return 0;
    if (farm_resolver_scratch_bytes(e->pair_nsplit) > kLdsDefaultMax) return 0;
    if (wide && farm_wide_lds(e) > kFarmWideLdsMax) return 0;
    return std::min(kFarmMaxChains, e->n_replicas);
}

int mgpu_farm_window_capacity(const mgpu_engine *e, int *max_chains, int *max_in_flight) {
    if (!e || !max_chains) return set_error(MGPU_ERR_INVALID_ARG, "farm_window_capacity: null argument");
    *max_chains = farm_max_chains(e);
    if (max_in_flight) *max_in_flight = kFarmDepth;
    return MGPU_OK;
}

int mgpu_farm_window_get_stats(const mgpu_engine *e, long long *windows, long long *undecided) {
    if (!e) return set_error(MGPU_ERR_INVALID_ARG, "null engine");
    if (windows) *windows = e->farm.windows;
    if (undecided) *undecided = e->farm.undecided;
    return MGPU_OK;
}

static int farm_lane(mgpu_engine *e, int lane, Lane **ln) {
    if (!e) return set_error(MGPU_ERR_INVALID_ARG, "null engine");
    if (lane < 0 || lane >= kLanes) return set_error(MGPU_ERR_INVALID_ARG, "lane out of range");
    *ln = &e->lanes[lane];
    return MGPU_OK;
}

static int farm_reserve(mgpu_engine *e, Lane &ln, int cap) {
    Lane::FarmWindow &fw = ln.farm;
    if (int rc = alt_reserve(e)) return rc;
    if (!e->farm.d_stalled) {
        HIP_TRY(hipMalloc((void **)&e->farm.d_stalled, (size_t)e->n_replicas * sizeof(int)));
        HIP_TRY(hipMemset(e->farm.d_stalled, 0, (size_t)e->n_replicas * sizeof(int)));
        HIP_TRY(hipDeviceSynchronize());
    }
    if (cap <= fw.cap) return MGPU_OK;
    if (!fw.pending.empty()) return set_error(MGPU_ERR_STATE, "farm_window_submit: a larger window than the lane's blocks while windows are in flight");
    HIP_TRY(hipStreamSynchronize(ln.stream));
    const unsigned long long seq = fw.seq;
    fw.release();
    fw.seq = seq;
    cap = std::max(cap, 64);
    HIP_TRY(hipHostMalloc((void **)&fw.h_recs, (size_t)kFarmDepth * cap * sizeof(FarmRec), hipHostMallocCoherent));
    HIP_TRY(hipHostMalloc((void **)&fw.h_out, (size_t)kFarmDepth * cap * kFarmOut * sizeof(double), hipHostMallocCoherent));
    HIP_TRY(hipHostMalloc((void **)&fw.h_tag, (size_t)kFarmDepth * cap * sizeof(unsigned long long), hipHostMallocCoherent));
    std::memset(fw.h_tag, 0xff, (size_t)kFarmDepth * cap * sizeof(unsigned long long));
    HIP_TRY(hipMalloc((void **)&fw.d_part, (size_t)cap * 2 * e->pair_nsplit * sizeof(double2)));
    HIP_TRY(hipMalloc((void **)&fw.d_res, (size_t)cap * sizeof(ChainResult)));
    HIP_TRY(hipMalloc((void **)&fw.d_tickets, (size_t)cap * sizeof(int)));
    HIP_TRY(hipMemset(fw.d_tickets, 0, (size_t)cap * sizeof(int)));
    HIP_TRY(hipMemset(fw.d_res, 0, (size_t)cap * sizeof(ChainResult)));
    HIP_TRY(hipDeviceSynchronize());
    fw.cap = cap;
    return MGPU_OK;
}

int mgpu_farm_window_submit(mgpu_engine *e, int lane, int n, const int *replica, const int *t, const int *m, const int *move,
                            const int *forced, const double *u5, const double *accept_u, const double *accept_pref,
                            const double *slot_u, double t_step, double r_step, double temperature) {
    Lane *lp = nullptr;
    int rc = farm_lane(e, lane, &lp);
    if (rc) return rc;
    Lane &ln = *lp;
    if (!replica || !t || !m || !move || !u5 || !accept_u || !accept_pref)
        return set_error(MGPU_ERR_INVALID_ARG, "farm_window_submit: null argument");
    const int n_max = farm_max_chains(e);
    if (n_max == 0) return set_error(MGPU_ERR_STATE, "farm_window_submit: not available for this engine (mgpu_farm_window_capacity)");
    if (n < 1 || n > n_max) return set_error(MGPU_ERR_INVALID_ARG, "farm_window_submit: number of chains out of range");
    if (!(temperature > 0.0)) return set_error(MGPU_ERR_INVALID_ARG, "farm_window_submit: temperature must be positive");
    if ((rc = use_device(e))) return rc;
    if (ln.n_submitted != 0) return set_error(MGPU_ERR_STATE, "farm_window_submit: the lane still holds an un-waited trial");
    Lane::FarmWindow &fw = ln.farm;
    if ((int)fw.pending.size() >= kFarmDepth) return set_error(MGPU_ERR_STATE, "farm_window_submit: too many windows of this lane in flight");
    if (!fw.pending.empty() && fw.pending.back().counts_change)
        return set_error(MGPU_ERR_STATE, "farm_window_submit: the lane's last window carries an insertion / deletion: collect it first");
    const Topo *d_topo = nullptr;
    {
        std::lock_guard<std::mutex> lock(e->farm.mu);
        if ((rc = farm_reserve(e, ln, n))) return rc;
        if ((rc = chain_topo(e, &d_topo))) return rc;
    }
    const int slot = (int)(fw.seq % kFarmDepth);
    Lane::FarmWindow::Pending pd;
    pd.seq = fw.seq + 1;
    pd.n = n; pd.slot = slot; pd.counts_change = false;
    pd.rep.assign(replica, replica + n);
    pd.t.assign(t, t + n);
    pd.kind.assign(n, -1);
    pd.ok.assign(n, 1);
    FarmArgs g{};
    FarmRec *recs = n <= kFarmInline ? g.inline_recs : fw.h_recs + (size_t)slot * fw.cap;
    bool fast = true;
    int n1_max = 1;
    std::string why;
    for (int c = 0; c < n; ++c) {
        FarmRec &r = recs[c];
        r = FarmRec{};
        const int mv = move[c];
        if (mv < 0 || mv > 4) { rc = set_error(MGPU_ERR_INVALID_ARG, "farm_window_submit: unknown move code"); break; }
        if (replica[c] < 0 || replica[c] >= e->n_replicas) { rc = set_error(MGPU_ERR_INVALID_ARG, "farm_window_submit: replica out of range"); break; }
        r.replica = replica[c];
        if (mv == 0) continue;
        if (t[c] < 0 || t[c] >= e->tp.n_res) { rc = set_error(MGPU_ERR_INVALID_ARG, "farm_window_submit: residue type out of range"); break; }
        const int n1 = e->tp.n1[t[c]];
        FarmTypeForm tf;
        if (!farm_type_form(e, t[c], tf) || e->frozen[t[c]]) { rc = set_error(MGPU_ERR_INVALID_ARG, "farm_window_submit: molecule too large for the one-launch path"); break; }
        const size_t idx = (size_t)replica[c] * e->tp.n_res + t[c];
        const int k = mv <= 2 ? MGPU_MOVE : (mv == 3 ? MGPU_CREATION : MGPU_DELETION);
        if ((rc = admit_built(e, idx, k, mv, kAdmitFrames, "farm_window_submit", "chain", c, why, pd.ok[c], fast))) { set_error(rc, why); break; }
        const int mc = k == MGPU_CREATION ? -1 : (slot_u ? 0 : m[c]);
        if (!slot_u) {
            if ((rc = check_candidate(e, c, replica[c], t[c], mc, k != MGPU_CREATION))) break;
            if (k == MGPU_CREATION && e->h_nmol[idx] >= e->tp.cap[t[c]]) { rc = set_error(MGPU_ERR_CAPACITY, "farm_window_submit: residue type is at mol_capacity"); break; }
            if (k != MGPU_MOVE) pd.counts_change = true;
        } else {
            if (!(slot_u[c] >= 0.0 && slot_u[c] < 1.0)) { rc = set_error(MGPU_ERR_INVALID_ARG, "farm_window_submit: slot_u must lie in [0, 1)"); break; }
            r.by_count = 1;
            r.sel_u = slot_u[c];
        }
        fast = fast && replica_in_range(e, replica[c]);
        if ((rc = admit_built(e, idx, k, mv, kAdmitInsertion | kAdmitRange, "farm_window_submit", "chain", c, why, pd.ok[c], fast))) { set_error(rc, why); break; }
        n1_max = std::max(n1_max, n1);
        pd.kind[c] = k;
        if (k != MGPU_DELETION && !pd.ok[c]) e->in_range[idx] = 0;
        r.t = t[c]; r.m = (k == MGPU_CREATION || slot_u) ? 0 : m[c]; r.move = mv;
        r.forced = forced ? forced[c] : 0;
        if (r.forced < 0 || r.forced > 2) { rc = set_error(MGPU_ERR_INVALID_ARG, "farm_window_submit: forced is 0, 1 (accept) or 2 (reject)"); break; }
        for (int d = 0; d < 5; ++d) r.u[d] = u5[5 * (size_t)c + d];
        r.acc_u = accept_u[c];
        r.pref = accept_pref[c];
    }
    if (rc) return rc;
    if (!one_record_per_replica(ln, e->n_replicas, replica, n)) return set_error(MGPU_ERR_INVALID_ARG, "farm_window_submit: more than one chain record for a replica");
    if (pd.counts_change && !fw.pending.empty())
        return set_error(MGPU_ERR_STATE, "farm_window_submit: a window with an insertion / deletion needs the lane's earlier windows collected "
                                         "(its molecule counts must be current)");
    const int nsplit = e->pair_nsplit;
    const bool wide = n1_max > kMaxFusedSitesWide;
    const size_t lds = wide ? farm_wide_lds(e)
                            : std::max(std::max(e->coul_bytes, recip_rows_lds_bytes(e, n1_max)), farm_resolver_scratch_bytes(nsplit));
    if (lds > (wide ? kFarmWideLdsMax : kLdsDefaultMax)) return set_error(MGPU_ERR_CAPACITY, "farm_window_submit: the window does not fit the LDS budget");
    auto tri_family = [](auto &&f, auto RSV) { f(farm_window_kernel<false, false, false, decltype(RSV)::value, true>); };
    auto wide_family = [](auto &&f, auto FLAT, auto FASTW, auto RSV) {
        f(farm_window_kernel<decltype(FLAT)::value, decltype(FASTW)::value, true, decltype(RSV)::value>);
    };
    auto narrow_family = [](auto &&f, auto FLAT, auto FASTW, auto RSV) {
        f(farm_window_kernel<decltype(FLAT)::value, decltype(FASTW)::value, false, decltype(RSV)::value>);
    };
    if (lds > kLdsDefaultMax) {
        hipError_t err = hipSuccess;
        auto opt_in = [&](auto kernel) {
            if (err == hipSuccess) err = hipFuncSetAttribute((const void *)kernel, hipFuncAttributeMaxDynamicSharedMemorySize, (int)lds);
        };
        for_all_bools([&](auto... flags) { wide_family(opt_in, flags...); }, std::integral_constant<int, 3>{});
        if (err != hipSuccess)
            return set_error(MGPU_ERR_HIP, std::string("hipFuncSetAttribute(k, hipFuncAttributeMaxDynamicSharedMemorySize, (int)lds): ") + hipGetErrorString(err));
    }
    fw.seq += 1;
    for (int tt = 0; tt < e->tp.n_res; ++tt) g.self_of_type[tt] = e->self_of_type[tt];
    g.recs = fw.h_recs + (size_t)slot * fw.cap;
    g.partials = fw.d_part; g.res = fw.d_res; g.tickets = fw.d_tickets;
    g.stalled = e->farm.d_stalled; g.acur = e->d_acur; g.A_alt = e->d_A_alt;
    g.host_out = fw.h_out + (size_t)slot * fw.cap * kFarmOut;
    g.host_tag = fw.h_tag + (size_t)slot * fw.cap;
    g.seq = pd.seq;
    g.n = n; g.nsplit = nsplit;
    g.t_step = t_step; g.r_step = r_step; g.temperature = temperature; g.margin = e->chain.margin;
    if (wide) {
        g.row_first = e->d_row_first;
        g.wide_at = (int)((e->coul_bytes + 15) & ~(size_t)15);
        for (int tt = 0; tt < e->tp.n_res; ++tt) {
            FarmTypeForm f;
            if (!farm_type_form(e, tt, f)) continue;
            g.kform[tt] = (signed char)f.form; g.wide_rpt[tt] = f.rpt; g.wide_nss[tt] = f.nss;
        }
    }
    const int wpc = 2 * nsplit;
    const int grid = (n * wpc + kPairWaves - 1) / kPairWaves + n;
    const bool ff = fast && e->pair_fast_fold;
    ln.dirty = true;
    ln.forget_trial();
    for (int c = 0; c < n; ++c) alt_forget(e, replica[c]);
    e->a_switched = true;
    auto launch = [&](auto kernel) {
        hipLaunchKernelGGL(kernel, dim3(grid), dim3(kChainBlock), lds, ln.stream, d_topo, e->bx, e->d_pos, e->d_nmol, e->d_res_q, e->d_res_atype,
                           e->d_pair_tab, e->d_coul_tab, e->d_trj, e->d_tw, e->n_rtasks, e->d_rrows, e->n_rrows, e->d_A, g);
    };
    if (e->bx.triclinic) with_bools([&](auto... flags) { tri_family(launch, flags...); }, e->rsv_any);
    else if (wide) with_bools([&](auto... flags) { wide_family(launch, flags...); }, e->pair_flat, ff, e->rsv_any);
    else with_bools([&](auto... flags) { narrow_family(launch, flags...); }, e->pair_flat, ff, e->rsv_any);
    HIP_TRY(hipGetLastError());
    fw.pending.push_back(std::move(pd));
    e->farm.windows += 1;
    return MGPU_OK;
}

int mgpu_farm_window_wait(mgpu_engine *e, int lane, double *old_energy, double *new_energy, int *verdict) {
    Lane *lp = nullptr;
    int rc = farm_lane(e, lane, &lp);
    if (rc) return rc;
    Lane &ln = *lp;
    if (!old_energy || !new_energy || !verdict) return set_error(MGPU_ERR_INVALID_ARG, "farm_window_wait: null argument");
    Lane::FarmWindow &fw = ln.farm;
    if (fw.pending.empty()) return set_error(MGPU_ERR_STATE, "farm_window_wait: no window of this lane is in flight");
    const Lane::FarmWindow::Pending &pd = fw.pending.front();
    const int n = pd.n;
    const double *out = fw.h_out + (size_t)pd.slot * fw.cap * kFarmOut;
    if ((rc = wait_for_tag(ln.stream, fw.h_tag + (size_t)pd.slot * fw.cap, n, pd.seq, 200000, 65536, "farm_window_wait"))) {
        fw.pending.pop_front();
        return rc;
    }
    for (int c = 0; c < n; ++c) {
        const double *o = out + (size_t)kFarmOut * c;
        std::memcpy(old_energy + 5 * (size_t)c, o, 5 * sizeof(double));
        std::memcpy(new_energy + 5 * (size_t)c, o + 5, 5 * sizeof(double));
        const int v = (int)o[10];
        verdict[c] = v;
        if (v == kFarmVerdictUndecided) e->farm.undecided += 1;
        if (v != kFarmVerdictAccepted) continue;
        const size_t idx = (size_t)pd.rep[c] * e->tp.n_res + pd.t[c];
        if (pd.kind[c] == MGPU_CREATION) e->h_nmol[idx] += 1;
        if (pd.kind[c] == MGPU_DELETION) e->h_nmol[idx] -= 1;
    }
    fw.pending.pop_front();
    return MGPU_OK;
}


static int run_max_k(const mgpu_engine *e) {
    if (e->rsv_any) return 0;
    if (e->bx.triclinic && !(e->run.triclinic && e->tri_moves)) return 0;
    for (int t = 0; t < e->tp.n_res; ++t) {
        if (!e->is_active[t]) continue;
        FarmTypeForm f;
        if (e->tp.n1[t] > kMaxFusedSitesWide || !farm_type_form(e, t, f)) return 0;
    }
    if (e->coul_bytes > kLdsDefaultMax) return 0;
    return std::max(0, std::min(kRunMaxK, chain_window_steps_by_lds(e->pair_nsplit)));
}

static void run_poll(mgpu_engine *e) {
    mgpu_engine::Run &rn = e->run;
    const volatile unsigned long long *info = rn.h_launch, *tag = rn.h_launch + kRunLaunchRing;
    while (rn.seq_done < rn.seq) {
        const unsigned long long s = rn.seq_done + 1;
        if (tag[s % kRunLaunchRing] != s) break;
        __atomic_thread_fence(__ATOMIC_ACQUIRE);
        const unsigned long long v = info[s % kRunLaunchRing];
        const int first = (int)(v >> 16), consumed = (int)((v >> 8) & 0xff), flags = (int)(v & 0xff);
        rn.launches += 1;
        rn.steps += consumed;
        if (flags & kRunTagVoid) rn.void_launches += 1;
        else if (flags & kRunTagStalled) rn.undecided += 1;
        rn.dev_stalled = (flags & kRunTagStalled) != 0;
        rn.log.emplace_back(first, consumed);
        if ((int)rn.log.size() > kRunLogMax) rn.log.pop_front();
        rn.seq_done = s;
    }
}

static int run_launch_one(mgpu_engine *e, int force_step, int force_verdict) {
    mgpu_engine::Run &rn = e->run;
    Lane &ln = e->lanes[0];
    const Topo *d_topo = nullptr;
    int rc = chain_topo(e, &d_topo);
    if (rc) return rc;
    const int nsplit = e->pair_nsplit;
    int n1_max = 1;
    for (int t = 0; t < e->tp.n_res; ++t)
        if (e->is_active[t]) n1_max = std::max(n1_max, e->tp.n1[t]);
    const size_t lds = std::max(std::max(e->coul_bytes, recip_rows_lds_bytes(e, n1_max)), chain_run_resolver_lds_bytes(rn.k, nsplit));
    if (lds > kLdsDefaultMax) return set_error(MGPU_ERR_CAPACITY, "chain_run_launch: the launch does not fit the LDS budget");
    ChainRunArgs g{};
    rn.seq += 1;
    g.state = rn.d_state; g.ring = rn.d_ring; g.partials = rn.d_part; g.res = rn.d_res; g.ticket = rn.d_ticket; g.alt = rn.d_alt;
    g.host_out = rn.h_out; g.step_tag = rn.h_step_tag;
    g.launch_info = rn.h_launch + rn.seq % kRunLaunchRing;
    g.launch_tag = rn.h_launch + kRunLaunchRing + rn.seq % kRunLaunchRing;
    g.seq = rn.seq;
    g.k = rn.k; g.nsplit = nsplit; g.replica = rn.replica; g.ring_steps = kRunRingSteps;
    g.force_step = force_step; g.force_verdict = force_verdict;
    g.t_step = rn.t_step; g.r_step = rn.r_step; g.temperature = rn.temperature; g.margin = e->chain.margin;
    const int grid = (rn.k * 2 * nsplit + kPairWaves - 1) / kPairWaves + rn.k;
    const bool ff = rn.fast && e->pair_fast_fold;
    ln.dirty = true;
    ln.forget_trial();
    alt_forget(e, rn.replica);
    auto tri_family = [](auto &&f) { f(chain_run_kernel<false, false, true>); };
    auto ortho_family = [](auto &&f, auto FLAT, auto FASTW) { f(chain_run_kernel<decltype(FLAT)::value, decltype(FASTW)::value>); };
    auto launch = [&](auto kernel) {
        hipLaunchKernelGGL(kernel, dim3(grid), dim3(kChainBlock), lds, ln.stream, d_topo, e->bx, e->d_pos, e->d_nmol, e->d_res_q, e->d_res_atype,
                           e->d_pair_tab, e->d_coul_tab, e->d_trj, e->d_tw, e->n_rtasks, e->d_rrows, e->n_rrows, e->d_A, g);
    };
    if (e->bx.triclinic) tri_family(launch);
    else with_bools([&](auto... flags) { ortho_family(launch, flags...); }, e->pair_flat, ff);
    HIP_TRY(hipGetLastError());
    return MGPU_OK;
}

int mgpu_chain_run_capacity(const mgpu_engine *e, int *max_k, int *max_in_flight, int *ring_steps) {
    if (!e || !max_k) return set_error(MGPU_ERR_INVALID_ARG, "chain_run_capacity: null argument");
    const int k = run_max_k(e);
    *max_k = k;
    if (max_in_flight) *max_in_flight = k ? kRunMaxInFlight : 0;
    if (ring_steps) *ring_steps = k ? kRunRingSteps : 0;
    return MGPU_OK;
}

int mgpu_chain_run_set_triclinic(mgpu_engine *e, int on) {
    if (!e) return set_error(MGPU_ERR_INVALID_ARG, "null engine");
    if (!e->bx.triclinic) return set_error(MGPU_ERR_STATE, "chain_run_set_triclinic: the box is orthorhombic");
    if (!e->tri_moves) return set_error(MGPU_ERR_STATE, "chain_run_set_triclinic: device-built triclinic moves are off (mgpu_set_triclinic_moves)");
    if (e->run.open) return set_error(MGPU_ERR_STATE, "chain_run_set_triclinic: a run is open");
    e->run.triclinic = on != 0;
    return MGPU_OK;
}

int mgpu_chain_run_open(mgpu_engine *e, int replica, int k, double t_step, double r_step, double temperature) {
    if (!e) return set_error(MGPU_ERR_INVALID_ARG, "null engine");
    mgpu_engine::Run &rn = e->run;
    const int k_max = run_max_k(e);
    if (k_max == 0) return set_error(MGPU_ERR_STATE, "chain_run_open: not available for this engine (mgpu_chain_run_capacity)");
    if (rn.open) return set_error(MGPU_ERR_STATE, "chain_run_open: a run is open (one per engine)");
    if (replica < 0 || replica >= e->n_replicas) return set_error(MGPU_ERR_INVALID_ARG, "chain_run_open: replica out of range");
    if (k < 1 || k > k_max) return set_error(MGPU_ERR_INVALID_ARG, "chain_run_open: steps per launch out of range");
    if (!(temperature > 0.0)) return set_error(MGPU_ERR_INVALID_ARG, "chain_run_open: temperature must be positive");
    for (int t = 0; t < e->tp.n_res; ++t)
        if (e->is_active[t] && (!e->d_com || !e->frames_ok[(size_t)replica * e->tp.n_res + t]))
            return set_error(MGPU_ERR_STATE, "chain_run_open: no molecule frames for this replica (mgpu_replica_set_frames)");
    int rc = use_device(e);
    if (rc) return rc;
    Lane &ln = e->lanes[0];
    if (ln.n_submitted != 0 || !ln.farm.pending.empty())
        return set_error(MGPU_ERR_STATE, "chain_run_open: lane 0 still holds an un-waited trial or farm window");
    if ((rc = sync_all_lanes(e))) return rc;
    if (!rn.d_state) {
        HIP_TRY(hipMalloc((void **)&rn.d_state, sizeof(RunState)));
        HIP_TRY(hipMalloc((void **)&rn.d_ring, sizeof(RunRec) * kRunRingSteps));
        HIP_TRY(hipHostMalloc((void **)&rn.h_ring, sizeof(RunRec) * kRunRingSteps, hipHostMallocDefault));
        HIP_TRY(hipHostMalloc((void **)&rn.h_pushed, sizeof(int) * kRunRingSteps, hipHostMallocDefault));
        HIP_TRY(hipHostMalloc((void **)&rn.h_out, sizeof(double) * kRunOut * kRunRingSteps, hipHostMallocCoherent));
        HIP_TRY(hipHostMalloc((void **)&rn.h_step_tag, sizeof(unsigned long long) * kRunRingSteps, hipHostMallocCoherent));
        HIP_TRY(hipHostMalloc((void **)&rn.h_launch, sizeof(unsigned long long) * 2 * kRunLaunchRing, hipHostMallocCoherent));
        std::memset(rn.h_launch, 0, sizeof(unsigned long long) * 2 * kRunLaunchRing);
        HIP_TRY(hipMalloc((void **)&rn.d_part, sizeof(double2) * 2 * kRunMaxK * (size_t)e->pair_nsplit));
        HIP_TRY(hipMalloc((void **)&rn.d_res, sizeof(ChainResult) * kRunMaxK));
        HIP_TRY(hipMalloc((void **)&rn.d_alt, sizeof(double2) * kRunMaxK * (size_t)e->n_slots));
        HIP_TRY(hipMalloc((void **)&rn.d_ticket, sizeof(int)));
        HIP_TRY(hipMemset(rn.d_ticket, 0, sizeof(int)));
    }
    const Topo *d_topo = nullptr;
    if ((rc = chain_topo(e, &d_topo))) return rc;
    HIP_TRY(hipMemset(rn.d_state, 0, sizeof(RunState)));
    HIP_TRY(hipDeviceSynchronize());
    std::memset(rn.h_step_tag, 0, sizeof(unsigned long long) * kRunRingSteps);
    rn.open = true;
    rn.replica = replica; rn.k = k;
    rn.t_step = t_step; rn.r_step = r_step; rn.temperature = temperature;
    rn.fast = replica_in_range(e, replica);
    rn.pushed = rn.collected = 0;
    rn.stalled_at = -1;
    rn.dev_stalled = false;
    rn.seq_done = rn.seq;
    rn.log.clear();
    return MGPU_OK;
}

int mgpu_chain_run_push(mgpu_engine *e, int n, const int *t, const int *m, const int *move, const double *u5, const double *accept_u) {
    if (!e) return set_error(MGPU_ERR_INVALID_ARG, "null engine");
    mgpu_engine::Run &rn = e->run;
    if (!rn.open) return set_error(MGPU_ERR_STATE, "chain_run_push: no run is open");
    if (n < 0 || (n > 0 && (!t || !m || !move || !u5 || !accept_u))) return set_error(MGPU_ERR_INVALID_ARG, "chain_run_push: bad argument");
    if (n == 0) return MGPU_OK;
    if (rn.pushed + n - rn.collected > kRunRingSteps)
        return set_error(MGPU_ERR_INVALID_ARG, "chain_run_push: beyond the ring (steps pushed and not yet collected: mgpu_chain_run_capacity)");
    if (rn.pushed + n >= (1ll << 30)) return set_error(MGPU_ERR_INVALID_ARG, "chain_run_push: too many steps in one run");
    int rc = use_device(e);
    if (rc) return rc;
    bool fast = rn.fast;
    for (int c = 0; c < n; ++c) {
        const int mv = move[c];
        if (mv == 3 || mv == 4) return set_error(MGPU_ERR_INVALID_ARG, "chain_run_push: insertions and deletions do not ride in a run (moves only)");
        if (mv < 0 || mv > 4) return set_error(MGPU_ERR_INVALID_ARG, "chain_run_push: unknown move code");
        if (mv == 0) continue;
        if (t[c] < 0 || t[c] >= e->tp.n_res || !e->is_active[t[c]] || e->frozen[t[c]])
            return set_error(MGPU_ERR_INVALID_ARG, "chain_run_push: residue type out of range or not active");
        if ((rc = check_candidate(e, c, rn.replica, t[c], m[c], true))) return rc;
        fast = fast && e->frames_tight[(size_t)rn.replica * e->tp.n_res + t[c]];
    }
    for (int c = 0; c < n; ++c) {
        RunRec &r = rn.h_ring[(rn.pushed + c) % kRunRingSteps];
        r = RunRec{};
        r.move = move[c];
        if (r.move == 0) continue;
        r.t = t[c]; r.m = m[c];
        for (int d = 0; d < 5; ++d) r.u[d] = u5[5 * (size_t)c + d];
        r.acc_u = accept_u[c];
        const size_t idx = (size_t)rn.replica * e->tp.n_res + t[c];
        if (!e->frames_tight[idx]) e->in_range[idx] = 0;
    }
    rn.fast = fast;
    Lane &ln = e->lanes[0];
    ln.dirty = true;
// ... 146 lines not shown
```

maniac_mc_amd/engine.py:

```python
from __future__ import annotations

import ctypes as C
from typing import Optional, Sequence

import numpy as np

from . import _lib
from ._lib import MGPU_CREATION, MGPU_DELETION, MGPU_MOVE, MGPU_NONE, check
from .system import System, Topology

_dp = C.POINTER(C.c_double)
_ip = C.POINTER(C.c_int)


def _d(a):
    return None if a is None else a.ctypes.data_as(_dp)


def _i(a):
    return None if a is None else a.ctypes.data_as(_ip)


def _ints(x, n=None):
    a = np.ascontiguousarray(np.atleast_1d(x), dtype=np.int32)
# ... 301 lines not shown
    def replace_molecule(self, replica, t, m_dst, m_src):
        check(self.L.mgpu_replica_replace_molecule(self.h, C.c_int(replica), C.c_int(t), C.c_int(m_dst),
                                                   C.c_int(m_src)))

    def kvectors(self):
        nk = self.nk
        kx = np.zeros(nk, np.int32); ky = np.zeros(nk, np.int32); kz = np.zeros(nk, np.int32)
        k2 = np.zeros(nk); ff = np.zeros(nk); w = np.zeros(nk)
        check(self.L.mgpu_engine_get_kvectors(self.h, _i(kx), _i(ky), _i(kz), _d(k2), _d(ff), _d(w)))
        return dict(kx=kx, ky=ky, kz=kz, k2mag=k2, form_factor=ff, weights=w)

    def system_energy(self, replica=0):
        out = np.zeros(6)
        check(self.L.mgpu_system_energy(self.h, C.c_int(replica), _d(out)))
        return dict(non_coulomb=out[0], coulomb=out[1], recip_coulomb=out[2], ewald_self=out[3],
                    intra_coulomb=out[4], total=out[5])

    def init_structure_factor(self, replica=0, full=True):
        check(self.L.mgpu_init_structure_factor(self.h, C.c_int(replica), C.c_int(1 if full else 0)))

    def structure_factor(self, replica=0):
        a = np.zeros((self.nk, 2))
        check(self.L.mgpu_get_structure_factor(self.h, C.c_int(replica), _d(a)))
        return a[:, 0] + 1j * a[:, 1]

    def set_structure_factor(self, z, replica=0):
        a = np.ascontiguousarray(np.stack([np.real(z), np.imag(z)], axis=1), dtype=np.float64)
        check(self.L.mgpu_set_structure_factor(self.h, C.c_int(replica), _d(a)))

    def _cand(self, replica, t, m, sites):
        m = _ints(m)
        n = m.shape[0]
        replica = _ints(replica, n)
        t = _ints(t, n)
        if sites is not None:
            sites = np.ascontiguousarray(sites, dtype=np.float64)
            if sites.ndim == 2:
                sites = sites[None]
            assert sites.shape[0] == n and sites.shape[2] == 3
        return n, replica, t, m, sites

    def pair_energy_candidates(self, replica, t, m, sites=None, use_resident=None):
        n, replica, t, m, sites = self._cand(replica, t, m, sites)
        if use_resident is None:
            use_resident = np.full(n, 1 if sites is None else 0, dtype=np.int32)
        use_resident = _ints(use_resident, n)
        e_nc = np.zeros(n); e_c = np.zeros(n)
        stride = 1 if sites is None else sites.shape[1]
        check(self.L.mgpu_pair_energy_candidates(self.h, C.c_int(n), _i(replica), _i(t), _i(m), _i(use_resident),
                                                 _d(sites), C.c_int(stride), _d(e_nc), _d(e_c)))
        return e_nc, e_c

    def recip_energy_candidates(self, replica, t, m, kind, sites=None):
        n, replica, t, m, sites = self._cand(replica, t, m, sites)
        kind = _ints(kind, n)
        u = np.zeros(n)
        stride = 1 if sites is None else sites.shape[1]
        check(self.L.mgpu_recip_energy_candidates(self.h, C.c_int(n), _i(replica), _i(t), _i(m), _i(kind),
                                                  _d(sites), C.c_int(stride), _d(u)))
        return u

    def intra_energy_candidates(self, replica, t, m, sites=None, use_resident=None):
        n, replica, t, m, sites = self._cand(replica, t, m, sites)
        if use_resident is None:
            use_resident = np.full(n, 1 if sites is None else 0, dtype=np.int32)
        use_resident = _ints(use_resident, n)
        u = np.zeros(n)
        stride = 1 if sites is None else sites.shape[1]
        check(self.L.mgpu_intra_energy_candidates(self.h, C.c_int(n), _i(replica), _i(t), _i(m), _i(use_resident),
                                                  _d(sites), C.c_int(stride), _d(u)))
        return u

    def recip_form(self, n1_max, commit=False):
        out = np.zeros(4, np.int32)
        check(self.L.mgpu_recip_form(self.h, C.c_int(int(n1_max)), C.c_int(_lib.RECIP_COMMIT if commit else _lib.RECIP_TRIAL), _i(out)))
        return dict(form=_lib.RECIP_FORMS[int(out[0])], site_states=int(out[1]), rows_per_tile=int(out[2]), site_tiles=int(out[3]))

    def pair_layout(self):
        out = np.zeros(_lib.PAIR_LAYOUT_LEN, np.int32)
        check(self.L.mgpu_pair_layout(self.h, _i(out)))
        return dict(flat=bool(out[0]), groups=int(out[1]), planes=int(out[2]), frozen_batch=int(out[3]),
                    site_major=[int(v) for v in out[4:4 + self.topo.n_res]])

    def self_energy(self, t):
        e = C.c_double()
        check(self.L.mgpu_self_energy(self.h, C.c_int(t), C.byref(e)))
        return e.value

    def trial_energy_candidates(self, replica, t, m, sites):
        n, replica, t, m, sites = self._cand(replica, t, m, sites)
        old = np.zeros((n, 3)); new = np.zeros((n, 3))
        check(self.L.mgpu_trial_energy_candidates(self.h, C.c_int(n), _i(replica), _i(t), _i(m), _d(sites),
                                                  C.c_int(sites.shape[1]), _d(old), _d(new)))
        return old, new

    def gcmc_trial(self, replica, t, m, kind, sites, lane=0):
        n, replica, t, m, sites = self._cand(replica, t, m, sites)
        kind = _ints(kind, n)
        old = np.zeros((n, 5)); new = np.zeros((n, 5))
        self._last_stride = sites.shape[1]
        check(self.L.mgpu_gcmc_trial_submit(self.h, C.c_int(lane), C.c_int(n), _i(replica), _i(t), _i(m), _i(kind),
                                            _d(sites), C.c_int(sites.shape[1])))
        check(self.L.mgpu_gcmc_trial_wait(self.h, C.c_int(lane), _d(old), _d(new)))
        return old, new

    def chain_window_capacity(self):
        n = C.c_int(0)
        check(self.L.mgpu_chain_window_capacity(self.h, C.byref(n)))
        return n.value

    def chain_window(self, replica, t, m, kind, sites, accept_u, accept_pref, temperature, recip_energy, link=None):
        kind = np.ascontiguousarray(kind, dtype=np.int32)
        n = kind.shape[0]
        t = _ints(t, n); m = _ints(m, n)
        link = _ints(-1 if link is None else link, n)
        sites = np.ascontiguousarray(sites, dtype=np.float64)
        assert sites.ndim == 3 and sites.shape[0] == n and sites.shape[2] == 3
        u = np.ascontiguousarray(accept_u, dtype=np.float64); pref = np.ascontiguousarray(accept_pref, dtype=np.float64)
        assert u.shape == (n,) and pref.shape == (n,)
        old = np.zeros((n, 5)); new = np.zeros((n, 5))
        first = C.c_int(-1); und = C.c_int(-1)
        check(self.L.mgpu_chain_window(self.h, C.c_int(int(replica)), C.c_int(n), _i(t), _i(m), _i(kind), _i(link), _d(sites),
                                       C.c_int(sites.shape[1]), _d(u), _d(pref), C.c_double(temperature), C.c_double(recip_energy),
                                       _d(old), _d(new), C.byref(first), C.byref(und)))
        return old, new, first.value, und.value

    def chain_set_margin(self, rel):
        check(self.L.mgpu_chain_set_margin(self.h, C.c_double(rel)))

    def chain_set_wide(self, on=True):
        check(self.L.mgpu_chain_set_wide(self.h, C.c_int(1 if on else 0)))

    def chain_set_timing(self, on=True):
        check(self.L.mgpu_chain_set_timing(self.h, C.c_int(1 if on else 0)))

    def chain_timing(self):
        us = np.zeros(15)
        check(self.L.mgpu_chain_get_timing(self.h, _d(us)))
        return us

    def chain_stats(self):
        w = C.c_longlong(0); u = C.c_longlong(0)
        check(self.L.mgpu_chain_get_stats(self.h, C.byref(w), C.byref(u)))
        return w.value, u.value

    def commit_lane(self, lane, replica, t, m, kind, accept, sites=None, sync=True):
        n, replica, t, m, sites = self._cand(replica, t, m, sites)
        kind = _ints(kind, n)
        accept = _ints(accept, n)
        stride = self._last_stride if sites is None else sites.shape[1]
        check(self.L.mgpu_commit_submit(self.h, C.c_int(lane), C.c_int(n), _i(replica), _i(t), _i(m), _i(kind),
                                        _d(sites), C.c_int(stride), _i(accept)))
        if sync:
            self.synchronize()

    def commit_candidates(self, replica, t, m, kind, sites, accept):
        n, replica, t, m, sites = self._cand(replica, t, m, sites)
        kind = _ints(kind, n)
        accept = _ints(accept, n)
        stride = 1 if sites is None else sites.shape[1]
        check(self.L.mgpu_commit_candidates(self.h, C.c_int(n), _i(replica), _i(t), _i(m), _i(kind), _d(sites),
                                            C.c_int(stride), _i(accept)))

    def ComputeSystemEnergy(self, replica=0):
        return self.system_energy(replica)

# ... 44 lines not shown
```

Measured before the change: 8.074 million.

## Add split-plane Coulomb table with degree-5 polynomial rows for pair sweep

```diff
diff --git a/include/maniac_gpu.h b/include/maniac_gpu.h
--- a/include/maniac_gpu.h
+++ b/include/maniac_gpu.h
@@ -47,6 +47,8 @@
                         double *weights);
 
 int mgpu_coulomb_table_eval(double alpha, double r2_max, int n, const double *r2, double *out);
+
+int mgpu_coulomb_table_split_eval(double alpha, double r2_max, int n, const double *r2, double *out);
 
 int mgpu_rng_seed_streams(long long seed, int n_streams, long long *state);
 int mgpu_rng_fill(long long *state, int n_streams, int n_per, double *out);
@@ -101,6 +103,8 @@
 
 #define MGPU_PAIR_LAYOUT_LEN 12
 int mgpu_pair_layout(const mgpu_engine *e, int out[MGPU_PAIR_LAYOUT_LEN]);
+
+int mgpu_pair_table_form(const mgpu_engine *e, int *form);
 
 int mgpu_self_energy(const mgpu_engine *e, int t, double *e_self);
 
diff --git a/maniac_mc_amd/_lib.py b/maniac_mc_amd/_lib.py
--- a/maniac_mc_amd/_lib.py
+++ b/maniac_mc_amd/_lib.py
@@ -21,11 +21,11 @@
 
 EXPORTS = [
     "mgpu_last_error", "mgpu_abi_version", "mgpu_device_count", "mgpu_box_prepare", "mgpu_ewald_setup",
-    "mgpu_ewald_kvectors", "mgpu_coulomb_table_eval", "mgpu_rng_seed_streams", "mgpu_rng_fill", "mgpu_host_prefetch", "mgpu_engine_create", "mgpu_engine_destroy", "mgpu_engine_get_ewald",
+    "mgpu_ewald_kvectors", "mgpu_coulomb_table_eval", "mgpu_coulomb_table_split_eval", "mgpu_rng_seed_streams", "mgpu_rng_fill", "mgpu_host_prefetch", "mgpu_engine_create", "mgpu_engine_destroy", "mgpu_engine_get_ewald",
     "mgpu_engine_get_kvectors", "mgpu_replica_set_molecules", "mgpu_replica_get_molecules",
     "mgpu_replica_num_molecules", "mgpu_replica_copy", "mgpu_system_energy", "mgpu_init_structure_factor",
     "mgpu_get_structure_factor", "mgpu_set_structure_factor", "mgpu_structure_factor_add", "mgpu_pair_energy_candidates",
-    "mgpu_recip_energy_candidates", "mgpu_recip_form", "mgpu_pair_layout", "mgpu_self_energy", "mgpu_intra_energy_candidates",
+    "mgpu_recip_energy_candidates", "mgpu_recip_form", "mgpu_pair_layout", "mgpu_pair_table_form", "mgpu_self_energy", "mgpu_intra_energy_candidates",
     "mgpu_trial_energy_candidates", "mgpu_commit_candidates", "mgpu_trial_submit", "mgpu_trial_wait",
     "mgpu_commit_submit", "mgpu_lane_site_buffer", "mgpu_set_host_team", "mgpu_set_triclinic_moves", "mgpu_replica_set_frames", "mgpu_replica_get_frames", "mgpu_replica_set_reservoir", "mgpu_replica_get_reservoir", "mgpu_farm_snapshot_submit", "mgpu_farm_snapshot_wait", "mgpu_move_trial_submit", "mgpu_move_trial_decide_submit", "mgpu_gcmc_trial_decide_submit", "mgpu_trial_decide_wait", "mgpu_gcmc_trial_submit", "mgpu_gcmc_trial_wait", "mgpu_replica_replace_molecule",
     "mgpu_replica_set_num_molecules", "mgpu_chain_window_capacity", "mgpu_chain_window", "mgpu_chain_set_margin", "mgpu_chain_set_wide",
diff --git a/maniac_mc_amd/csrc/mgpu_engine.h b/maniac_mc_amd/csrc/mgpu_engine.h
--- a/maniac_mc_amd/csrc/mgpu_engine.h
+++ b/maniac_mc_amd/csrc/mgpu_engine.h
@@ -224,6 +224,10 @@
     double2 *d_pair_tab = nullptr;
     char *d_coul_tab = nullptr;
     size_t coul_bytes = 0;
+    bool pair_split = false;
+    char *d_coul_split = nullptr;
+    int coul_split_rows = 0;
+    std::vector<const void *> split_opted;
     int n_cu = 256;
     int pair_blocks_per_cu = kPairBlock >= 1024 ? 1 : 2;
     int pair_nsplit = 1;
@@ -359,6 +363,8 @@
     return MGPU_OK;
 }
 int engine_nsplit(const mgpu_engine *e);
+bool engine_pair_split(const mgpu_engine *e, const int *is_active, bool table_fits);
+int refuse_split_form(const mgpu_engine *e, const char *who);
 void permute_frozen_rows(const mgpu_engine *e, double *rows, int n_rows, int site_stride, const int *t);
 bool any_frozen(const mgpu_engine *e, int n, const int *t);
 int upload_sites(Lane &ln, const double *sites, int n_rows, int site_stride);
diff --git a/maniac_mc_amd/csrc/mgpu_engine.hip b/maniac_mc_amd/csrc/mgpu_engine.hip
--- a/maniac_mc_amd/csrc/mgpu_engine.hip
+++ b/maniac_mc_amd/csrc/mgpu_engine.hip
@@ -117,6 +117,22 @@
             if (!(std::fabs(sites[3 * (size_t)i + d] - e->bx.ctr[d]) <= kFastFoldRange * e->bx.L[d])) return false;
     return true;
 }
+bool engine_pair_split(const mgpu_engine *e, const int *is_active, bool table_fits) {
+    bool ok = table_fits && e->box_type != 3 && !e->pair_flat;
+    for (int t = 0; t < e->tp.n_res; ++t) {
+        if (e->tp.site_major[t] != 0) ok = false;
+        if (is_active[t] != 0 && e->tp.n1[t] > kMaxFusedSites) ok = false;
+    }
+    bool want = e->n_replicas > kFarmMaxChains;
+    if (const char *ov = std::getenv("MGPU_PAIR_TABLE")) want = std::string(ov) == "split";
+    return ok && want;
+}
+int refuse_split_form(const mgpu_engine *e, const char *who) {
+    if (!e->pair_split) return MGPU_OK;
+    return set_error(MGPU_ERR_STATE, std::string(who) + ": the engine reads the split form of the Coulomb table (mgpu_pair_table_form), "
+                                     "the window kernels the 48-byte rows: create the engine with MGPU_PAIR_TABLE=rows");
+}
+
 bool replica_in_range(const mgpu_engine *e, int replica) {
     for (int t = 0; t < e->tp.n_res; ++t)
         if (!e->in_range[(size_t)replica * e->tp.n_res + t]) return false;
@@ -526,6 +542,17 @@
         if (e->coul_bytes + 16 * 1024 > 150 * 1024) return fail(set_error(MGPU_ERR_CAPACITY, "Coulomb table does not fit LDS"));
         HIP_TRY_E(hipMalloc(&e->d_coul_tab, e->coul_bytes));
         HIP_TRY_E(hipMemcpy(e->d_coul_tab, rows.data(), e->coul_bytes, hipMemcpyHostToDevice));
+        const double s_split = std::max(s_max, 1.0);
+        if (engine_pair_split(e, is_active, s_split < std::ldexp(1.0, kCoulEmin + (kCoulSplitMaxRows - 1) / (1 << kCoulSplitM)))) {
+            CoulSplitTable tab;
+            if (int rc2 = build_coulomb_table_split(e->alpha, s_split, tab)) return fail(rc2);
+            e->coul_split_rows = tab.n_rows();
+            const size_t plane = (size_t)tab.n_rows() * kCoulSplitEntry;
+            HIP_TRY_E(hipMalloc(&e->d_coul_split, 2 * plane));
+            HIP_TRY_E(hipMemcpy(e->d_coul_split, tab.a.data(), plane, hipMemcpyHostToDevice));
+            HIP_TRY_E(hipMemcpy(e->d_coul_split + plane, tab.b.data(), plane, hipMemcpyHostToDevice));
+            e->pair_split = true;
+        }
     }
     {
         hipDeviceProp_t prop;
@@ -586,7 +613,7 @@
     (void)hipSetDevice(e->device);
     for (auto &ln : e->lanes) if (ln.stream) (void)hipStreamSynchronize(ln.stream);
     for (void *p : {(void *)e->d_pos, (void *)e->d_nmol, (void *)e->d_A, (void *)e->d_kpack, (void *)e->d_kw,
-                    (void *)e->d_pair_tab, (void *)e->d_coul_tab, (void *)e->d_res_q, (void *)e->d_res_atype, (void *)e->d_atom_res,
+                    (void *)e->d_pair_tab, (void *)e->d_coul_tab, (void *)e->d_coul_split, (void *)e->d_res_q, (void *)e->d_res_atype, (void *)e->d_atom_res,
                     (void *)e->d_atom_mol, (void *)e->d_atom_q, (void *)e->d_atom_q_on, (void *)e->d_phase_tab, (void *)e->d_S, (void *)e->d_trj,
                     (void *)e->d_tw, (void *)e->d_kslot, (void *)e->d_rrows, (void *)e->d_row_first, (void *)e->d_atom_ty, (void *)e->d_com, (void *)e->d_off})
         if (p) (void)hipFree(p);
diff --git a/maniac_mc_amd/csrc/mgpu_host_setup.cpp b/maniac_mc_amd/csrc/mgpu_host_setup.cpp
--- a/maniac_mc_amd/csrc/mgpu_host_setup.cpp
+++ b/maniac_mc_amd/csrc/mgpu_host_setup.cpp
@@ -188,6 +188,142 @@
     return p;
 }
 
+int build_coulomb_table_split(double alpha, double s_max, CoulSplitTable &tab) {
+    if (!(alpha > 0.0) || !(s_max > 0.0) || !std::isfinite(s_max))
+        return set_error(MGPU_ERR_INVALID_ARG, "build_coulomb_table_split: bad alpha / range");
+    int emax = kCoulEmin;
+    while (emax < 64 && std::ldexp(1.0, emax + 1) <= s_max) ++emax;
+    const int per_oct = 1 << kCoulSplitM, n_oct = emax - kCoulEmin + 1;
+    if ((long long)n_oct * per_oct + 1 > kCoulSplitMaxRows) return set_error(MGPU_ERR_CAPACITY, "build_coulomb_table_split: range too large");
+    tab.a.assign((size_t)n_oct * per_oct + 1, CoulSplitA{});
+    tab.b.assign((size_t)n_oct * per_oct + 1, CoulSplitB{});
+    constexpr int N = kCoulSplitDeg + 1;
+    const long double pi = 3.14159265358979323846264338327950288L;
+    long double node[N], cosjk[N][N];
+    for (int k = 0; k < N; ++k) {
+        node[k] = cosl(pi * (2 * k + 1) / (2.0L * N));
+        for (int j = 0; j < N; ++j) cosjk[j][k] = cosl(pi * j * (2 * k + 1) / (2.0L * N));
+    }
+    long double T[N][N] = {};
+    T[0][0] = 1.0L;
+    T[1][1] = 1.0L;
+    for (int j = 2; j < N; ++j)
+        for (int i = 0; i < N; ++i) T[j][i] = (i > 0 ? 2.0L * T[j - 1][i - 1] : 0.0L) - T[j - 2][i];
+    long double binom[N][N] = {};
+    for (int j = 0; j < N; ++j) {
+        binom[j][0] = 1.0L;
+        for (int i = 1; i <= j; ++i) binom[j][i] = binom[j - 1][i - 1] + (i <= j - 1 ? binom[j - 1][i] : 0.0L);
+    }
+    auto to_row = [&](const long double *mono, long double *out) {
+        for (int i = 0; i < N; ++i) out[i] = 0.0L;
+        for (int j = 0; j < N; ++j)
+            for (int i = 0; i <= j; ++i) {
+                const long double sign = ((j - i) & 1) ? -1.0L : 1.0L;
+                out[i] += mono[j] * binom[j][i] * ldexpl(1.0L, i) * sign;
+            }
+    };
+    long double Ts[N][N];
+    for (int k = 0; k < N; ++k) to_row(T[k], Ts[k]);
+    auto settle = [&](long double *tc, int k, long double q) {
+        const long double d = tc[k] - q;
+        tc[k] = q;
+        for (int i = 0; i < k; ++i) tc[i] -= d * Ts[k][i] / ldexpl(1.0L, 2 * k - 1);
+    };
+    auto to_f32 = [](long double v) {
+        const float f = (float)v;
+        return std::fabs(f) < 1.17549435e-38f ? 0.0f : f;
+    };
+    const long double al = alpha;
+    for (int o = 0; o < n_oct; ++o)
+        for (int q = 0; q < per_oct; ++q) {
+            const long double base = ldexpl(1.0L, kCoulEmin + o);
+            const long double a = base * (1.0L + (long double)q / per_oct), b = base * (1.0L + (long double)(q + 1) / per_oct);
+            long double f[N], c[N], mono[N] = {}, tc[N];
+            for (int k = 0; k < N; ++k) {
+                const long double sv = 0.5L * (a + b) + 0.5L * (b - a) * node[k], r = sqrtl(sv);
+                f[k] = erfcl(al * r) / r;
+            }
+            for (int j = 0; j < N; ++j) {
+                long double acc = 0.0L;
+                for (int k = 0; k < N; ++k) acc += f[k] * cosjk[j][k];
+                c[j] = acc * 2.0L / N;
+            }
+            c[0] *= 0.5L;
+            for (int j = 0; j < N; ++j)
+                for (int i = 0; i <= j; ++i) mono[i] += c[j] * T[j][i];
+            to_row(mono, tc);
+            const int sh = kCoulSplitM - (kCoulEmin + o);
+            unsigned b5;
+            {
+                const float f5 = to_f32(ldexpl(tc[5], sh * 5));
+                unsigned u;
+                std::memcpy(&u, &f5, 4);
+                b5 = ((u + 0x8000u) >> 16) & 0xffffu;
+                u = b5 << 16;
+                float back;
+                std::memcpy(&back, &u, 4);
+                if (std::fabs(back) < 1.17549435e-38f || !std::isfinite(back)) { b5 = 0; back = 0.0f; }
+                settle(tc, 5, ldexpl((long double)back, -sh * 5));
+            }
+            const float c4 = to_f32(ldexpl(tc[4], sh * 4));
+            settle(tc, 4, ldexpl((long double)c4, -sh * 4));
+            const float c3 = to_f32(ldexpl(tc[3], sh * 3));
+            settle(tc, 3, ldexpl((long double)c3, -sh * 3));
+            double c2;
+            {
+                const long double want = ldexpl(tc[2], sh * 2);
+                const double near = (double)want;
+                unsigned long long u;
+                std::memcpy(&u, &near, 8);
+                const unsigned long long hi = u & ~0xffffull;
+                long double best_err = -1.0L;
+                c2 = 0.0;
+                for (int step = -1; step <= 1; ++step) {
+                    const unsigned long long cand = (hi + (unsigned long long)((long long)step * 0x10000ll)) | b5;
+                    double v;
+                    std::memcpy(&v, &cand, 8);
+                    const long double err = fabsl((long double)v - want);
+                    if (std::isfinite(v) && (best_err < 0.0L || err < best_err)) { best_err = err; c2 = v; }
+                }
+                settle(tc, 2, ldexpl((long double)c2, -sh * 2));
+            }
+            const size_t row = (size_t)o * per_oct + q;
+            tab.a[row] = CoulSplitA{(double)tc[0], (double)ldexpl(tc[1], sh)};
+            tab.b[row] = CoulSplitB{c2, c3, c4};
+        }
+    return MGPU_OK;
+}
+
+double coulomb_table_split_eval_host(const CoulSplitTable &tab, double alpha, double s) {
+    unsigned long long bits;
+    std::memcpy(&bits, &s, 8);
+    const int hi = (int)(bits >> 32);
+    int row = (hi >> (20 - kCoulSplitM)) - kCoulSplitIdxBase;
+    if (row < 0) {
+        const double r = std::sqrt(s);
+        return std::erfc(alpha * r) / r;
+    }
+    const int last = tab.n_rows() - 1;
+    if (row > last) row = last;
+    const unsigned long long ab = bits & ~((1ull << (52 - kCoulSplitM)) - 1);
+    double a;
+    std::memcpy(&a, &ab, 8);
+    const double t = s - a;
+    const CoulSplitA &ra = tab.a[row];
+    const CoulSplitB &rb = tab.b[row];
+    unsigned long long c2bits;
+    std::memcpy(&c2bits, &rb.c2, 8);
+    const unsigned u5 = (unsigned)(c2bits & 0xffffull) << 16;
+    float c5;
+    std::memcpy(&c5, &u5, 4);
+    double p = std::fma((double)c5, t, (double)rb.c4);
+    p = std::fma(p, t, (double)rb.c3);
+    p = std::fma(p, t, rb.c2);
+    p = std::fma(p, t, ra.c1);
+    p = std::fma(p, t, ra.c0);
+    return p;
+}
+
 }
 
 namespace {
@@ -317,6 +453,15 @@
     int rc = mgpu::build_coulomb_table(alpha, r2_max, rows, &idx_base);
     if (rc) return rc;
     for (int k = 0; k < n; ++k) out[k] = mgpu::coulomb_table_eval_host(rows, idx_base, alpha, r2[k]);
+    return MGPU_OK;
+}
+
+int mgpu_coulomb_table_split_eval(double alpha, double r2_max, int n, const double *r2, double *out) {
+    if (n < 0 || (n > 0 && (!r2 || !out))) return mgpu::set_error(MGPU_ERR_INVALID_ARG, "mgpu_coulomb_table_split_eval: bad argument");
+    mgpu::CoulSplitTable tab;
+    int rc = mgpu::build_coulomb_table_split(alpha, r2_max, tab);
+    if (rc) return rc;
+    for (int k = 0; k < n; ++k) out[k] = mgpu::coulomb_table_split_eval_host(tab, alpha, r2[k]);
     return MGPU_OK;
 }
 
diff --git a/maniac_mc_amd/csrc/mgpu_internal.h b/maniac_mc_amd/csrc/mgpu_internal.h
--- a/maniac_mc_amd/csrc/mgpu_internal.h
+++ b/maniac_mc_amd/csrc/mgpu_internal.h
@@ -34,6 +34,26 @@
 constexpr int kCoulRowVec = sizeof(CoulRow) / 16;
 int build_coulomb_table(double alpha, double s_max, std::vector<CoulRow> &rows, int *idx_base);
 double coulomb_table_eval_host(const std::vector<CoulRow> &rows, int idx_base, double alpha, double s);
+
+constexpr int kCoulSplitM = 8;
+constexpr int kCoulSplitDeg = 5;
+constexpr int kCoulSplitIdxBase = (1023 + kCoulEmin) << kCoulSplitM;
+constexpr int kCoulSplitMaxRows = 15 * (1 << kCoulSplitM) + 1;
+constexpr size_t kCoulSplitEntry = 16;
+constexpr size_t kCoulSplitPlaneBytes = (size_t)kCoulSplitMaxRows * kCoulSplitEntry;
+static_assert(kCoulSplitPlaneBytes <= 65535, "plane B must lie within the offset field of an LDS read");
+struct CoulSplitA { double c0, c1; };
+struct CoulSplitB { double c2; float c3, c4; };
+static_assert(sizeof(CoulSplitA) == kCoulSplitEntry && sizeof(CoulSplitB) == kCoulSplitEntry, "one 16-byte LDS read per plane");
+struct CoulSplitTable {
+    std::vector<CoulSplitA> a;
+    std::vector<CoulSplitB> b;
+    int n_rows() const { return (int)a.size(); }
+};
+int build_coulomb_table_split(double alpha, double s_max, CoulSplitTable &tab);
+double coulomb_table_split_eval_host(const CoulSplitTable &tab, double alpha, double s);
+constexpr int kPairSplitBlock = 1024;
+inline size_t pair_split_lds_bytes(int n_rows) { return kCoulSplitPlaneBytes + (size_t)n_rows * kCoulSplitEntry; }
 
 constexpr size_t kLdsDefaultMax = 64 * 1024;
 constexpr size_t kLdsPhase = 16, kLdsRowRec = 16;
diff --git a/maniac_mc_amd/csrc/mgpu_kernels_common.h b/maniac_mc_amd/csrc/mgpu_kernels_common.h
--- a/maniac_mc_amd/csrc/mgpu_kernels_common.h
+++ b/maniac_mc_amd/csrc/mgpu_kernels_common.h
@@ -252,6 +252,28 @@
     return p;
 }
 
+__device__ __forceinline__ const char *coul_split_adjusted(const char *plane_a) {
+    return plane_a - (size_t)kCoulSplitIdxBase * kCoulSplitEntry;
+}
+__device__ __forceinline__ double coul_lds_split(double s, const char *__restrict__ tab_adj, unsigned &sh_out) {
+    const int hi = __double2hiint(s);
+    const unsigned sh = (unsigned)hi >> (20 - kCoulSplitM);
+    sh_out = sh;
+    constexpr int kMant = (1 << (20 - kCoulSplitM)) - 1;
+    const double s0 = __hiloint2double(hi & ~kMant, 0);
+    const double t = s - s0;
+    const char *r = tab_adj + __umul24(sh, (unsigned)kCoulSplitEntry);
+    const double2 c01 = *reinterpret_cast<const double2 *>(r);
+    const double2 c2f = *reinterpret_cast<const double2 *>(r + kCoulSplitPlaneBytes);
+    const double c3 = (double)__int_as_float(__double2loint(c2f.y)), c4 = (double)__int_as_float(__double2hiint(c2f.y));
+    double p = fma((double)__int_as_float(__double2loint(c2f.x) << 16), t, c4);
+    p = fma(p, t, c3);
+    p = fma(p, t, c2f.x);
+    p = fma(p, t, c01.y);
+    p = fma(p, t, c01.x);
+    return p;
+}
+
 __device__ __attribute__((noinline)) double coul_slow(double s, double alpha, bool guard) {
     const double r = sqrt(s);
     if (guard && r < kErrorTol) return 0.0;
diff --git a/maniac_mc_amd/csrc/mgpu_kernels_pair.h b/maniac_mc_amd/csrc/mgpu_kernels_pair.h
--- a/maniac_mc_amd/csrc/mgpu_kernels_pair.h
+++ b/maniac_mc_amd/csrc/mgpu_kernels_pair.h
@@ -5,7 +5,7 @@
 
 namespace mgpu {
 
-template <int NS, bool ORDERED, bool TRI, bool FUSED, bool FASTW, bool SC1OUT = false>
+template <int NS, bool ORDERED, bool TRI, bool FUSED, bool FASTW, bool SC1OUT = false, bool SPLIT = false>
 __device__ __forceinline__ void pair_sweep_item(
     const Topo &tp, const BoxDev &bx, const double *__restrict__ pos, const int *__restrict__ nmol,
     const double *__restrict__ res_q, const int *__restrict__ res_atype, const double2 *__restrict__ pair_tab,
@@ -14,11 +14,13 @@
     double2 *__restrict__ partials, int w) {
     static_assert(!FUSED || (NS > 0 && !ORDERED && !TRI), "the fused old + new sweep is a register-site, unordered, orthorhombic path");
     static_assert(!FASTW || (NS > 0 && !ORDERED && !TRI), "the two-instruction fold is a register-site, unordered, orthorhombic path");
+    static_assert(!SPLIT || (NS > 0 && !ORDERED && !TRI), "the split table is a register-site, unordered, orthorhombic path");
     constexpr int NTY = NS > 0 ? NS : 1;
     constexpr int NST = FUSED ? 2 : 1;
     constexpr int NREG = NTY * NST;
     const int nt = tp.n_types;
-    [[maybe_unused]] const char *coul_adj = coul_tab_adjusted(s_coul, bx.coul_idx_base);
+    [[maybe_unused]] const char *coul_adj = SPLIT ? coul_split_adjusted(s_coul) : coul_tab_adjusted(s_coul, bx.coul_idx_base);
+    [[maybe_unused]] const unsigned coul_first = SPLIT ? (unsigned)kCoulSplitIdxBase : (unsigned)bx.coul_idx_base;
     {
         const double *px = pos + (size_t)it.replica * 3 * tp.n_cap_atoms;
         const double *py = px + tp.n_cap_atoms, *pz = py + tp.n_cap_atoms;
@@ -146,10 +148,10 @@
                             for (int s = 0; s < NREG; ++s) {
                                 if (!ALL_C && !c_on[s % NTY]) { g[s] = 0.0; continue; }
                                 unsigned sh;
-                                g[s] = coul_lds(r2[s], coul_adj, sh);
+                                g[s] = SPLIT ? coul_lds_split(r2[s], coul_adj, sh) : coul_lds(r2[s], coul_adj, sh);
                                 sh_min = min(sh_min, sh);
                             }
-                            if (sh_min < (unsigned)bx.coul_idx_base) {
+                            if (sh_min < coul_first) {
 #pragma unroll
                                 for (int s = 0; s < NREG; ++s)
                                     if ((ALL_C || c_on[s % NTY]) && r2[s] < kCoulSlowBelow) g[s] = coul_slow(r2[s], bx.alpha, ORDERED);
@@ -185,7 +187,7 @@
 #pragma unroll
                     for (int s = 0; s < NREG; ++s) ec[s / NTY] = fma(qq[s % NTY], acc[s], ec[s / NTY]);
                 };
-                if (!tp.site_major[t2]) {
+                if (SPLIT || !tp.site_major[t2]) {
                     if constexpr (NS > 0) {
                         const int cap2 = tp.cap[t2], seg2 = tp.seg_off[t2];
                         int dummy_m = 0;
@@ -295,6 +297,35 @@
         const PairItem it = items[item_id];
         pair_sweep_item<NS, ORDERED, TRI, FUSED, FASTW>(tp, bx, pos, nmol, res_q, res_atype, pair_tab, s_coul, s_pair, w_site, w_sty, it,
                                                         cand_sites, site_stride, split, nsplit, lane, partials, w);
+    }
+}
+
+template <int NS, bool FUSED, bool FASTW>
+__global__ __launch_bounds__(kPairSplitBlock, MGPU_PAIR_MINWAVES) void pair_sweep_split_kernel(
+    Topo tp, BoxDev bx, const double *__restrict__ pos, const int *__restrict__ nmol,
+    const double *__restrict__ res_q, const int *__restrict__ res_atype, const double2 *__restrict__ pair_tab,
+    const char *__restrict__ coul_split_g, const PairItem *__restrict__ items, const double *__restrict__ cand_sites,
+    int site_stride, int nsplit, int n_work, double2 *__restrict__ partials, int n_rows) {
+    constexpr int kWaves = kPairSplitBlock / 64;
+    extern __shared__ __attribute__((aligned(16))) char s_coul[];
+    __shared__ double2 s_pair[kMaxTypes * kMaxTypes];
+
+    for (int i = threadIdx.x; i < n_rows; i += kPairSplitBlock) {
+        reinterpret_cast<double2 *>(s_coul)[i] = reinterpret_cast<const double2 *>(coul_split_g)[i];
+        reinterpret_cast<double2 *>(s_coul + kCoulSplitPlaneBytes)[i] = reinterpret_cast<const double2 *>(coul_split_g)[n_rows + i];
+    }
+    const int nt = tp.n_types;
+    for (int i = threadIdx.x; i < nt * nt; i += kPairSplitBlock) s_pair[i] = pair_tab[i];
+    __syncthreads();
+
+    const int lane = threadIdx.x & 63;
+    const int wave = __builtin_amdgcn_readfirstlane(threadIdx.x >> 6);
+    const int n_waves = gridDim.x * kWaves;
+    for (int w = blockIdx.x * kWaves + wave; w < n_work; w += n_waves) {
+        const int item_id = w / nsplit, split = w - item_id * nsplit;
+        const PairItem it = items[item_id];
+        pair_sweep_item<NS, false, false, FUSED, FASTW, false, true>(tp, bx, pos, nmol, res_q, res_atype, pair_tab, s_coul, s_pair, nullptr,
+                                                                     nullptr, it, cand_sites, site_stride, split, nsplit, lane, partials, w);
     }
 }
 
diff --git a/maniac_mc_amd/csrc/mgpu_lanes.hip b/maniac_mc_amd/csrc/mgpu_lanes.hip
--- a/maniac_mc_amd/csrc/mgpu_lanes.hip
+++ b/maniac_mc_amd/csrc/mgpu_lanes.hip
@@ -134,6 +134,12 @@
     out[2] = e->flat_planes;
     out[3] = frozen_batch_type(e);
     for (int t = 0; t < kMaxRes; ++t) out[4 + t] = t < e->tp.n_res ? e->tp.site_major[t] : -1;
+    return MGPU_OK;
+}
+
+int mgpu_pair_table_form(const mgpu_engine *e, int *form) {
+    if (!e || !form) return set_error(MGPU_ERR_INVALID_ARG, "mgpu_pair_table_form: null argument");
+    *form = e->pair_split ? 1 : 0;
     return MGPU_OK;
 }
 
diff --git a/maniac_mc_amd/csrc/mgpu_launch.hip b/maniac_mc_amd/csrc/mgpu_launch.hip
--- a/maniac_mc_amd/csrc/mgpu_launch.hip
+++ b/maniac_mc_amd/csrc/mgpu_launch.hip
@@ -20,6 +20,8 @@
     int rc = MGPU_OK;
     if (fused && (!host_partials || ordered || e->bx.triclinic || common_n1 < 1 || common_n1 > kMaxFusedSites))
         return set_error(MGPU_ERR_STATE, "launch_pair: fused sweep needs register sites, an orthorhombic box and a partials buffer");
+    if (e->pair_split && !ordered && (common_n1 < 1 || common_n1 > kMaxFusedSites))
+        return set_error(MGPU_ERR_STATE, "launch_pair: on a split-form engine (mgpu_pair_table_form) a pair launch takes candidates of one site count, 1 to 3");
     if (!host_partials && (rc = ln.d_partials.reserve((size_t)n_work * sizeof(double2)))) return rc;
     double2 *d_part = host_partials ? host_partials : (double2 *)ln.d_partials.p;
     const int per_cu = e->pair_blocks_per_cu;
@@ -35,6 +37,26 @@
     const bool ff = fast_fold && !ordered && !e->bx.triclinic && e->pair_fast_fold;
     auto sweep = [&](auto NS, auto FU) {
         with_bools([&](auto FW) { launch(pair_sweep_kernel<decltype(NS)::value, false, false, decltype(FU)::value, decltype(FW)::value>, grid); }, ff);
+    };
+    auto split_sweep = [&](auto NS, auto FU) {
+        with_bools([&](auto FW) {
+            constexpr auto kernel = &pair_sweep_split_kernel<decltype(NS)::value, decltype(FU)::value, decltype(FW)::value>;
+            const size_t lds = pair_split_lds_bytes(e->coul_split_rows);
+            const void *key = (const void *)kernel;
+            if (std::find(e->split_opted.begin(), e->split_opted.end(), key) == e->split_opted.end()) {
+                const hipError_t err = hipFuncSetAttribute(key, hipFuncAttributeMaxDynamicSharedMemorySize, (int)lds);
+                if (err != hipSuccess) {
+                    rc = set_error(MGPU_ERR_HIP, std::string("hipFuncSetAttribute(pair_sweep_split_kernel, hipFuncAttributeMaxDynamicSharedMemorySize): ") + hipGetErrorString(err));
+                    return;
+                }
+                e->split_opted.push_back(key);
+            }
+            constexpr int waves = kPairSplitBlock / 64;
+            const int grid_s = std::max(1, std::min((n_work + waves - 1) / waves, e->n_cu));
+            hipExtLaunchKernelGGL(kernel, dim3(grid_s), dim3(kPairSplitBlock), lds, ln.stream, a, b, 0, e->tp, e->bx, e->d_pos, e->d_nmol,
+                                  e->d_res_q, e->d_res_atype, e->d_pair_tab, (const char *)e->d_coul_split, d_items, (const double *)ln.d_sites.p,
+                                  site_stride, nsplit, n_work, d_part, e->coul_split_rows);
+        }, ff);
     };
     auto flat_sweep = [&](auto NS, auto FU) {
         with_bools([&](auto FW) {
@@ -44,7 +66,10 @@
         }, ff);
     };
     const bool flat = e->pair_flat && !ordered && !e->bx.triclinic && common_n1 >= 1 && common_n1 <= kMaxFusedSitesWide;
-    if (flat && fused) {
+    if (e->pair_split && !ordered) {
+        if (fused) with_int<1, kMaxFusedSites>(common_n1, [&](auto NS) { split_sweep(NS, std::true_type{}); });
+        else with_int<1, kMaxFusedSites>(common_n1, [&](auto NS) { split_sweep(NS, std::false_type{}); });
+    } else if (flat && fused) {
         with_int<1, kMaxFusedSites>(common_n1, [&](auto NS) { flat_sweep(NS, std::true_type{}); });
     } else if (flat) {
         with_int<1, kMaxFusedSitesWide>(common_n1, [&](auto NS) { flat_sweep(NS, std::false_type{}); });
@@ -59,6 +84,7 @@
     } else if (!with_int<1, kMaxFusedSitesWide>(common_n1, [&](auto NS) { sweep(NS, std::false_type{}); })) {
         launch(pair_sweep_kernel<0, false, false>, grid);
     }
+    if (rc) return rc;
     rc = prof_end(e, ln, MGPU_KERNEL_PAIR, a, b);
     if (rc) return rc;
     if (!host_partials)
diff --git a/maniac_mc_amd/csrc/mgpu_windows.hip b/maniac_mc_amd/csrc/mgpu_windows.hip
--- a/maniac_mc_amd/csrc/mgpu_windows.hip
+++ b/maniac_mc_amd/csrc/mgpu_windows.hip
@@ -133,6 +133,7 @@
 }
 
 static int chain_max_candidates(const mgpu_engine *e) {
+    if (e->pair_split) return 0;
     int n1_max = 1;
     bool wide = false;
     for (int t = 0; t < e->tp.n_res; ++t) {
@@ -207,6 +208,7 @@
     if (!e) return set_error(MGPU_ERR_INVALID_ARG, "null engine");
     if (!t || !m || !kind || !link || !sites || !accept_u || !accept_pref || !old_energy || !new_energy || !first_accepted || !undecided)
         return set_error(MGPU_ERR_INVALID_ARG, "chain_window: null argument");
+    if (int rcs = refuse_split_form(e, "chain_window")) return rcs;
     const int n_max = chain_max_candidates(e);
     if (n_max == 0) return set_error(MGPU_ERR_STATE, "chain_window: not available for this engine (mgpu_chain_window_capacity)");
     if (n < 1 || n > n_max) return set_error(MGPU_ERR_INVALID_ARG, "chain_window: window size out of range");
@@ -358,6 +360,7 @@
 }
 
 static int farm_max_chains(const mgpu_engine *e) {
+    if (e->pair_split) return 0;
     if (e->bx.triclinic && !e->tri_moves) return 0;
     bool wide = false;
     for (int t = 0; t < e->tp.n_res; ++t) {
@@ -431,6 +434,7 @@
     Lane &ln = *lp;
     if (!replica || !t || !m || !move || !u5 || !accept_u || !accept_pref)
         return set_error(MGPU_ERR_INVALID_ARG, "farm_window_submit: null argument");
+    if ((rc = refuse_split_form(e, "farm_window_submit"))) return rc;
     const int n_max = farm_max_chains(e);
     if (n_max == 0) return set_error(MGPU_ERR_STATE, "farm_window_submit: not available for this engine (mgpu_farm_window_capacity)");
     if (n < 1 || n > n_max) return set_error(MGPU_ERR_INVALID_ARG, "farm_window_submit: number of chains out of range");
@@ -595,6 +599,7 @@
 
 
 static int run_max_k(const mgpu_engine *e) {
+    if (e->pair_split) return 0;
     if (e->rsv_any) return 0;
     if (e->bx.triclinic && !(e->run.triclinic && e->tri_moves)) return 0;
     for (int t = 0; t < e->tp.n_res; ++t) {
@@ -686,6 +691,7 @@
 int mgpu_chain_run_open(mgpu_engine *e, int replica, int k, double t_step, double r_step, double temperature) {
     if (!e) return set_error(MGPU_ERR_INVALID_ARG, "null engine");
     mgpu_engine::Run &rn = e->run;
+    if (int rcs = refuse_split_form(e, "chain_run_open")) return rcs;
     const int k_max = run_max_k(e);
     if (k_max == 0) return set_error(MGPU_ERR_STATE, "chain_run_open: not available for this engine (mgpu_chain_run_capacity)");
     if (rn.open) return set_error(MGPU_ERR_STATE, "chain_run_open: a run is open (one per engine)");
diff --git a/maniac_mc_amd/engine.py b/maniac_mc_amd/engine.py
--- a/maniac_mc_amd/engine.py
+++ b/maniac_mc_amd/engine.py
@@ -407,6 +407,11 @@
         return dict(flat=bool(out[0]), groups=int(out[1]), planes=int(out[2]), frozen_batch=int(out[3]),
                     site_major=[int(v) for v in out[4:4 + self.topo.n_res]])
 
+    def pair_table_form(self):
+        form = C.c_int()
+        check(self.L.mgpu_pair_table_form(self.h, C.byref(form)))
+        return "split" if form.value else "rows"
+
     def self_energy(self, t):
         e = C.c_double()
         check(self.L.mgpu_self_energy(self.h, C.c_int(t), C.byref(e)))
```

Measured after the change: 7.904 million. 2.1% lower.
